# cboin1996/avddpg

Hardware: AMD Instinct MI355X
Metric: env-steps/sec + DDPG updates/sec, 4096x5-vehicle platoons (higher is better)
Workload: dtype f32-class (fp16 hi+lo operand pairs on the 16-bit matrix cores, f32 accumulate)

## Files before the change

avddpg_amd/_hip.py:

```python
import ctypes as C
import os

_HERE = os.path.dirname(os.path.abspath(__file__))
LIB_PATH = os.path.join(_HERE, "lib", "libavddpg_hip.so")
if os.environ.get("AVDDPG_HIP_LIB"):
    LIB_PATH = os.path.abspath(os.environ["AVDDPG_HIP_LIB"])
HEADER_PATH = os.path.join(os.path.dirname(_HERE), "include", "avddpg_hip.h")
AVD_MAX_L = 16


class AvdError(RuntimeError):
    pass


class EnvConsts(C.Structure):
    _fields_ = [("L", C.c_int32), ("model_a", C.c_int32), ("can_terminate", C.c_int32), ("uniform_reset", C.c_int32),
                ("max_ep", C.c_float), ("max_ev", C.c_float), ("abs_action_high", C.c_float),
                ("two_max_a", C.c_float), ("T", C.c_float),
                ("ca", C.c_float), ("cb", C.c_float), ("cc", C.c_float), ("cd", C.c_float),
                ("re_scalar", C.c_float), ("terminal_reward", C.c_float),
                ("stand_still", C.c_float), ("timegap", C.c_float),
                ("reset_ep_max", C.c_float), ("reset_max_ev", C.c_float), ("reset_max_a", C.c_float),
                ("reset_ep_eval", C.c_float), ("reset_ev_eval", C.c_float), ("reset_a_eval", C.c_float),
                ("leader_reset_a", C.c_float),
                ("A", (C.c_float * 16) * AVD_MAX_L), ("B", (C.c_float * 4) * AVD_MAX_L),
                ("C", (C.c_float * 4) * AVD_MAX_L)]


_LAYOUT_FIELDS = ["S", "A", "H1", "H2", "Ha", "B",
                  "aW1", "ab1", "ag1", "abe1", "aW2", "ab2", "ag2", "abe2", "aW3", "ab3", "actor_size",
                  "cWs", "cbs", "cgs", "cbes", "cWa", "cba", "cga", "cbea", "cW2", "cb2", "cg3", "cbe3", "cW3", "cb3",
                  "theta_size",
                  "amm1", "amv1", "amm2", "amv2", "cmms", "cmvs", "cmma", "cmva", "cmm3", "cmv3", "stats_size"]


class MlpLayout(C.Structure):
    _fields_ = [(n, C.c_int32) for n in _LAYOUT_FIELDS]


_P = C.c_void_p
_i, _f, _d, _u64, _i64 = C.c_int, C.c_float, C.c_double, C.c_uint64, C.c_int64
_LP = C.POINTER(MlpLayout)

_PROTOS = {
    "avd_mlp_layout_init": [_LP, _i, _i, _i, _i, _i, _i],
    "avd_env_step_f32": [_P, _i, _i, _P, _P, _P, _P, _P, _P, _P, _P, _P, _P, _P, _P],
    "avd_env_reset_f32": [_P, _i, _i, _P, _P, _P, _P, _P, _i, _u64, _u64, _P, _P],
    "avd_episode_end_f32": [_P, _i, _i, _i, _P, _P, _P, _P, _P, _P, _i, _P, _P, _P, _P, _i, _u64, _u64, _P],
    "avd_ou_step_f32": [_i, _P, _P, _f, _f, _f, _f, _u64, _u64, _P],
    "avd_policy_f32": [_i, _P, _P, _f, _f, _P, _P],
    "avd_normal_f32": [_i, _P, _f, _u64, _u64, _P],
    "avd_uniform_f32": [_i, _P, _f, _u64, _u64, _P],
    "avd_step_fused_f32": [_P, _i, _i, _i, _P, _P, _P, _P, _P, _P, _P, _P, _P, _P, _P, _P, _P, _f, _f, _f, _f, _f, _f, _f, _i, _u64, _u64,
                           _u64, _P, _i, _i64, _P, _P],
    "avd_replay_sample_f32": [_i, _i, _i, _i, _i, _P, _i, _u64, _u64, _P, _P, _P, _P, _P, _P],
    "avd_actor_forward_set_f32": [_LP, _i, _i, _P, _P, _P, _i, _f, _P, _P, _P],
    "avd_replay_add_f32": [_i, _i, _i, _i, _P, _i64, _P, _P, _i, _P, _P, _P],
    "avd_replay_indices": [_i, _i, _i, _u64, _u64, _P, _P],
    "avd_replay_gather_f32": [_i, _i, _i, _i, _i, _P, _P, _P, _P, _P, _P, _P],
    "avd_actor_forward_f32": [_LP, _i, _i, _P, _P, _P, _i, _f, _P, _P],
    "avd_actor_forward_cond_f32": [_LP, _i, _i, _P, _P, _P, _i, _f, _P, _P, _P],
    "avd_critic_forward_f32": [_LP, _i, _i, _P, _P, _P, _i, _P, _P, _P],
    "avd_learn_f32": [_LP, _i, _i, _P, _P, _P, _P, _P, _P, _P, _P, _f, _f, _P, _P, _P],
    "avd_learn_update_f32": [_LP, _i, _P, _P, _P, _P, _P, _P, _P, _P, _P, _P, _P, _P, _f, _f, _f, _f, _d, _P, _P, _P],
    "avd_learn_update_act_f32": [_LP, _i, _P, _P, _P, _P, _P, _P, _P, _P, _P, _P, _P, _P, _f, _f, _f, _f, _d, _P, _P, _P, _i, _P, _P],
    "avd_learn_update_plan": [_LP, _i, C.POINTER(C.c_int), C.POINTER(C.c_int), C.POINTER(C.c_int)],
    "avd_adam_polyak_f32": [_LP, _i, _P, _P, _P, _P, _P, _P, _P, _P, _f, _f, _d, _P],
    "avd_adam_polyak_guarded_f32": [_LP, _i, _P, _P, _P, _P, _P, _P, _P, _P, _f, _f, _d, _P, _P],
    "avd_polyak_f32": [_i64, _P, _P, _d, _P],
    "avd_fed_sum_f32": [_i, _i, _i, _i, _i, _P, _P, _P, _P, _P],
    "avd_fed_finalize_f32": [_i, _i, _P, _f, _P, _P],
    "avd_fed_scatter_f32": [_i, _i, _i, _i, _i, _i, _P, _P, _P],
    "avd_adam_polyak_intra_f32": [_LP, _i, _i, _i, _P, _P, _P, _P, _P, _P, _P, _P, _P, _f, _f, _d, _P],
    "avd_fed_history_push_f32": [_i, _i, _i, _P, _P, _P, _i, _P, _i, _i, _P, _P, _P],
    "avd_fed_weights_f32": [_i, _i, _i, _P, _P, _i, _P, _P, _P, _P],
    "avd_learn_shared_workspace": [_LP, _i, _i, C.POINTER(C.c_size_t)],
    "avd_learn_shared_bf16": [_LP, _i, _i, _P, _P, _P, _P, _P, _P, _P, _P, _P, _f, _f, _P, _P, _P, C.c_size_t, _P],
    "avd_learn_set_fused_workspace": [_LP, _i, _i, C.POINTER(C.c_size_t)],
    "avd_learn_set_fused_bf16": [_LP, _i, _i, _P, _P, _P, _P, _P, _P, _P, _P, _P, _f, _f, _P, _P, _P, C.c_size_t, _P],
    "avd_learn_set_split_workspace": [_LP, _i, _i, C.POINTER(C.c_size_t)],
    "avd_learn_set_split_mfma_count": [_LP, _i, _i, C.POINTER(C.c_ulonglong)],
    "avd_learn_set_split_critic": [_LP, _i, _i, _P, _P, _P, _P, _P, _P, _P, _P, _P, _f, _f, _P, _P, _P, C.c_size_t, _P],
    "avd_learn_set_split_actor": [_LP, _i, _i, _P, _P, _P, _f, _P, _P, C.c_size_t, _P],
    "avd_learn_set_split_bf16x3": [_LP, _i, _i, _P, _P, _P, _P, _P, _P, _P, _P, _P, _f, _f, _P, _P, _P, C.c_size_t, _P],
    "avd_learn_set_split_f16x3": [_LP, _i, _i, _P, _P, _P, _P, _P, _P, _P, _P, _P, _f, _f, _P, _P, _P, C.c_size_t, _P],
    "avd_actor_forward_shared_workspace": [_LP, _i, _i, C.POINTER(C.c_size_t)],
    "avd_actor_forward_shared_bf16": [_LP, _i, _i, _P, _P, _P, _f, _P, _P, C.c_size_t, _P],
    "avd_eval_rollout_f32": [_LP, _P, _i, _i, _i, _i, _P, _P, _i, _P, _P, _P, _P, _i, _P, _f, _f, _f, _f, _P, _i, _P, _P, _P, _P,
                             _P],
    "avd_gemm_bt_bf16": [_i, _i, _i, _P, C.c_long, _P, C.c_long, _P, C.c_long, _P],
}

_lib = None
DIAG_LIB_PATH = os.path.join(_HERE, "lib", "libavddpg_hip_diag.so")


def _load(path):
    if not os.path.exists(path):
        raise AvdError(f"{path} not found: build the HIP extension first (__graft_entry__.build()); "
                       "avddpg_amd has no CPU fallback")
    l = C.CDLL(path)
    missing = []
    for name, args in _PROTOS.items():
        fn = getattr(l, name, None)
        if fn is None:
            missing.append(name)
            continue
        fn.argtypes = args
        fn.restype = C.c_int
    if missing and not os.environ.get("AVDDPG_HIP_LIB"):
        raise AvdError(f"{path} does not export {', '.join(missing)}: rebuild it (make -C avddpg_amd/csrc)")
    l.avd_last_error.restype = C.c_char_p
    l.avd_last_error.argtypes = []
    l.avd_version.restype, l.avd_version.argtypes = C.c_int, []
    if getattr(l, "avd_diagnostics_enabled", None) is None:
        l.avd_diagnostics_enabled = lambda: 0
    else:
        l.avd_diagnostics_enabled.restype, l.avd_diagnostics_enabled.argtypes = C.c_int, []
    return l


def lib():
    global _lib
    if _lib is None:
        _lib = _load(LIB_PATH)
    return _lib


class diag_library:
    _cached = None
    _stack = []

    def __enter__(self):
        global _lib, LIB_PATH
        if diag_library._cached is None:
            diag_library._cached = _load(DIAG_LIB_PATH)
            if not diag_library._cached.avd_diagnostics_enabled():
                raise AvdError(f"{DIAG_LIB_PATH} is not a diagnostic build")
        diag_library._stack.append((lib(), LIB_PATH))
        _lib, LIB_PATH = diag_library._cached, DIAG_LIB_PATH
        return _lib

    def __exit__(self, *exc):
        global _lib, LIB_PATH
        _lib, LIB_PATH = diag_library._stack.pop()
        return False


def call(name, *args):
    fn = getattr(lib(), name, None)
    if fn is None:
        raise AvdError(f"{name} is not exported by the loaded library (an older build?)")
    rc = fn(*args)
    if rc != 0:
        raise AvdError(f"{name} failed ({rc}): {lib().avd_last_error().decode()}")


def ptr(t):
    if t is None:
        return None
    if not t.is_contiguous():
        raise AvdError("non-contiguous tensor passed to the C ABI")
    return C.c_void_p(t.data_ptr())


def stream_handle():
    import torch
    return C.c_void_p(torch.cuda.current_stream().cuda_stream)


def make_layout(S, A, H1, H2, Ha, B):
    lay = MlpLayout()
    call("avd_mlp_layout_init", C.byref(lay), S, A, H1, H2, Ha, B)
    return lay
```

avddpg_amd/csrc/fset.hip:

```cpp
#include "fset_common.h"

namespace avd {
namespace fset {

__device__ __forceinline__ bf16x8 make_xf(float x0, float x1, float x2, float x3, int h) {
    const bf16 a0 = (bf16)x0, a1 = (bf16)x1, a2 = (bf16)x2, a3 = (bf16)x3;
    const bf16 l0 = (bf16)(x0 - (float)a0), l1 = (bf16)(x1 - (float)a1), l2 = (bf16)(x2 - (float)a2), l3 = (bf16)(x3 - (float)a3);
    const bf16 one = (bf16)1.f, zero = (bf16)0.f;
    bf16x8 v;
    v[0] = a0, v[1] = a1, v[2] = a2, v[3] = a3;
    v[4] = h ? one : l0, v[5] = h ? one : l1, v[6] = h ? zero : l2, v[7] = h ? zero : l3;
    return v;
}
__device__ __forceinline__ bf16x8 make_wf(float w0, float w1, float w2, float w3, float b, int h) {
    const bf16 a0 = (bf16)w0, a1 = (bf16)w1, a2 = (bf16)w2, a3 = (bf16)w3, bh = (bf16)b;
    const bf16 l0 = (bf16)(w0 - (float)a0), l1 = (bf16)(w1 - (float)a1), l2 = (bf16)(w2 - (float)a2), l3 = (bf16)(w3 - (float)a3);
    const bf16 bl = (bf16)(b - (float)bh), zero = (bf16)0.f;
    bf16x8 v;
    v[0] = h ? l0 : a0, v[1] = h ? l1 : a1, v[2] = h ? l2 : a2, v[3] = h ? l3 : a3;
    v[4] = h ? bh : a0, v[5] = h ? bl : a1, v[6] = h ? zero : a2, v[7] = h ? zero : a3;
    return v;
}

struct NetP {
// ... 412 lines not shown
    };
    bf16x8 nx0 = {}, nx1 = {};
    float na0 = 0.f, na1 = 0.f;
    auto fetch_x = [&](int agent) {
        const bf16x8* xa = (const bf16x8*)p.xf + (long)agent * TILE * 2;
        nx0 = xa[2 * r + h], nx1 = xa[2 * (32 + r) + h];
        if (act_tiles) na0 = p.act[(long)agent * TILE + r], na1 = p.act[(long)agent * TILE + 32 + r];
    };
    if (j0 < P) fetch(j0 * p.n_sets + set), fetch_x(j0 * p.n_sets + set), stage(0);
    __syncthreads();
    const int g4 = lane >> 4, q = (lane & 15) >> 2, pp = lane & 3;
    int buf = 0;
    for (int pi = j0; pi < P; pi += J, buf ^= 1) {
        const bool more = pi + J < P;
        const bf16x8 xs0 = nx0, xs1 = nx1;
        const bf16x8 xa0 = make_xf(na0, 0.f, 0.f, 0.f, h), xa1 = make_xf(na1, 0.f, 0.f, 0.f, h);
        if (more) fetch((pi + J) * p.n_sets + set), fetch_x((pi + J) * p.n_sets + set);
        bf16x8 bfr[2][2];
#pragma unroll
        for (int rh = 0; rh < 2; ++rh)
#pragma unroll
            for (int s = 0; s < 2; ++s)
#pragma unroll
                for (int hf = 0; hf < 2; ++hf) {
                    const int R0 = 32 * rh + 16 * s + 8 * hf + 4 * (g4 >> 1);
                    const bf16x4 t = __builtin_amdgcn_ds_read_tr16_b64_v4bf16(
                        (__attribute__((address_space(3))) bf16x4*)(dzimg[buf] + (R0 + q) * LDZ + 32 * wn + 16 * (g4 & 1) + 4 * pp));
#pragma unroll
                    for (int j = 0; j < 4; ++j) bfr[rh][s][4 * hf + j] = t[j];
                }
#pragma unroll
        for (int i = 0; i < NFW; ++i) {
            if (fg * NFW + i >= NGT) continue;
            const bool at = act_tiles && i >= 3;
#pragma unroll
            for (int rh = 0; rh < 2; ++rh) {
                const bf16x8 xf = rh ? (at ? xa1 : xs1) : (at ? xa0 : xs0);
                const f32x16 p1 = mfma(xf, wf[i], zero16);
#pragma unroll
                for (int s = 0; s < 2; ++s) {
                    uint4 xu;
                    xu.x = relu_bf16x2(p1[8 * s], p1[8 * s + 1]), xu.y = relu_bf16x2(p1[8 * s + 2], p1[8 * s + 3]);
                    xu.z = relu_bf16x2(p1[8 * s + 4], p1[8 * s + 5]), xu.w = relu_bf16x2(p1[8 * s + 6], p1[8 * s + 7]);
                    G[i] = mfma(__builtin_bit_cast(bf16x8, xu), bfr[rh][s], G[i]);
                }
            }
        }
        if (more) stage(buf ^ 1);
        __syncthreads();
    }
#pragma unroll
    for (int i = 0; i < NFW; ++i) {
        if (fg * NFW + i >= NGT) continue;
        float* dst = p.partG + ((long)blockIdx.x * KG + 32 * (fg * NFW + i)) * H2 + 32 * wn + r;
#pragma unroll
        for (int k = 0; k < 16; ++k) dst[(long)acc_row(k, h) * H2] = G[i][k];
    }
}

struct DxArgs {
    NetP net;
    int n_agents, n_sets;
    const bf16* xf;
    const float* x;
    const bf16* dz;
    float* partU;
    float* partV;
};
template <int S, class NET>
__global__ __launch_bounds__(NT) void dx_kernel(const DxArgs p) {
    constexpr int KP = NET::KP, NF = 2, LDZ = 136;
    __shared__ __attribute__((aligned(16))) bf16 dzimg[2][TILE * LDZ];
    __shared__ __attribute__((aligned(16))) bf16 xt[8][2][32 * 32];
    const int tid = threadIdx.x, w = tid >> 6, lane = tid & 63, r = lane & 31, h = lane >> 5, rh = w & 1, fg = w >> 1;
    const int set = blockIdx.x % p.n_sets, j0 = blockIdx.x / p.n_sets, J = gridDim.x / p.n_sets, P = p.n_agents / p.n_sets;
    const float* th = p.net.th + (long)set * p.net.th_stride;
    const f32x16 zero16 = {};
    bf16x8 w2[NF][8], wf[NF];
    f32x16 V[NF];
    float U0[NF], U1[NF];
#pragma unroll
    for (int i = 0; i < NF; ++i) {
        const int ft = fg + 4 * i;
        const bf16* src = p.net.W2R + ((long)set * KP + 32 * ft + r) * H2 + 8 * h;
#pragma unroll
        for (int s = 0; s < 8; ++s) w2[i][s] = *(const bf16x8*)(src + 16 * s);
        wf[i] = layer1_wf<S, NET>(p.net, th, ft, r, h);
        V[i] = zero16, U0[i] = 0.f, U1[i] = 0.f;
    }
    for (int i = lane; i < 2 * 32 * 32; i += 64) {
        const int k = (i >> 5) & 31;
        xt[w][0][i] = (bf16)(k == 8 ? 1.f : 0.f);
    }
    const int srow = tid >> 3, sch = tid & 7;
    uint4 d0 = {}, d1 = {};
    auto fetch = [&](int agent) {
        const uint4* src = (const uint4*)(p.dz + ((long)agent * TILE + srow) * H2 + 16 * sch);
        d0 = src[0], d1 = src[1];
    };
    auto stage = [&](int buf) {
        uint4* dst = (uint4*)(dzimg[buf] + srow * LDZ + 16 * sch);
        dst[0] = d0, dst[1] = d1;
    };
    bf16x8 xfn = {};
    auto fetch_x = [&](int agent) { xfn = ((const bf16x8*)p.xf)[((long)agent * TILE + 32 * rh + r) * 2 + h]; };
    auto stage_x = [&](int buf) {
        if (h == 0) {
#pragma unroll
            for (int k = 0; k < 8; ++k) xt[w][buf][k * 32 + r] = xfn[k];
        }
    };
    __syncthreads();
    if (j0 < P) fetch(j0 * p.n_sets + set), fetch_x(j0 * p.n_sets + set), stage(0), stage_x(0);
    __syncthreads();
    int buf = 0;
    for (int pi = j0; pi < P; pi += J, buf ^= 1) {
        const bool more = pi + J < P;
        const bf16x8 xf = xfn;
        if (more) fetch((pi + J) * p.n_sets + set), fetch_x((pi + J) * p.n_sets + set);
        bf16x8 dzf[8];
        const bf16* arow = dzimg[buf] + (32 * rh + r) * LDZ + 8 * h;
#pragma unroll
        for (int s = 0; s < 8; ++s) dzf[s] = *(const bf16x8*)(arow + 16 * s);
        bf16x8 xb[2];
#pragma unroll
        for (int s = 0; s < 2; ++s) {
            const bf16x4 lo = *(const bf16x4*)(&xt[w][buf][r * 32 + 16 * s + 4 * h]);
            const bf16x4 hi = *(const bf16x4*)(&xt[w][buf][r * 32 + 16 * s + 8 + 4 * h]);
#pragma unroll
            for (int j = 0; j < 4; ++j) xb[s][j] = lo[j], xb[s][4 + j] = hi[j];
        }
#pragma unroll
        for (int i = 0; i < NF; ++i) {
            f32x16 dc = zero16;
#pragma unroll
            for (int s = 0; s < 8; ++s) dc = mfma(dzf[s], w2[i][s], dc);
            const f32x16 p1 = mfma(xf, wf[i], zero16);
            float u0 = 0.f, u1 = 0.f;
            bf16x8 va[2];
#pragma unroll
            for (int k = 0; k < 16; ++k) {
                const float pr = relu(p1[k]);
                u0 += dc[k];
                u1 = fmaf(dc[k], pr, u1);
                va[k >> 3][k & 7] = (bf16)(pr > 0.f ? dc[k] : 0.f);
            }
            U0[i] += u0, U1[i] += u1;
            V[i] = mfma(va[0], xb[0], V[i]);
            V[i] = mfma(va[1], xb[1], V[i]);
        }
        if (more) stage(buf ^ 1), stage_x(buf ^ 1);
        __syncthreads();
    }
#pragma unroll
    for (int i = 0; i < NF; ++i) {
        const int ft = fg + 4 * i;
        float* pu = p.partU + ((((long)blockIdx.x * 2 + rh) * 2 + h) * KP + 32 * ft + r) * 2;
        pu[0] = U0[i], pu[1] = U1[i];
        if (r < 16) {
            float* pv = p.partV + (((long)blockIdx.x * 2 + rh) * KP + 32 * ft) * 16 + r;
#pragma unroll
            for (int k = 0; k < 16; ++k) pv[(long)acc_row(k, h) * 16] = V[i][k];
        }
    }
}

template <int S>
__global__ __launch_bounds__(NT) void dxa_kernel(const DxArgs p) {
    typedef Critic NET;
    constexpr int KP = NET::KP;
    __shared__ __attribute__((aligned(16))) bf16 xt[8][2][32 * 32];
    __shared__ float comb[4][64][2 + 16];
    const int tid = threadIdx.x, w = tid >> 6, lane = tid & 63, r = lane & 31, h = lane >> 5, rh = w & 1, ftl = (w >> 1) & 1, par = w >> 2;
    const int set = blockIdx.x % p.n_sets, j0 = blockIdx.x / p.n_sets, J = gridDim.x / p.n_sets, P = p.n_agents / p.n_sets;
    const float* th = p.net.th + (long)set * p.net.th_stride;
    const f32x16 zero16 = {};
    const int ft = 8 + ftl;
    bf16x8 w2[8];
    {
        const bf16* src = p.net.W2R + ((long)set * KP + 32 * ft + r) * H2 + 8 * h;
#pragma unroll
        for (int s = 0; s < 8; ++s) w2[s] = *(const bf16x8*)(src + 16 * s);
    }
    const bf16x8 wf = layer1_wf<S, NET>(p.net, th, ft, r, h);
    f32x16 V = zero16;
    float U0 = 0.f, U1 = 0.f;
    for (int i = lane; i < 2 * 32 * 32; i += 64) {
        const int k = (i >> 5) & 31;
        xt[w][0][i] = (bf16)(k == 8 ? 1.f : 0.f);
    }
    __syncthreads();
    const int ntile = j0 < P ? (P - j0 + J - 1) / J : 0;
    bf16x8 dzn[8];
    float an = 0.f;
    auto fetch = [&](int k) {
        const long ri = (long)((j0 + k * J) * p.n_sets + set) * TILE + 32 * rh + r;
        const bf16* src = p.dz + ri * H2 + 8 * h;
#pragma unroll
        for (int s = 0; s < 8; ++s) dzn[s] = *(const bf16x8*)(src + 16 * s);
        an = p.x[ri];
    };
    if (par < ntile) fetch(par);
    int buf = 0;
    for (int k = par; k < ntile; k += 2, buf ^= 1) {
        bf16x8 dzf[8];
#pragma unroll
        for (int s = 0; s < 8; ++s) dzf[s] = dzn[s];
        const bf16x8 xf = make_xf(an, 0.f, 0.f, 0.f, h);
        if (k + 2 < ntile) fetch(k + 2);
        if (h == 0) {
            xt[w][buf][r] = xf[0];
            xt[w][buf][4 * 32 + r] = xf[4];
        }
        __builtin_amdgcn_fence(__ATOMIC_RELEASE, "wavefront");
        __builtin_amdgcn_wave_barrier();
        bf16x8 xb[2];
#pragma unroll
        for (int s = 0; s < 2; ++s) {
            const bf16x4 lo = *(const bf16x4*)(&xt[w][buf][r * 32 + 16 * s + 4 * h]);
            const bf16x4 hi = *(const bf16x4*)(&xt[w][buf][r * 32 + 16 * s + 8 + 4 * h]);
#pragma unroll
            for (int j = 0; j < 4; ++j) xb[s][j] = lo[j], xb[s][4 + j] = hi[j];
        }
        f32x16 dc = zero16;
#pragma unroll
        for (int s = 0; s < 8; ++s) dc = mfma(dzf[s], w2[s], dc);
        const f32x16 p1 = mfma(xf, wf, zero16);
        float u0 = 0.f, u1 = 0.f;
        bf16x8 va[2];
#pragma unroll
        for (int i = 0; i < 16; ++i) {
            const float pr = relu(p1[i]);
            u0 += dc[i];
            u1 = fmaf(dc[i], pr, u1);
            va[i >> 3][i & 7] = (bf16)(pr > 0.f ? dc[i] : 0.f);
        }
        U0 += u0, U1 += u1;
        V = mfma(va[0], xb[0], V);
        V = mfma(va[1], xb[1], V);
    }
    const int pw = w & 3;
    if (par == 1) {
        comb[pw][lane][0] = U0, comb[pw][lane][1] = U1;
#pragma unroll
        for (int i = 0; i < 16; ++i) comb[pw][lane][2 + i] = V[i];
    }
    __syncthreads();
    if (par == 0) {
        U0 += comb[pw][lane][0], U1 += comb[pw][lane][1];
        float* pu = p.partU + ((((long)blockIdx.x * 2 + rh) * 2 + h) * KP + 32 * ft + r) * 2;
        pu[0] = U0, pu[1] = U1;
        if (r < 16) {
            float* pv = p.partV + (((long)blockIdx.x * 2 + rh) * KP + 32 * ft) * 16 + r;
#pragma unroll
            for (int i = 0; i < 16; ++i) pv[(long)acc_row(i, h) * 16] = V[i] + comb[pw][lane][2 + i];
        }
    }
}

__global__ __launch_bounds__(512) void finalize_small_kernel(const FinArgs a) {
    const int set = blockIdx.x, net = a.net_lo + blockIdx.y, tid = threadIdx.x, jl = tid & 31;
    const int item = a.item_base + blockIdx.z * 16 + (tid >> 5);
    const bool critic = net;
    const avd_mlp_layout& L = a.L;
    const float* th = a.theta + (long)set * L.theta_size + (critic ? L.actor_size : 0);
    const float* st = a.stats + (long)set * L.stats_size;
    float* g = a.grads + (long)set * L.theta_size + (critic ? L.actor_size : 0);
    const int K = critic ? Critic::K : Actor::K, KP = critic ? Critic::KP : Actor::KP;
    auto allsum = [&](float v) {
#pragma unroll
        for (int o = 1; o < 32; o <<= 1) v += __shfl_xor(v, o);
        return v;
    };
    if (item < H2) {
        const int n = item;
        const int og2 = critic ? L.cg3 : L.ag2, obe2 = critic ? L.cbe3 : L.abe2, omm2 = critic ? L.cmm3 : L.amm2, omv2 = critic ? L.cmv3 : L.amv2;
        const int oW3 = critic ? L.cW3 : L.aW3, ob3 = critic ? L.cb3 : L.ab3, ob2 = critic ? L.cb2 : L.ab2;
        const int KG = critic ? Critic::KG : Actor::KG;
        float T1 = 0.f, S2 = 0.f, D = 0.f, Lc = 0.f, La = 0.f;
        const bool t1g = a.t1_from_g[net] != 0;
        for (int j = jl; j < a.J; j += 32) {
            const long wg = (long)j * a.n_sets + set;
            for (int w = 0; w < 8; ++w) {
                if (!t1g) T1 += a.partH[net][(wg * 8 + w) * H2 + n];
                D += a.partHs[net][(wg * 8 + w) * 2];
                if (critic && n == 0) Lc += a.partHs[1][(wg * 8 + w) * 2 + 1], La += a.partLa[(wg * 8 + w) * 2 + 1];
            }
            S2 += a.partG[net][(wg * KG + K) * H2 + n];
        }
        T1 = allsum(T1), S2 = allsum(S2), D = allsum(D);
        if (t1g && jl == 0) a.s2raw[((long)net * a.n_sets + set) * H2 + n] = S2;
        if (a.c3[net]) S2 *= a.c3[net][(long)set * VEC + H2 + n];
        if (critic && n == 0) Lc = allsum(Lc), La = allsum(La);
        if (a.bad && *a.bad) T1 = S2 = D = Lc = La = __uint_as_float(0x7fc00000u);
        if (jl == 0) {
            const float rs2 = 1.0f / sqrtf(st[omv2 + n] + BN_EPS), inv2 = rs2 * th[og2 + n], mm2 = st[omm2 + n];
            const float sh2 = th[obe2 + n] - mm2 * inv2, w3 = th[oW3 + n];
            if (!t1g) {
                g[oW3 + n] = inv2 * T1 + sh2 * D;
                g[og2 + n] = w3 * rs2 * (T1 - mm2 * D);
            }
            g[obe2 + n] = w3 * D;
            g[ob2 + n] = S2;
            if (n == 0) g[ob3] = D;
            if (critic && n == 0 && a.losses) a.losses[2 * set] = Lc * a.inv_n, a.losses[2 * set + 1] = -La * a.inv_n;
        }
        return;
    }
    const int f = item - H2;
    if (f >= K) return;
    float U0 = 0.f, U1 = 0.f, V[9];
#pragma unroll
    for (int k = 0; k < 9; ++k) V[k] = 0.f;
    const bool have_u = a.partU[net] != nullptr;
    for (int j = jl; j < a.J; j += 32) {
        const long wg = (long)j * a.n_sets + set;
        for (int rh = 0; rh < a.nrh; ++rh) {
            if (have_u)
                for (int h = 0; h < 2; ++h) {
                    const float* pu = a.partU[net] + ((((wg * a.nrh + rh) * 2 + h) * KP) + f) * 2;
                    U0 += pu[0], U1 += pu[1];
                }
            const float* pv = a.partV[net] + ((wg * a.nrh + rh) * KP + f) * 16;
#pragma unroll
            for (int k = 0; k < 9; ++k) V[k] += pv[k];
        }
    }
    U0 = allsum(U0), U1 = allsum(U1);
#pragma unroll
    for (int k = 0; k < 9; ++k) V[k] = allsum(V[k]);
    if (!have_u) {
        const int oW2 = critic ? L.cW2 : L.aW2, ob2 = critic ? L.cb2 : L.ab2;
        float u0 = 0.f;
        for (int n = jl; n < H2; n += 32) u0 = fmaf(th[oW2 + (long)f * H2 + n], g[ob2 + n], u0);
        U0 = allsum(u0);
        int oW, ob, ff = f, ld = H1, sin = a.S;
        if (!critic) oW = L.aW1, ob = L.ab1;
        else if (f < H1) oW = L.cWs, ob = L.cbs;
        else oW = L.cWa, ob = L.cba, ff = f - H1, ld = HA, sin = 1;
        U1 = th[ob + ff] * V[8];
        for (int k = 0; k < sin; ++k) U1 = fmaf(th[oW + k * ld + ff], V[k] + V[4 + k], U1);
    }
    if (a.bad && *a.bad) U0 = U1 = V[0] = V[4] = V[8] = __uint_as_float(0x7fc00000u);
    if (jl == 0) {
        int og, obe, omm, omv, oW, ob, ff = f, ld = H1, sin = a.S;
        if (!critic) og = L.ag1, obe = L.abe1, omm = L.amm1, omv = L.amv1, oW = L.aW1, ob = L.ab1;
        else if (f < H1) og = L.cgs, obe = L.cbes, omm = L.cmms, omv = L.cmvs, oW = L.cWs, ob = L.cbs;
        else og = L.cga, obe = L.cbea, omm = L.cmma, omv = L.cmva, oW = L.cWa, ob = L.cba, ff = f - H1, ld = HA, sin = 1;
        const float rs1 = 1.0f / sqrtf(st[omv + ff] + BN_EPS), inv1 = rs1 * th[og + ff], mm1 = st[omm + ff];
        g[obe + ff] = U0;
        g[og + ff] = rs1 * (U1 - mm1 * U0);
        g[ob + ff] = inv1 * V[8];
        for (int k = 0; k < sin; ++k) g[oW + k * ld + ff] = inv1 * (V[k] + V[4 + k]);
    }
}
__global__ __launch_bounds__(128) void finalize_w2_kernel(const FinArgs a) {
    const int f = blockIdx.x, set = blockIdx.y, net = a.net_lo + blockIdx.z, n = threadIdx.x;
    const bool critic = net;
    const int K = critic ? Critic::K : Actor::K, KG = critic ? Critic::KG : Actor::KG;
    if (f >= K) return;
    const avd_mlp_layout& L = a.L;
    const float* th = a.theta + (long)set * L.theta_size + (critic ? L.actor_size : 0);
    const float* st = a.stats + (long)set * L.stats_size;
    float* g = a.grads + (long)set * L.theta_size + (critic ? L.actor_size : 0);
    int og, obe, omm, omv, ff = f;
    if (!critic) og = L.ag1, obe = L.abe1, omm = L.amm1, omv = L.amv1;
    else if (f < H1) og = L.cgs, obe = L.cbes, omm = L.cmms, omv = L.cmvs;
    else og = L.cga, obe = L.cbea, omm = L.cmma, omv = L.cmva, ff = f - H1;
    const float inv1 = (1.0f / sqrtf(st[omv + ff] + BN_EPS)) * th[og + ff], sh1 = th[obe + ff] - st[omm + ff] * inv1;
    float G = 0.f;
    const float* pg = a.partG[net] + ((long)set * KG + f) * H2 + n;
    const long stride = (long)a.n_sets * KG * H2;
    int j = 0;
    for (; j + 8 <= a.J; j += 8) {
        float v[8];
#pragma unroll
        for (int u = 0; u < 8; ++u) v[u] = pg[(j + u) * stride];
#pragma unroll
        for (int u = 0; u < 8; ++u) G += v[u];
    }
    for (; j < a.J; ++j) G += pg[j * stride];
    const int oW2 = critic ? L.cW2 : L.aW2, ob2 = critic ? L.cb2 : L.ab2;
    if (a.t1_from_g[net]) a.t1p[(((long)net * a.n_sets + set) * Critic::K + f) * H2 + n] = inv1 * th[oW2 + (long)f * H2 + n] * G;
    if (a.c3[net]) G *= a.c3[net][(long)set * VEC + H2 + n];
    if (a.bad && *a.bad) G = __uint_as_float(0x7fc00000u);
    g[oW2 + (long)f * H2 + n] = inv1 * G + sh1 * g[ob2 + n];
}
__global__ __launch_bounds__(128) void finalize_t1_kernel(const FinArgs a) {
    const int set = blockIdx.x, net = a.net_lo + blockIdx.y, n = threadIdx.x;
    if (!a.t1_from_g[net]) return;
    const bool critic = net;
    const avd_mlp_layout& L = a.L;
    const float* th = a.theta + (long)set * L.theta_size + (critic ? L.actor_size : 0);
    const float* st = a.stats + (long)set * L.stats_size;
    float* g = a.grads + (long)set * L.theta_size + (critic ? L.actor_size : 0);
    const int K = critic ? Critic::K : Actor::K;
    const int og2 = critic ? L.cg3 : L.ag2, obe2 = critic ? L.cbe3 : L.abe2, omm2 = critic ? L.cmm3 : L.amm2, omv2 = critic ? L.cmv3 : L.amv2;
    const int oW3 = critic ? L.cW3 : L.aW3, ob3 = critic ? L.cb3 : L.ab3;
    const float* tp = a.t1p + ((long)net * a.n_sets + set) * Critic::K * H2 + n;
    float T1 = 0.f;
    int f = 0;
    for (; f + 8 <= K; f += 8) {
        float v[8];
#pragma unroll
        for (int u = 0; u < 8; ++u) v[u] = tp[(long)(f + u) * H2];
#pragma unroll
        for (int u = 0; u < 8; ++u) T1 += v[u];
    }
    for (; f < K; ++f) T1 += tp[(long)f * H2];
    T1 = fmaf(a.c3[net][(long)set * VEC + n], a.s2raw[((long)net * a.n_sets + set) * H2 + n], T1);
    const float D = g[ob3];
    if (a.bad && *a.bad) T1 = __uint_as_float(0x7fc00000u);
    const float rs2 = 1.0f / sqrtf(st[omv2 + n] + BN_EPS), inv2 = rs2 * th[og2 + n], mm2 = st[omm2 + n];
    const float sh2 = th[obe2 + n] - mm2 * inv2, w3 = th[oW3 + n];
    g[oW3 + n] = inv2 * T1 + sh2 * D;
    g[og2 + n] = w3 * rs2 * (T1 - mm2 * D);
}

void launch_finalize(const FinArgs& fa0, hipStream_t st, int net_lo, int n_nets) {
    FinArgs fa = fa0;
    fa.net_lo = net_lo, fa.item_base = 0;
    const int K = (net_lo + n_nets > 1) ? Critic::K : Actor::K;
    if (fa.partU[net_lo]) {
        hipLaunchKernelGGL(finalize_small_kernel, dim3(fa.n_sets, n_nets, (H2 + K + 15) / 16), dim3(512), 0, st, fa);
    } else {
        hipLaunchKernelGGL(finalize_small_kernel, dim3(fa.n_sets, n_nets, H2 / 16), dim3(512), 0, st, fa);
        fa.item_base = H2;
        hipLaunchKernelGGL(finalize_small_kernel, dim3(fa.n_sets, n_nets, (K + 15) / 16), dim3(512), 0, st, fa);
    }
    hipLaunchKernelGGL(finalize_w2_kernel, dim3(K, fa.n_sets, n_nets), dim3(H2), 0, st, fa);
    bool any = false;
    for (int net = net_lo; net < net_lo + n_nets; ++net) any = any || fa.t1_from_g[net];
    if (any) hipLaunchKernelGGL(finalize_t1_kernel, dim3(fa.n_sets, n_nets), dim3(H2), 0, st, fa);
}

struct Plan {
    int grid, J;
    size_t W2T[4], W2R[2], vec[4], a2, y, mu, dmu, dz, xfs, xfs2, partH[2], partHs[3], partU[2], partV[2], partG[2], bad, total;
};
int cu_count() {
    static int cache[64] = {0};
    int dev = 0;
    if (hipGetDevice(&dev) != hipSuccess || dev < 0) return 256;
    if (dev < 64 && cache[dev]) return cache[dev];
    hipDeviceProp_t prop;
    if (hipGetDeviceProperties(&prop, dev) != hipSuccess) return 256;
    const int n = prop.multiProcessorCount > 0 ? prop.multiProcessorCount : 256;
    if (dev < 64) cache[dev] = n;
    return n;
}
static Plan make_plan(int n_agents, int n_sets) {
    Plan pl;
    const int P = n_agents / n_sets;
    int J = cu_count() / n_sets;
    if (J < 1) J = 1;
    if (J > P) J = P;
    pl.J = J, pl.grid = J * n_sets;
    size_t o = 0;
    auto take = [&](size_t bytes) {
        const size_t at = o;
        o += (bytes + 255) / 256 * 256;
        return at;
    };
    for (int i = 0; i < 4; ++i) {
        const int KP = (i & 1) ? Critic::KP : Actor::KP, KW = (i & 1) ? Critic::KW : Actor::KW;
        pl.W2T[i] = take(sizeof(bf16) * (size_t)n_sets * H2 * KW);
        pl.vec[i] = take(sizeof(float) * (size_t)n_sets * VEC);
        if (i < 2) pl.W2R[i] = take(sizeof(bf16) * (size_t)n_sets * KP * H2);
    }
    const size_t rows = (size_t)n_agents * TILE;
    pl.a2 = take(4 * rows), pl.y = take(4 * rows), pl.mu = take(4 * rows), pl.dmu = take(4 * rows);
    pl.dz = take(sizeof(bf16) * rows * H2);
    pl.xfs = take(sizeof(bf16) * rows * 16), pl.xfs2 = take(sizeof(bf16) * rows * 16);
    for (int i = 0; i < 2; ++i) {
        const int KP = i ? Critic::KP : Actor::KP, KG = i ? Critic::KG : Actor::KG;
        pl.partH[i] = take(4 * (size_t)pl.grid * 8 * H2);
        pl.partU[i] = take(4 * (size_t)pl.grid * 2 * 2 * KP * 2);
        pl.partV[i] = take(4 * (size_t)pl.grid * 2 * KP * 16);
        pl.partG[i] = take(4 * (size_t)pl.grid * KG * H2);
    }
    for (int i = 0; i < 3; ++i) pl.partHs[i] = take(4 * (size_t)pl.grid * 8 * 2);
    pl.bad = take(sizeof(int));
    pl.total = o;
    return pl;
}
static int check_fset(const avd_mlp_layout* L, int n_agents, int n_sets, const char* who) {
    AVD_REQUIRE(L, "%s: null layout", who);
    if (L->H1 != H1 || L->H2 != H2 || L->Ha != HA || L->A != 1 || (L->S != 3 && L->S != 4) || L->B != TILE) {
        set_error("%s: serves the reference widths only (layer1 256, layer2 128, action layer 48, A = 1, S in {3, 4}, B = 64); "
                  "got H1=%d H2=%d Ha=%d A=%d S=%d B=%d (avd_learn_shared_bf16 takes other widths)",
                  who, L->H1, L->H2, L->Ha, L->A, L->S, L->B);
        return AVD_E_UNSUPPORTED;
    }
    AVD_REQUIRE(n_sets > 0 && n_sets <= 64 && n_agents > 0 && n_agents % n_sets == 0, "%s: n_agents=%d n_sets=%d", who, n_agents,
                n_sets);
    return AVD_OK;
}

template <int S>
static int run(const avd_mlp_layout& L, int n_agents, int n_sets, const float* theta, const float* stats, const float* theta_t,
               const float* stats_t, const float* s, const float* a, const float* r, const float* s2, const float* aw, float gamma,
               float high, float* grads, float* losses, unsigned char* ws, const Plan& pl, hipStream_t st) {
    PrepArgs pa;
    pa.L = L, pa.theta = theta, pa.stats = stats, pa.theta_t = theta_t, pa.stats_t = stats_t;
    NetP net[4];
    for (int i = 0; i < 4; ++i) {
        const bool critic = i & 1, target = i >= 2;
        pa.W2T[i] = (bf16*)(ws + pl.W2T[i]), pa.vec[i] = (float*)(ws + pl.vec[i]);
        pa.W2R[i] = i < 2 ? (bf16*)(ws + pl.W2R[i]) : nullptr;
        NetP& n = net[i];
        n.th = (target ? theta_t : theta) + (critic ? L.actor_size : 0), n.st = target ? stats_t : stats;
        n.th_stride = L.theta_size, n.st_stride = L.stats_size;
        n.oW1 = critic ? L.cWs : L.aW1, n.ob1 = critic ? L.cbs : L.ab1;
        n.oWa = critic ? L.cWa : 0, n.oba = critic ? L.cba : 0, n.oga = critic ? L.cga : 0, n.omva = critic ? L.cmva : 0;
        n.W2T = pa.W2T[i], n.W2R = pa.W2R[i], n.vec = pa.vec[i];
    }
    pa.bad = (int*)(ws + pl.bad);
    (void)hipMemsetAsync(ws + pl.bad, 0, sizeof(int), st);
    hipLaunchKernelGGL(prep_kernel, dim3(H2, 4, n_sets), dim3(320), 0, st, pa);
    const long nrows = (long)n_agents * TILE;
    bf16 *xfs = (bf16*)(ws + pl.xfs), *xfs2 = (bf16*)(ws + pl.xfs2);
    int* bad = (int*)(ws + pl.bad);
    hipLaunchKernelGGL(pack_x_kernel<S>, dim3((unsigned)((2 * nrows + 255) / 256)), dim3(256), 0, st, s, a, nrows, xfs, bad);
    hipLaunchKernelGGL(pack_x_kernel<S>, dim3((unsigned)((2 * nrows + 255) / 256)), dim3(256), 0, st, s2, r, nrows, xfs2, bad);
    const int P = n_agents / n_sets;
    const float inv_n = 1.0f / ((float)P * TILE);
    float *a2 = (float*)(ws + pl.a2), *y = (float*)(ws + pl.y), *mu = (float*)(ws + pl.mu), *dmu = (float*)(ws + pl.dmu);
    bf16* dz = (bf16*)(ws + pl.dz);
    auto F = [&](size_t off) { return (float*)(ws + off); };
    const dim3 grid(pl.grid), block(NT);
    HeadArgs h;
    h.n_agents = n_agents, h.n_sets = n_sets, h.gamma = gamma, h.high = high, h.inv_n = inv_n, h.aw = aw, h.dz = dz, h.dmu = dmu;
    auto head = [&](auto kern, int mode, int ni, const bf16* x, const float* act, const float* rr, const float* yin, float* out,
                    float* part, float* part_s) {
        h.net = net[ni], h.xf = x, h.act = act, h.r = rr, h.yin = yin, h.out = out, h.part = part, h.part_s = part_s;
        hipLaunchKernelGGL(kern, grid, dim3(64 * head_waves(mode)), 0, st, h);
    };
    DwArgs dw;
    dw.n_agents = n_agents, dw.n_sets = n_sets, dw.dz = dz;
    DxArgs dx;
    dx.n_agents = n_agents, dx.n_sets = n_sets, dx.dz = dz;
    head(head_kernel<S, Actor, OUT_TANH>, OUT_TANH, 2, xfs2, nullptr, nullptr, nullptr, a2, nullptr, nullptr);
    head(head_kernel<S, Critic, OUT_TD>, OUT_TD, 3, xfs2, a2, r, nullptr, y, nullptr, nullptr);
    head(head_kernel<S, Actor, OUT_TANH>, OUT_TANH, 0, xfs, nullptr, nullptr, nullptr, mu, nullptr, nullptr);
    head(head_kernel<S, Critic, HEAD_CRITIC>, HEAD_CRITIC, 1, xfs, a, nullptr, y, nullptr, F(pl.partH[1]), F(pl.partHs[1]));
    dw.net = net[1], dw.xf = xfs, dw.act = a, dw.partG = F(pl.partG[1]);
    hipLaunchKernelGGL((dw_kernel<S, Critic>), grid, block, 0, st, dw);
    dx.net = net[1], dx.partU = F(pl.partU[1]), dx.partV = F(pl.partV[1]);
    dx.xf = xfs, dx.x = nullptr;
    hipLaunchKernelGGL((dx_kernel<S, Critic>), grid, block, 0, st, dx);
    dx.x = a;
    hipLaunchKernelGGL((dxa_kernel<S>), grid, block, 0, st, dx);
    head(head_kernel<S, Critic, HEAD_CONST>, HEAD_CONST, 1, xfs, mu, nullptr, nullptr, nullptr, nullptr, F(pl.partHs[2]));
    head(head_kernel<S, Actor, HEAD_ACTOR>, HEAD_ACTOR, 0, xfs, nullptr, nullptr, dmu, nullptr, F(pl.partH[0]), F(pl.partHs[0]));
    dw.net = net[0], dw.xf = xfs, dw.act = nullptr, dw.partG = F(pl.partG[0]);
    hipLaunchKernelGGL((dw_kernel<S, Actor>), grid, block, 0, st, dw);
    dx.net = net[0], dx.partU = F(pl.partU[0]), dx.partV = F(pl.partV[0]), dx.x = nullptr;
    hipLaunchKernelGGL((dx_kernel<S, Actor>), grid, block, 0, st, dx);
    FinArgs fa;
    fa.L = L, fa.n_sets = n_sets, fa.J = pl.J, fa.S = S, fa.theta = theta, fa.stats = stats, fa.grads = grads, fa.losses = losses;
    fa.inv_n = inv_n, fa.partLa = F(pl.partHs[2]);
    for (int i = 0; i < 2; ++i)
        fa.partH[i] = F(pl.partH[i]), fa.partHs[i] = F(pl.partHs[i]), fa.partU[i] = F(pl.partU[i]), fa.partV[i] = F(pl.partV[i]),
        fa.partG[i] = F(pl.partG[i]);
    fa.nrh = 2, fa.c3[0] = fa.c3[1] = nullptr, fa.bad = (const int*)(ws + pl.bad);
    fa.t1_from_g[0] = fa.t1_from_g[1] = 0, fa.t1p = nullptr, fa.s2raw = nullptr;
    launch_finalize(fa, st);
    return check_launch("avd_learn_set_fused_bf16");
}

}
}

using namespace avd;

extern "C" int avd_learn_set_fused_workspace(const avd_mlp_layout* lay, int n_agents, int n_sets, size_t* bytes) {
    int rc = fset::check_fset(lay, n_agents, n_sets, "avd_learn_set_fused_workspace");
    if (rc) return rc;
    AVD_REQUIRE(bytes, "avd_learn_set_fused_workspace: null pointer");
    *bytes = fset::make_plan(n_agents, n_sets).total;
    return AVD_OK;
}

extern "C" int avd_learn_set_fused_bf16(const avd_mlp_layout* lay, int n_agents, int n_sets, const float* theta, const float* stats,
                                        const float* theta_t, const float* stats_t, const float* s, const float* a, const float* r,
                                        const float* s2, const float* agent_weight, float gamma, float high, float* grads,
                                        float* losses, void* workspace, size_t workspace_bytes, void* stream) {
    int rc = fset::check_fset(lay, n_agents, n_sets, "avd_learn_set_fused_bf16");
    if (rc) return rc;
    AVD_REQUIRE(theta && stats && theta_t && stats_t && s && a && r && s2 && grads && workspace,
                "avd_learn_set_fused_bf16: null pointer");
    const fset::Plan pl = fset::make_plan(n_agents, n_sets);
    AVD_REQUIRE(workspace_bytes >= pl.total, "avd_learn_set_fused_bf16: workspace %zu B < %zu B", workspace_bytes, pl.total);
    if (hipMemsetAsync(grads, 0, sizeof(float) * (size_t)n_sets * lay->theta_size, (hipStream_t)stream) != hipSuccess)
        return check_launch("avd_learn_set_fused_bf16: hipMemsetAsync(grads)");
    if (lay->S == 4)
        return fset::run<4>(*lay, n_agents, n_sets, theta, stats, theta_t, stats_t, s, a, r, s2, agent_weight, gamma, high, grads,
                            losses, (unsigned char*)workspace, pl, (hipStream_t)stream);
    return fset::run<3>(*lay, n_agents, n_sets, theta, stats, theta_t, stats_t, s, a, r, s2, agent_weight, gamma, high, grads, losses,
                        (unsigned char*)workspace, pl, (hipStream_t)stream);
}
```

avddpg_amd/csrc/fsplit.hip:

```cpp
#include <type_traits>

#include "fset_common.h"

namespace avd {
namespace fsplit {
using namespace fset;

struct ActorS {
    static constexpr int K = 256, KP = 256, NFT = 8, NKS = 16, LD = 264, NGT = 9, KG = 288;
    static constexpr bool critic = false;
};
struct CriticS {
    static constexpr int K = 304, KP = 320, NFT = 10, NKS = 19, LD = 312, NGT = 10, KG = 320;
    static constexpr bool critic = true;
};
constexpr int NGT_MAX = 10;

template <int I, int N, class F>
__device__ __forceinline__ void static_for(F&& f) {
    if constexpr (I < N) {
        f(std::integral_constant<int, I>{});
        static_for<I + 1, N>(f);
    }
}

typedef _Float16 f16;
typedef _Float16 f16x2 __attribute__((ext_vector_type(2)));
typedef _Float16 f16x8 __attribute__((ext_vector_type(8)));
constexpr float S1 = 64.f;
constexpr float F16_OVERFLOW = 65520.f;
#if defined(FSPLIT_ABL_CONST)
#define FSPLIT_ABL(x) FSPLIT_ABL_CONST
#elif defined(AVD_DIAG)
#define FSPLIT_ABL(x) (x)
#else
#define FSPLIT_ABL(x) 0
#endif
__device__ __forceinline__ void split2h(float a, float b, unsigned& hi, unsigned& lo) {
    const f32x2 f = {a, b};
    const f16x2 h = __builtin_convertvector(f, f16x2);
    hi = __builtin_bit_cast(unsigned, h);
    f32x2 l;
#ifdef __HIP_DEVICE_COMPILE__
    asm("v_fma_mix_f32 %0, -%1, 1.0, %2 op_sel:[0,0,0] op_sel_hi:[1,0,0]" : "=v"(l[0]) : "v"(hi), "v"(a));
    asm("v_fma_mix_f32 %0, -%1, 1.0, %2 op_sel:[1,0,0] op_sel_hi:[1,0,0]" : "=v"(l[1]) : "v"(hi), "v"(b));
#else
    l[0] = a - (float)h[0], l[1] = b - (float)h[1];
#endif
    lo = __builtin_bit_cast(unsigned, __builtin_convertvector(l, f16x2));
}
__device__ __forceinline__ void split1h(float x, f16& hi, f16& lo) {
    hi = (f16)x;
    lo = (f16)(x - (float)hi);
}
template <class V>
__device__ __forceinline__ void pin16(V& x) {
#pragma unroll
    for (int q = 0; q < 2; ++q) {
        float a = x[8 * q], b = x[8 * q + 1], c = x[8 * q + 2], d = x[8 * q + 3], e = x[8 * q + 4], f = x[8 * q + 5], g = x[8 * q + 6], h = x[8 * q + 7];
        asm volatile("" : "+v"(a), "+v"(b), "+v"(c), "+v"(d), "+v"(e), "+v"(f), "+v"(g), "+v"(h));
        x[8 * q] = a, x[8 * q + 1] = b, x[8 * q + 2] = c, x[8 * q + 3] = d, x[8 * q + 4] = e, x[8 * q + 5] = f, x[8 * q + 6] = g, x[8 * q + 7] = h;
    }
}
__device__ __forceinline__ f16x8 fragh(unsigned a, unsigned b, unsigned c, unsigned d) {
    uint4 o;
    o.x = a, o.y = b, o.z = c, o.w = d;
    return __builtin_bit_cast(f16x8, o);
}
__device__ __forceinline__ f32x16 mfmah(f16x8 a, f16x8 b, f32x16 c) {
    return __builtin_amdgcn_mfma_f32_32x32x16_f16(a, b, c, 0, 0, 0);
}
__device__ __forceinline__ f16x8 make_xh(float x0, float x1, float x2, float x3, int h) {
    f16 a0, a1, a2, a3, l0, l1, l2, l3;
    split1h(x0, a0, l0), split1h(x1, a1, l1), split1h(x2, a2, l2), split1h(x3, a3, l3);
    const f16 one = (f16)1.f, zero = (f16)0.f;
    f16x8 v;
    v[0] = a0, v[1] = a1, v[2] = a2, v[3] = a3;
    v[4] = h ? one : l0, v[5] = h ? one : l1, v[6] = h ? zero : l2, v[7] = h ? zero : l3;
    return v;
}
__device__ __forceinline__ f16x8 make_wh(float w0, float w1, float w2, float w3, float b, float sc, int h) {
    f16 a0, a1, a2, a3, l0, l1, l2, l3, bh, bl;
    split1h(sc * w0, a0, l0), split1h(sc * w1, a1, l1), split1h(sc * w2, a2, l2), split1h(sc * w3, a3, l3), split1h(sc * b, bh, bl);
    const f16 zero = (f16)0.f;
    f16x8 v;
    v[0] = h ? l0 : a0, v[1] = h ? l1 : a1, v[2] = h ? l2 : a2, v[3] = h ? l3 : a3;
    v[4] = h ? bh : a0, v[5] = h ? bl : a1, v[6] = h ? bh : a2, v[7] = h ? zero : a3;
    return v;
}
__device__ __forceinline__ f16x8 make_xg(float x0, float x1, float x2, float x3, float g, int h) {
    f16 a0, a1, a2, a3, l0, l1, l2, l3, gh, gl;
    split1h(x0, a0, l0), split1h(x1, a1, l1), split1h(x2, a2, l2), split1h(x3, a3, l3), split1h(g, gh, gl);
    const f16 zero = (f16)0.f;
    f16x8 v;
    v[0] = a0, v[1] = a1, v[2] = a2, v[3] = a3;
    v[4] = h ? gh : l0, v[5] = h ? gh : l1, v[6] = h ? gl : l2, v[7] = h ? zero : l3;
    return v;
}

template <int S>
__device__ __forceinline__ void load_x(const float* xa, long row, float (&x)[4]) {
    if (S == 4) {
        const float4 v = *(const float4*)(xa + 4 * row);
        x[0] = v.x, x[1] = v.y, x[2] = v.z, x[3] = v.w;
    } else {
#pragma unroll
        for (int k = 0; k < 4; ++k) x[k] = k < S ? xa[S * row + k] : 0.f;
    }
}

__host__ __device__ constexpr int wpos(int f) { return (f & ~12) | ((f & 4) << 1) | ((f & 8) >> 1); }

struct NetP {
    const float* th;
    long th_stride;
    const f16* Whi;
    const f16* Wlo;
    const f16* Wchi;
    const f16* Wclo;
    const f16x8* wf1h;
    const float* vec;
    const unsigned* wap;
};

struct PackArgs {
    const float* x[2];
    const float* extra[2];
    f16x8* outh[2];
    long rows;
    int* bad;
};
template <int S>
__global__ __launch_bounds__(256) void pack_x_kernel(const PackArgs a) {
    const int which = blockIdx.y;
    const float* x = a.x[which];
    const float* extra = a.extra[which];
    const bool extra_is_action = which == 0;
    const long i = (long)blockIdx.x * 256 + threadIdx.x;
    if (i >= 2 * a.rows) return;
    float v[4];
    load_x<S>(x, i >> 1, v);
    bool nf = not_finite(v[0]) || not_finite(v[1]) || not_finite(v[2]) || not_finite(v[3]);
    nf = nf || fmaxf(fmaxf(fabsf(v[0]), fabsf(v[1])), fmaxf(fabsf(v[2]), fabsf(v[3]))) >= F16_OVERFLOW;
    if (!(i & 1)) {
        const float e = extra[i >> 1];
        nf = nf || not_finite(e) || (extra_is_action && fabsf(e) >= F16_OVERFLOW);
    }
    if (nf) atomicOr(a.bad, 1);
    a.outh[which][i] = make_xh(v[0], v[1], v[2], v[3], (int)(i & 1));
}

struct PrepArgs {
    avd_mlp_layout L;
    int S;
    const float *theta, *stats, *theta_t, *stats_t;
    f16 *Whi[4], *Wlo[4];
    f16 *Wchi[4], *Wclo[4];
    f16x8* wf1h[4];
    float* vec[4];
    unsigned* wap;
    unsigned* smax;
    int* bad;
};
constexpr int SCALE_SLICES = 16;
__device__ __forceinline__ float pow2_for(float mx) {
    int e = 0;
    if (mx > 0.f && !not_finite(mx)) (void)frexpf(mx, &e);
    int k = 13 - e;
    k = k < -14 ? -14 : (k > 30 ? 30 : k);
    return ldexpf(1.f, k);
}
__global__ __launch_bounds__(256) void scale_kernel(const PrepArgs a) {
    __shared__ float red[256], red2[256], c3a[H2], inva[CriticS::K];
    const int net = blockIdx.x, set = blockIdx.y, slice = blockIdx.z, tid = threadIdx.x;
    const bool critic = net & 1, target = net >= 2;
    const avd_mlp_layout& L = a.L;
    const float* th = (target ? a.theta_t : a.theta) + (long)set * L.theta_size + (critic ? L.actor_size : 0);
    const float* st = (target ? a.stats_t : a.stats) + (long)set * L.stats_size;
    const int K = critic ? CriticS::K : ActorS::K, oW2 = critic ? L.cW2 : L.aW2;
    const int og2 = critic ? L.cg3 : L.ag2, omv2 = critic ? L.cmv3 : L.amv2, oW3 = critic ? L.cW3 : L.aW3;
    if (tid < H2) c3a[tid] = fabsf((1.0f / sqrtf(st[omv2 + tid] + BN_EPS)) * th[og2 + tid] * th[oW3 + tid]);
    for (int f = tid; f < K; f += 256) {
        int og, omv, ff = f;
        if (!critic) og = L.ag1, omv = L.amv1;
        else if (f < H1) og = L.cgs, omv = L.cmvs;
        else og = L.cga, omv = L.cmva, ff = f - H1;
        inva[f] = fabsf((1.0f / sqrtf(st[omv + ff] + BN_EPS)) * th[og + ff]);
    }
    __syncthreads();
    const int total = K * H2, per = (total + SCALE_SLICES - 1) / SCALE_SLICES, lo = slice * per, hi = min(total, lo + per);
    float m = 0.f, m2 = 0.f;
    for (int i = lo + tid; i < hi; i += 256) {
        const float w = fabsf(th[oW2 + i]);
        m = fmaxf(m, inva[i / H2] * w);
        m2 = fmaxf(m2, c3a[i % H2] * w);
    }
    red[tid] = m, red2[tid] = m2;
    __syncthreads();
    for (int o = 128; o > 0; o >>= 1) {
        if (tid < o) red[tid] = fmaxf(red[tid], red[tid + o]), red2[tid] = fmaxf(red2[tid], red2[tid + o]);
        __syncthreads();
    }
    if (tid == 0) {
        unsigned* dst = a.smax + ((long)net * gridDim.y + set) * 2;
        atomicMax(dst, __float_as_uint(red[0]));
        atomicMax(dst + 1, __float_as_uint(red2[0]));
    }
}
__global__ __launch_bounds__(320) void prep_kernel(const PrepArgs a) {
    __shared__ float red[320];
    const int n = blockIdx.x, net = blockIdx.y, set = blockIdx.z, f = threadIdx.x;
    const bool critic = net & 1, target = net >= 2;
    const avd_mlp_layout& L = a.L;
    const float* th = (target ? a.theta_t : a.theta) + (long)set * L.theta_size + (critic ? L.actor_size : 0);
    const float* st = (target ? a.stats_t : a.stats) + (long)set * L.stats_size;
    const int K = critic ? CriticS::K : ActorS::K, KP = critic ? CriticS::KP : ActorS::KP;
    const int oW2 = critic ? L.cW2 : L.aW2, ob2 = critic ? L.cb2 : L.ab2, oW3 = critic ? L.cW3 : L.aW3, ob3 = critic ? L.cb3 : L.ab3;
    const int og2 = critic ? L.cg3 : L.ag2, obe2 = critic ? L.cbe3 : L.abe2, omm2 = critic ? L.cmm3 : L.amm2, omv2 = critic ? L.cmv3 : L.amv2;
    const float inv2n = (1.0f / sqrtf(st[omv2 + n] + BN_EPS)) * th[og2 + n], c3n = inv2n * th[oW3 + n];
    const unsigned* smax = a.smax + ((long)net * gridDim.z + set) * 2;
    const float SW = pow2_for(__uint_as_float(smax[0])), SWC = pow2_for(__uint_as_float(smax[1]));
    float shw = 0.f;
    if (f < KP) {
        float w = 0.f, inv = 0.f;
        if (f < K) {
            int og, obe, omm, omv, ff = f;
            if (!critic) og = L.ag1, obe = L.abe1, omm = L.amm1, omv = L.amv1;
            else if (f < H1) og = L.cgs, obe = L.cbes, omm = L.cmms, omv = L.cmvs;
            else og = L.cga, obe = L.cbea, omm = L.cmma, omv = L.cmva, ff = f - H1;
            inv = (1.0f / sqrtf(st[omv + ff] + BN_EPS)) * th[og + ff];
            const float sh = th[obe + ff] - st[omm + ff] * inv;
            w = th[oW2 + (long)f * H2 + n];
            shw = sh * w;
            if (not_finite(w) || not_finite(inv) || not_finite(sh)) atomicOr(a.bad, 1);
            f16 hi, lo;
            const float ws = SW * (inv * w);
            if (fabsf(ws) >= F16_OVERFLOW) atomicOr(a.bad, 1);
            split1h(ws, hi, lo);
            const long at = ((long)set * H2 + n) * K + wpos(f);
            a.Whi[net][at] = hi, a.Wlo[net][at] = lo;
        }
        if (!target) {
            f16 hi, lo;
            const float wc = SWC * (c3n * w);
            if (fabsf(wc) >= F16_OVERFLOW) atomicOr(a.bad, 1);
            split1h(wc, hi, lo);
            const long at = ((long)set * KP + f) * H2 + n;
            a.Wchi[net][at] = hi, a.Wclo[net][at] = lo;
        }
    }
    red[f] = shw;
    __syncthreads();
    if (f < 64) red[f] += red[f + 256];
    __syncthreads();
    for (int o = 128; o > 0; o >>= 1) {
        if (f < o) red[f] += red[f + o];
        __syncthreads();
    }
    float* vec = a.vec[net] + (long)set * VEC;
    if (f == 0) {
        if (n == 0) vec[2 * H2 + 1] = SW, vec[2 * H2 + 2] = SWC;
        vec[n] = th[ob2 + n] + red[0];
        vec[H2 + n] = c3n;
        if (not_finite(vec[n]) || not_finite(c3n) || not_finite(th[ob3])) atomicOr(a.bad, 1);
    }
    if (n == 0) {
        __syncthreads();
        float v = 0.f;
        if (f < H2) {
            const float inv2 = (1.0f / sqrtf(st[omv2 + f] + BN_EPS)) * th[og2 + f];
            v = (th[obe2 + f] - st[omm2 + f] * inv2) * th[oW3 + f];
        }
        red[f] = v;
        __syncthreads();
        for (int o = 64; o > 0; o >>= 1) {
            if (f < o) red[f] += red[f + o];
            __syncthreads();
        }
        if (f == 0) vec[2 * H2] = th[ob3] + red[0];
    }
}
__global__ __launch_bounds__(64) void prep1_kernel(const PrepArgs a) {
    const int ft = blockIdx.x, net = blockIdx.y, set = blockIdx.z, lane = threadIdx.x, r = lane & 31, h = lane >> 5;
    const bool critic = net & 1, target = net >= 2;
    const avd_mlp_layout& L = a.L;
    const float* th = (target ? a.theta_t : a.theta) + (long)set * L.theta_size + (critic ? L.actor_size : 0);
    const int K = critic ? CriticS::K : ActorS::K;
    const int f = 32 * ft + r;
    float w[4] = {0.f, 0.f, 0.f, 0.f}, b = 0.f;
    if (f == K) {
        b = 1.f;
    } else if (f < K) {
        if (critic && ft >= 8) {
            w[0] = th[L.cWa + (f - H1)], b = th[L.cba + (f - H1)];
        } else {
            const float* W = th + (critic ? L.cWs : L.aW1);
#pragma unroll
            for (int k = 0; k < 4; ++k) w[k] = k < a.S ? W[k * H1 + f] : 0.f;
            b = th[(critic ? L.cbs : L.ab1) + f];
        }
        if (not_finite(w[0]) || not_finite(w[1]) || not_finite(w[2]) || not_finite(w[3]) || not_finite(b)) atomicOr(a.bad, 1);
        if (S1 * fmaxf(fmaxf(fabsf(w[0]), fabsf(w[1])), fmaxf(fmaxf(fabsf(w[2]), fabsf(w[3])), fabsf(b))) >= F16_OVERFLOW) atomicOr(a.bad, 1);
    }
    a.wf1h[net][((long)set * NGT_MAX + ft) * 64 + lane] = make_wh(w[0], w[1], w[2], w[3], b, S1, h);
    if (net == 1 && ft == 0 && lane < 48) {
        const int hl = lane / 24, hh = (lane / 12) & 1, ks = (lane / 4) % 3, m = lane & 3;
        unsigned v = 0;
#pragma unroll
        for (int e = 0; e < 2; ++e) {
            const int jj = 2 * m + e, fa = 16 * ks + 8 * (jj >> 2) + 4 * hh + (jj & 3);
            f16 hi, lo;
            split1h(S1 * th[L.cWa + fa], hi, lo);
            v |= (unsigned)__builtin_bit_cast(unsigned short, hl ? lo : hi) << (16 * e);
        }
        a.wap[(long)set * 48 + lane] = v;
    }
}

enum HeadMode { OUT_TANH = 0, OUT_TD = 1, HEAD_BOTH = 5, OUT_TANH_SAVE = 6 };
struct HeadArgs {
    unsigned long long* stamp;
    NetP net;
    int n_agents, n_sets;
    const f16x8* xf;
    const float* act;
    const float* act2;
    const float* r;
    const float* yin;
    const float* aw;
    float* out;
    f16* sm;
    float* g3;
    float* dmu;
    float* part_s;
    float* part_s2;
    float* part_m;
    float* tz;
    float gamma, high, inv_n;
    int* bad;
    int abl;
};
#ifndef HEAD_FAST
#define HEAD_FAST 5
#define HEAD_SLOW 3
#endif

template <int S, class NET, int MODE>
__global__ __launch_bounds__(NT) void head_kernel(const HeadArgs p) {
    constexpr int K = NET::K, NKS = NET::NKS, NFT = NET::NFT, LD = NET::LD;
    constexpr int NTH = NT;
    constexpr bool BOTH = (MODE == HEAD_BOTH);
    static_assert(!BOTH || NET::critic, "HEAD_BOTH is a critic mode");
    __shared__ __attribute__((aligned(16))) f16 wimg[2][H2 * LD];
    __shared__ __attribute__((aligned(16))) float b2s[H2];
    __shared__ __attribute__((aligned(16))) float c3s[H2];
    __shared__ __attribute__((aligned(16))) unsigned waps[BOTH ? 48 : 4];
    const int tid = threadIdx.x, w = tid >> 6, lane = tid & 63, r = lane & 31, h = lane >> 5, q = w >> 1, rh = w & 1;
    const int set = blockIdx.x % p.n_sets, j0 = blockIdx.x / p.n_sets, J = gridDim.x / p.n_sets, P = p.n_agents / p.n_sets;
    for (int i = tid; i < 2 * H2 * (K / 8); i += NTH) {
        const int hl = i / (H2 * (K / 8)), rem = i - hl * (H2 * (K / 8)), n = rem / (K / 8), c = rem - n * (K / 8);
        const f16* src = (hl ? p.net.Wlo : p.net.Whi) + ((long)set * H2 + n) * K + 8 * c;
        *(uint4*)(&wimg[hl][n * LD + 8 * c]) = *(const uint4*)src;
    }
    const float* vec = p.net.vec + (long)set * VEC;
    const float SW = vec[2 * H2 + 1], sc = SW * S1, isc = 1.f / sc;
    if (tid < H2) b2s[tid] = vec[tid] * sc, c3s[tid] = vec[H2 + tid] * isc;
    if (BOTH && tid < 48) waps[tid] = p.net.wap[(long)set * 48 + tid];
    const float d3 = vec[2 * H2];
    const f16x8* wf1 = p.net.wf1h + (long)set * NGT_MAX * 64 + lane;
    const f32x16 zero16 = {};
#ifdef AVD_STAMP
    unsigned long long hacc[4] = {0, 0, 0, 0}, hlast = __builtin_amdgcn_s_memtime();
    const unsigned long long hstart = hlast;
#define HSTAMP(i) { const unsigned long long t_ = __builtin_amdgcn_s_memtime(); hacc[i] += t_ - hlast; hlast = t_; }
#else
#define HSTAMP(i)
#endif
    float Dacc = 0.f, Lacc = 0.f, Dacc2 = 0.f, Lacc2 = 0.f, gmax = 0.f;
    unsigned watch = 0;
    auto look = [&](float x) {
        unsigned u = __float_as_uint(x);
        asm volatile("" : "+v"(u));
        u &= 0x7fffffffu;
        watch = watch > u ? watch : u;
    };
    __syncthreads();

    const int ntile = j0 < P ? (P - j0 + J - 1) / J : 0;
    const int row = 32 * rh + r;
    f16x8 nx = {};
    float na = 0.f, nb = 0.f, ny = 0.f, nw = 1.f;
    auto fetch_in = [&](int k) {
        const int agent = (j0 + k * J) * p.n_sets + set;
        const long ri = (long)agent * TILE + row;
        nx = p.xf[2 * ri + h];
        if (NET::critic) na = p.act[ri];
        if (BOTH) nb = p.act2[ri];
        if (MODE == OUT_TD) ny = p.r[ri];
        if (BOTH) ny = p.yin[ri];
        if (BOTH && p.aw) nw = p.aw[agent];
    };
    const f16* whi0 = &wimg[0][r * LD + 8 * h];
    const f16* wlo0 = &wimg[1][r * LD + 8 * h];
    constexpr int NSEQ = BOTH ? 8 : NFT;
    HSTAMP(3);
    constexpr int FAST = HEAD_FAST, SLOW = HEAD_SLOW, PERIOD = 2 * (FAST + SLOW);
    const int qs = __builtin_amdgcn_readfirstlane(q);
    const int cnt = qs < 2 ? FAST : SLOW, start = qs < 2 ? qs * FAST : 2 * FAST + (qs - 2) * SLOW;
    int k = start, pos = 0;
    auto next_tile = [&](int kk, int pp) { return pp + 1 == cnt ? kk + PERIOD - cnt + 1 : kk + 1; };
    if (k < ntile) fetch_in(k);
    for (int ui = 0; k < ntile; ++ui, k = next_tile(k, pos), pos = pos + 1 == cnt ? 0 : pos + 1) {
        const int agent = (j0 + k * J) * p.n_sets + set;
        const long ri = (long)agent * TILE + row;
        const f16x8 xs = nx, xa = make_xh(na, 0.f, 0.f, 0.f, h), xb = BOTH ? make_xh(nb, 0.f, 0.f, 0.f, h) : xa;
        const float ty = ny, tw = nw;
        if (next_tile(k, pos) < ntile) fetch_in(next_tile(k, pos));
        f32x16 acc[4];
#pragma unroll
        for (int t = 0; t < 4; ++t)
#pragma unroll
            for (int g = 0; g < 4; ++g) {
                const float4 b = *(const float4*)(b2s + 32 * t + 8 * g + 4 * h);
                acc[t][4 * g] = b.x, acc[t][4 * g + 1] = b.y, acc[t][4 * g + 2] = b.z, acc[t][4 * g + 3] = b.w;
            }
        unsigned ph[8], pl[8];
        auto split16 = [&](const f32x16& p1) {
            if (FSPLIT_ABL(p.abl) & 4) {
#pragma unroll
                for (int m = 0; m < 8; ++m) ph[m] = __float_as_uint(p1[2 * m]), pl[m] = __float_as_uint(p1[2 * m + 1]);
                return;
            }
#pragma unroll
            for (int m = 0; m < 8; ++m) split2h(relu(p1[2 * m]), relu(p1[2 * m + 1]), ph[m], pl[m]);
        };
        auto zdot_t = [&](f32x16& a, int t) {
            float zp = 0.f;
#pragma unroll
            for (int g = 0; g < 4; ++g) {
                const float4 c = *(const float4*)(c3s + 32 * t + 8 * g + 4 * h);
                const float cc[4] = {c.x, c.y, c.z, c.w};
#pragma unroll
                for (int j = 0; j < 4; ++j) {
                    a[4 * g + j] = relu(a[4 * g + j]);
                    zp = fmaf(a[4 * g + j], cc[j], zp);
                }
            }
            return zp;
        };
        auto zdot_nd = [&](const f32x16& a, int t) {
            float zp = 0.f;
#pragma unroll
            for (int g = 0; g < 4; ++g) {
                const float4 c = *(const float4*)(c3s + 32 * t + 8 * g + 4 * h);
                const float cc[4] = {c.x, c.y, c.z, c.w};
#pragma unroll
                for (int j = 0; j < 4; ++j) zp = fmaf(relu(a[4 * g + j]), cc[j], zp);
            }
            return zp;
        };
        auto mask_t = [&](const f32x16& a, int t, unsigned s16, f16* dst) {
            unsigned pk[4][2];
#pragma unroll
            for (int g = 0; g < 4; ++g)
#pragma unroll
                for (int e = 0; e < 2; ++e) {
                    const int i = 4 * g + 2 * e;
                    pk[g][e] = (a[i] > 0.f ? s16 : 0u) | (a[i + 1] > 0.f ? s16 << 16 : 0u);
                }
#pragma unroll
            for (int gg = 0; gg < 2; ++gg) {
                const auto s0 = __builtin_amdgcn_permlane32_swap(pk[2 * gg][0], pk[2 * gg + 1][0], false, false);
                const auto s1 = __builtin_amdgcn_permlane32_swap(pk[2 * gg][1], pk[2 * gg + 1][1], false, false);
                uint4 o;
                o.x = s0[0], o.y = s1[0], o.z = s0[1], o.w = s1[1];
                *(uint4*)(dst + 32 * t + 16 * gg) = o;
            }
        };
        auto out_z = [&](f32x16 (&ac)[4]) {
            float zp = 0.f;
#pragma unroll
            for (int t = 0; t < 4; ++t) zp += zdot_t(ac[t], t);
            zp += __shfl_xor(zp, 32);
            return d3 + zp;
        };
        split16(mfmah(wf1[0], xs, zero16));
        f16x8 wfn = wf1[64];
        f16x8 wg[2][2][2];
        auto read_group = [&](int g, f16x8 (&dst)[2][2]) {
            const int ks = g >> 1, th = g & 1;
#pragma unroll
            for (int tt = 0; tt < 2; ++tt) {
                dst[tt][0] = *(const f16x8*)(whi0 + 32 * (2 * th + tt) * LD + 16 * ks);
                dst[tt][1] = *(const f16x8*)(wlo0 + 32 * (2 * th + tt) * LD + 16 * ks);
            }
        };
        read_group(0, wg[0]);
        auto tile = [&](auto si_c, f32x16 (&ac)[4]) {
            constexpr int si = decltype(si_c)::value;
            constexpr int ft = si;
            f32x16 p1n = zero16;
            if constexpr (si + 1 < NSEQ) {
                p1n = mfmah(wfn, (NET::critic && si + 1 >= 8) ? xa : xs, zero16);
                if constexpr (si + 2 < NSEQ) wfn = wf1[64 * (si + 2)];
            }
#pragma unroll
            for (int s = 0; s < 2; ++s) {
                const int ks = 2 * ft + s;
                if (ks >= NKS) continue;
                const f16x8 bhi = fragh(ph[4 * s], ph[4 * s + 1], ph[4 * s + 2], ph[4 * s + 3]);
                const f16x8 blo = fragh(pl[4 * s], pl[4 * s + 1], pl[4 * s + 2], pl[4 * s + 3]);
#pragma unroll
                for (int th = 0; th < 2; ++th) {
                    const int g = 2 * ks + th;
                    if (g + 1 < 2 * (BOTH ? 16 : NKS)) read_group(g + 1, wg[(g + 1) & 1]);
#pragma unroll
                    for (int tt = 0; tt < 2; ++tt) {
                        const int t = 2 * th + tt;
                        const f16x8 whi = wg[g & 1][tt][0], wlo = wg[g & 1][tt][1];
                        ac[t] = mfmah(whi, bhi, ac[t]);
                        ac[t] = mfmah(wlo, bhi, ac[t]);
                        ac[t] = mfmah(whi, blo, ac[t]);
                    }
                }
// ... 389 lines not shown
    if (p.stamp && blockIdx.x == 16 && lane == 0)
        for (int i = 0; i < 4; ++i) p.stamp[w * 8 + i] = tacc[i];
#endif
    const float dsc = 1.f / (gsc * S1);
    float* comb = (float*)&smimg[0][0];
    const int cidx = NET::critic ? 2 * (w >> 2) + (w & 1) : (w & 3);
    if (xrh == 1) {
#pragma unroll
        for (int c = 0; c < XC; ++c)
#pragma unroll
            for (int k = 0; k < 16; ++k) comb[((cidx * XC + c) * 16 + k) * 64 + lane] = G1[c][k];
    }
    __syncthreads();
#pragma unroll
    for (int c = 0; c < 4; ++c) {
        float* dst = p.partG + ((long)blockIdx.x * KG + 32 * w) * H2 + 32 * c + r;
#pragma unroll
        for (int k = 0; k < 16; ++k) dst[(long)acc_row(k, h) * H2] = G0[c][k] * dsc;
    }
    if (xrh == 0) {
#pragma unroll
        for (int c = 0; c < XC; ++c) {
            float* dst = p.partG + ((long)blockIdx.x * KG + 32 * xt) * H2 + 32 * (xc0 + c) + r;
#pragma unroll
            for (int k = 0; k < 16; ++k) dst[(long)acc_row(k, h) * H2] = (G1[c][k] + comb[((cidx * XC + c) * 16 + k) * 64 + lane]) * dsc;
        }
    }
}

struct DxArgs {
    NetP net;
    int n_agents, n_sets;
    const f16x8* xfh;
    const float* act;
    int L_cWa, L_cba;
    const float* g3;
    const float* part_m;
    const f16* sm;
    int unsigned_mask;
    float* partV;
    int abl;
    unsigned long long* stamp;
};
template <int S, class NET>
__global__ __launch_bounds__(NT) void dx_kernel(const DxArgs p) {
    constexpr int KP = NET::KP, LDZ = 136;
    constexpr float VSH = 1.f / 32.f;
    __shared__ __attribute__((aligned(16))) f16 smimg[2][TILE * LDZ];
    __shared__ __attribute__((aligned(16))) f16 xt[2][2][32 * 32];
    __shared__ __attribute__((aligned(16))) float g3s[2][TILE];
    __shared__ float gred[8];
    const int tid = threadIdx.x, w = __builtin_amdgcn_readfirstlane(tid >> 6), lane = tid & 63, r = lane & 31, h = lane >> 5, ft = w;
    const int set = blockIdx.x % p.n_sets, j0 = blockIdx.x / p.n_sets, J = gridDim.x / p.n_sets, P = p.n_agents / p.n_sets;
    const f32x16 zero16 = {};
    const float gsc = set_gscale(p.part_m, set, p.n_sets, J, gred);
    f16x8 wch[8], wcl[8];
    {
        const long at = ((long)set * KP + 32 * ft + r) * H2 + 8 * h;
#pragma unroll
        for (int s = 0; s < 8; ++s) wch[s] = *(const f16x8*)(p.net.Wchi + at + 16 * s), wcl[s] = *(const f16x8*)(p.net.Wclo + at + 16 * s);
    }
    const float swc = __uint_as_float(__builtin_amdgcn_readfirstlane(__float_as_uint(p.net.vec[(long)set * VEC + 2 * H2 + 2])));
    const float gv = gsc * VSH, vs = gsc * swc * VSH;
    const f16x8 wf = p.net.wf1h[((long)set * NGT_MAX + ft) * 64 + lane];
    f32x16 V = zero16;
    for (int i = tid; i < 2 * 2 * 32 * 32; i += NT) {
        const int k = (i >> 5) & 31;
        (&xt[0][0][0])[i] = (f16)(k == 8 ? 1.f : 0.f);
    }
    const int srow = tid >> 3, sch = tid & 7;
    uint4 d0 = {}, d1 = {};
    float gn = 0.f;
    auto fetch = [&](int agent) {
        if (FSPLIT_ABL(p.abl) & 1) agent = j0 * p.n_sets + set;
        const uint4* src = (const uint4*)(p.sm + ((long)agent * TILE + srow) * H2 + 16 * sch);
        d0 = src[0], d1 = src[1];
        if (tid < TILE) gn = p.g3[(long)agent * TILE + tid];
    };
    auto stage = [&](int buf) {
        uint4* dst = (uint4*)(smimg[buf] + srow * LDZ + 16 * sch);
        dst[0] = d0, dst[1] = d1;
        if (tid < TILE) g3s[buf][tid] = (p.unsigned_mask ? gn : fabsf(gn)) * gv;
    };
    f16x8 xfn0 = {}, xfn1 = {};
    auto fetch_x = [&](int agent) {
        xfn0 = p.xfh[((long)agent * TILE + r) * 2 + h];
        xfn1 = p.xfh[((long)agent * TILE + 32 + r) * 2 + h];
    };
    auto stage_x = [&](int buf) {
        if (w < 2 && h == 0) {
            f16x8 src = xfn0;
            if (w == 1) src = xfn1;
            asm volatile("" : "+v"(src));
#pragma unroll
            for (int k = 0; k < 8; ++k) xt[buf][w][k * 32 + r] = src[k];
        }
    };
    __syncthreads();
    if (j0 < P) fetch(j0 * p.n_sets + set), fetch_x(j0 * p.n_sets + set), stage(0), stage_x(0);
    __syncthreads();
#ifdef AVD_STAMP
    unsigned long long dacc[4] = {0, 0, 0, 0}, dlast = __builtin_amdgcn_s_memtime();
#define DXSTAMP(i) { const unsigned long long t_ = __builtin_amdgcn_s_memtime(); dacc[i] += t_ - dlast; dlast = t_; }
#else
#define DXSTAMP(i)
#endif
    int buf = 0;
    for (int pi = j0; pi < P; pi += J, buf ^= 1) {
        const bool more = pi + J < P;
        const f16x8 xf[2] = {xfn0, xfn1};
        if (more) fetch((pi + J) * p.n_sets + set), fetch_x((pi + J) * p.n_sets + set);
        DXSTAMP(0);
        auto read_a = [&](int e, f16x8 (&smf)[8]) {
            const f16* arow = smimg[buf] + (32 * e + r) * LDZ + 8 * h;
#pragma unroll
            for (int s = 0; s < 8; ++s) smf[s] = *(const f16x8*)(arow + 16 * s);
        };
        typedef _Float16 f16x4 __attribute__((ext_vector_type(4)));
        auto read_img = [&](const f16* img, f16x8 (&xb)[2]) {
#pragma unroll
            for (int s = 0; s < 2; ++s) {
                const f16x4 lo = *(const f16x4*)(img + r * 32 + 16 * s + 4 * h);
                const f16x4 hi = *(const f16x4*)(img + r * 32 + 16 * s + 8 + 4 * h);
#pragma unroll
                for (int j = 0; j < 4; ++j) xb[s][j] = lo[j], xb[s][4 + j] = hi[j];
            }
        };
        auto backward = [&](int e, const f32x16& dc, const f32x16& p1, unsigned (&vh)[8], unsigned (&vl)[8]) {
            if (FSPLIT_ABL(p.abl) & 4) {
#pragma unroll
                for (int m = 0; m < 8; ++m) vh[m] = __float_as_uint(dc[2 * m]) ^ __float_as_uint(p1[2 * m]), vl[m] = __float_as_uint(dc[2 * m + 1]);
                return;
            }
#pragma unroll
            for (int g = 0; g < 4; ++g) {
                const float4 gq = *(const float4*)(&g3s[buf][32 * e + 8 * g + 4 * h]);
                const float gg[4] = {gq.x, gq.y, gq.z, gq.w};
                float dm[4];
#pragma unroll
                for (int j = 0; j < 4; ++j) {
                    const int k = 4 * g + j;
                    dm[j] = p1[k] > 0.f ? dc[k] * gg[j] : 0.f;
                }
                split2h(dm[0], dm[1], vh[2 * g], vl[2 * g]);
                split2h(dm[2], dm[3], vh[2 * g + 1], vl[2 * g + 1]);
            }
        };
        f16x8 smf[8], xb0[2], xb1[2];
        unsigned vh0[8], vl0[8], vh1[8], vl1[8];
        read_a(0, smf);
        f32x16 dc0 = zero16;
#pragma unroll
        for (int s = 0; s < 8; ++s) dc0 = mfmah(smf[s], wch[s], dc0), dc0 = mfmah(smf[s], wcl[s], dc0);
        const f32x16 p10 = mfmah(xf[0], wf, zero16);
        __builtin_amdgcn_sched_barrier(0);
        read_a(1, smf);
        read_img(xt[buf][0], xb0);
        f32x16 dc1 = zero16;
#pragma unroll
        for (int s = 0; s < 8; ++s) dc1 = mfmah(smf[s], wch[s], dc1), dc1 = mfmah(smf[s], wcl[s], dc1);
        const f32x16 p11 = mfmah(xf[1], wf, zero16);
        backward(0, dc0, p10, vh0, vl0);
        __builtin_amdgcn_sched_group_barrier(0x100, 12, 0);
#pragma unroll
        for (int i = 0; i < 17; ++i) {
            __builtin_amdgcn_sched_group_barrier(0x008, 1, 0);
            __builtin_amdgcn_sched_group_barrier(0x002, 5, 0);
            __builtin_amdgcn_sched_group_barrier(0x100, 1, 0);
        }
        __builtin_amdgcn_sched_barrier(0);
        read_img(xt[buf][1], xb1);
#pragma unroll
        for (int s = 0; s < 2; ++s) {
            V = mfmah(fragh(vh0[4 * s], vh0[4 * s + 1], vh0[4 * s + 2], vh0[4 * s + 3]), xb0[s], V);
            V = mfmah(fragh(vl0[4 * s], vl0[4 * s + 1], vl0[4 * s + 2], vl0[4 * s + 3]), xb0[s], V);
        }
        backward(1, dc1, p11, vh1, vl1);
#pragma unroll
        for (int s = 0; s < 2; ++s) {
            V = mfmah(fragh(vh1[4 * s], vh1[4 * s + 1], vh1[4 * s + 2], vh1[4 * s + 3]), xb1[s], V);
            V = mfmah(fragh(vl1[4 * s], vl1[4 * s + 1], vl1[4 * s + 2], vl1[4 * s + 3]), xb1[s], V);
        }
        DXSTAMP(1);
        if (more) stage(buf ^ 1), stage_x(buf ^ 1);
        DXSTAMP(2);
        if (!(FSPLIT_ABL(p.abl) & 2)) __syncthreads();
        DXSTAMP(3);
    }
#ifdef AVD_STAMP
    if (p.stamp && blockIdx.x == 16 && lane == 0)
        for (int i = 0; i < 4; ++i) p.stamp[w * 8 + i] = dacc[i];
#endif
    const float ivs = 1.f / vs;
    if (r < 16) {
        float* pv = p.partV + ((long)blockIdx.x * KP + 32 * ft) * 16 + r;
#pragma unroll
        for (int k = 0; k < 16; ++k) pv[(long)acc_row(k, h) * 16] = V[k] * ivs;
    }
}

template <int S>
__global__ __launch_bounds__(NT) void dxa_kernel(const DxArgs p) {
    typedef CriticS NET;
    constexpr int KP = NET::KP;
    constexpr float VSH = 1.f / 32.f;
    constexpr int LDZ = 136;
    __shared__ __attribute__((aligned(16))) f16 simg[8][32 * LDZ];
    __shared__ __attribute__((aligned(16))) float ga[8][2][2][32];
    __shared__ float comb[8][64][2];
    __shared__ float gred[8];
    const int tid = threadIdx.x, w = __builtin_amdgcn_readfirstlane(tid >> 6), lane = tid & 63, r = lane & 31, h = lane >> 5;
    const int rh = w & 1, ftl = (w >> 1) & 1, par = w >> 2;
    const int set = blockIdx.x % p.n_sets, j0 = blockIdx.x / p.n_sets, J = gridDim.x / p.n_sets, P = p.n_agents / p.n_sets;
    const f32x16 zero16 = {};
    const int ft = 8 + ftl, f = 32 * ftl + r;
    const float gsc = set_gscale(p.part_m, set, p.n_sets, J, gred);
    f16x8 wch[8], wcl[8];
    {
        const long at = ((long)set * KP + 32 * ft + r) * H2 + 8 * h;
#pragma unroll
        for (int s = 0; s < 8; ++s) wch[s] = *(const f16x8*)(p.net.Wchi + at + 16 * s), wcl[s] = *(const f16x8*)(p.net.Wclo + at + 16 * s);
    }
    const float swc = __uint_as_float(__builtin_amdgcn_readfirstlane(__float_as_uint(p.net.vec[(long)set * VEC + 2 * H2 + 2])));
    const float gv = gsc * VSH, vs = gsc * swc * VSH;
    const float* th = p.net.th + (long)set * p.net.th_stride;
    const float wa = f < HA ? th[p.L_cWa + f] : 0.f, ba = f < HA ? th[p.L_cba + f] : 0.f;
    float Sa = 0.f, Sb = 0.f;
    const int ntile = j0 < P ? (P - j0 + J - 1) / J : 0;
    uint4 A0 = {}, A1 = {}, A2 = {}, A3 = {}, A4 = {}, A5 = {}, A6 = {}, A7 = {}, B0 = {}, B1 = {}, B2 = {}, B3 = {}, B4 = {}, B5 = {}, B6 = {}, B7 = {};
    float gA = 0.f, aA = 0.f, gB = 0.f, aB = 0.f;
#define DXA_FETCH(k_, X, g_, a_)                                                                                    \
    {                                                                                                               \
        const long r0_ = (long)((j0 + (k_) * J) * p.n_sets + set) * TILE + 32 * rh;                                 \
        const uint4* src_ = (const uint4*)(p.sm + r0_ * H2) + lane;  \
        X##0 = src_[0], X##1 = src_[64], X##2 = src_[128], X##3 = src_[192], X##4 = src_[256], X##5 = src_[320], X##6 = src_[384], X##7 = src_[448]; \
        g_ = p.g3[r0_ + r], a_ = p.act[r0_ + r];                                                                    \
    }
#define DXA_PUT(buf_, X, g_, a_)                                                                                    \
    {                                                                                                               \
        if (h == 0) ga[w][buf_][0][r] = fabsf(g_) * gv, ga[w][buf_][1][r] = a_;                                     \
        f16* dst_ = simg[w] + (lane >> 4) * LDZ + 8 * (lane & 15);                                                   \
        *(uint4*)(dst_) = X##0, *(uint4*)(dst_ + 4 * LDZ) = X##1, *(uint4*)(dst_ + 8 * LDZ) = X##2, *(uint4*)(dst_ + 12 * LDZ) = X##3; \
        *(uint4*)(dst_ + 16 * LDZ) = X##4, *(uint4*)(dst_ + 20 * LDZ) = X##5, *(uint4*)(dst_ + 24 * LDZ) = X##6, *(uint4*)(dst_ + 28 * LDZ) = X##7; \
        __builtin_amdgcn_fence(__ATOMIC_RELEASE, "wavefront");                                                      \
        __builtin_amdgcn_wave_barrier();                                                                            \
    }
    auto unit = [&](int buf) {
        f32x16 dc = zero16;
        const f16* arow = simg[w] + r * LDZ + 8 * h;
#pragma unroll
        for (int s = 0; s < 8; ++s) {
            const f16x8 af = *(const f16x8*)(arow + 16 * s);
            dc = mfmah(af, wch[s], dc), dc = mfmah(af, wcl[s], dc);
        }
        float sa = 0.f, sb = 0.f;
#pragma unroll
        for (int q = 0; q < 4; ++q) {
            const float4 gq = *(const float4*)(&ga[w][buf][0][8 * q + 4 * h]), aq = *(const float4*)(&ga[w][buf][1][8 * q + 4 * h]);
            const float gg[4] = {gq.x, gq.y, gq.z, gq.w}, av[4] = {aq.x, aq.y, aq.z, aq.w};
#pragma unroll
            for (int j = 0; j < 4; ++j) {
                const float m = fmaf(av[j], wa, ba) > 0.f ? dc[4 * q + j] * gg[j] : 0.f;
                sa = fmaf(m, av[j], sa);
                sb += m;
            }
        }
        Sa += sa, Sb += sb;
        __builtin_amdgcn_fence(__ATOMIC_ACQ_REL, "wavefront");
        __builtin_amdgcn_wave_barrier();
    };
    if (par < ntile) DXA_FETCH(par, A, gA, aA);
    if (par + 2 < ntile) DXA_FETCH(par + 2, B, gB, aB);
    for (int k = par; k < ntile; k += 4) {
        DXA_PUT(0, A, gA, aA);
        if (k + 4 < ntile) DXA_FETCH(k + 4, A, gA, aA);
        unit(0);
        if (k + 2 < ntile) {
            DXA_PUT(1, B, gB, aB);
            if (k + 6 < ntile) DXA_FETCH(k + 6, B, gB, aB);
            unit(1);
        }
    }
#undef DXA_FETCH
#undef DXA_PUT
    comb[w][lane][0] = Sa, comb[w][lane][1] = Sb;
    __syncthreads();
    if (rh == 0 && par == 0 && h == 0) {
        const int ws[4] = {w, w + 1, w + 4, w + 5};
        float t[2] = {0.f, 0.f};
#pragma unroll
        for (int i = 0; i < 4; ++i)
#pragma unroll
            for (int c = 0; c < 2; ++c) t[c] += comb[ws[i]][r][c] + comb[ws[i]][32 + r][c];
        const float ivs = 1.f / vs;
        float* pv = p.partV + ((long)blockIdx.x * KP + 32 * ft + r) * 16;
#pragma unroll
        for (int c = 0; c < 9; ++c) pv[c] = c == 0 ? t[0] * ivs : (c == 8 ? t[1] * ivs : 0.f);
    }
}

struct Plan {
    int grid, J;
    size_t Whi[4], Wlo[4], Wchi[2], Wclo[2], wf1h[4], vec[4], wap, a2, y, mu, dmu, g3, sm, sma, tz, t1p, s2raw, xfs, xfs2, partHs[3], partM[2],
        partV[2], partG[2], bad, total;
};
static Plan make_plan(int n_agents, int n_sets) {
    Plan pl;
    const int P = n_agents / n_sets;
    int J = cu_count() / n_sets;
    if (const char* e = AVD_DIAG_ENV("FSPLIT_J")) J = atoi(e);
    if (J < 1) J = 1;
    if (J > P) J = P;
    pl.J = J, pl.grid = J * n_sets;
    size_t o = 0;
    auto take = [&](size_t bytes) {
        const size_t at = o;
        o += (bytes + 255) / 256 * 256;
        return at;
    };
    for (int i = 0; i < 4; ++i) {
        const int K = (i & 1) ? CriticS::K : ActorS::K, KP = (i & 1) ? CriticS::KP : ActorS::KP;
        pl.Whi[i] = take(sizeof(f16) * (size_t)n_sets * H2 * K), pl.Wlo[i] = take(sizeof(f16) * (size_t)n_sets * H2 * K);
        pl.vec[i] = take(sizeof(float) * (size_t)n_sets * VEC);
        pl.wf1h[i] = take(16 * (size_t)n_sets * NGT_MAX * 64);
        if (i < 2) pl.Wchi[i] = take(sizeof(f16) * (size_t)n_sets * KP * H2), pl.Wclo[i] = take(sizeof(f16) * (size_t)n_sets * KP * H2);
    }
    pl.wap = take(4 * (size_t)n_sets * 48);
    const size_t rows = (size_t)n_agents * TILE;
    pl.a2 = take(4 * rows), pl.y = take(4 * rows), pl.mu = take(4 * rows), pl.dmu = take(4 * rows), pl.g3 = take(4 * rows);
    pl.sm = take(sizeof(f16) * rows * H2);
    pl.sma = take(sizeof(f16) * rows * H2);
    pl.tz = take(4 * rows);
    pl.t1p = take(2 * 4 * (size_t)n_sets * CriticS::K * H2), pl.s2raw = take(2 * 4 * (size_t)n_sets * H2);
    pl.xfs = take(32 * rows), pl.xfs2 = take(32 * rows);
    for (int i = 0; i < 2; ++i) {
        const int KP = i ? CriticS::KP : ActorS::KP, KG = i ? CriticS::KG : ActorS::KG;
        pl.partM[i] = take(4 * (size_t)pl.grid * 8);
        pl.partV[i] = take(4 * (size_t)pl.grid * KP * 16);
        pl.partG[i] = take(4 * (size_t)pl.grid * KG * H2);
    }
    for (int i = 0; i < 3; ++i) pl.partHs[i] = take(4 * (size_t)pl.grid * 8 * 2);
    pl.bad = take(sizeof(int) + sizeof(unsigned) * 4 * (size_t)n_sets * 2);
    pl.total = o;
    return pl;
}
static int check_shape(const avd_mlp_layout* L, int n_agents, int n_sets, const char* who) {
    AVD_REQUIRE(L, "%s: null layout", who);
    if (L->H1 != H1 || L->H2 != H2 || L->Ha != HA || L->A != 1 || (L->S != 3 && L->S != 4) || L->B != TILE) {
        set_error("%s: serves the reference widths only (layer1 256, layer2 128, action layer 48, A = 1, S in {3, 4}, B = 64); "
                  "got H1=%d H2=%d Ha=%d A=%d S=%d B=%d (avd_learn_shared_bf16 takes other widths)",
                  who, L->H1, L->H2, L->Ha, L->A, L->S, L->B);
        return AVD_E_UNSUPPORTED;
    }
    AVD_REQUIRE(n_sets > 0 && n_sets <= 64 && n_agents > 0 && n_agents % n_sets == 0, "%s: n_agents=%d n_sets=%d", who, n_agents,
                n_sets);
    return AVD_OK;
}

enum Phase { PH_CRITIC = 1, PH_ACTOR = 2, PH_BOTH = 3 };
template <int S>
static int run(int phases, const avd_mlp_layout& L, int n_agents, int n_sets, const float* theta, const float* stats, const float* theta_t,
               const float* stats_t, const float* s, const float* a, const float* r, const float* s2, const float* aw, float gamma,
               float high, float* grads, float* losses, unsigned char* ws, const Plan& pl, hipStream_t st) {
    PrepArgs pa;
    pa.L = L, pa.S = S, pa.theta = theta, pa.stats = stats, pa.theta_t = theta_t, pa.stats_t = stats_t;
    pa.wap = (unsigned*)(ws + pl.wap), pa.bad = (int*)(ws + pl.bad), pa.smax = (unsigned*)(ws + pl.bad + sizeof(int));
    NetP net[4];
    for (int i = 0; i < 4; ++i) {
        const bool critic = i & 1, target = i >= 2;
        pa.Whi[i] = (f16*)(ws + pl.Whi[i]), pa.Wlo[i] = (f16*)(ws + pl.Wlo[i]), pa.vec[i] = (float*)(ws + pl.vec[i]);
        pa.wf1h[i] = (f16x8*)(ws + pl.wf1h[i]);
        pa.Wchi[i] = i < 2 ? (f16*)(ws + pl.Wchi[i]) : nullptr, pa.Wclo[i] = i < 2 ? (f16*)(ws + pl.Wclo[i]) : nullptr;
        NetP& n = net[i];
        n.th = (target ? theta_t : theta) + (critic ? L.actor_size : 0), n.th_stride = L.theta_size;
        n.Whi = pa.Whi[i], n.Wlo = pa.Wlo[i], n.Wchi = pa.Wchi[i], n.Wclo = pa.Wclo[i], n.wf1h = pa.wf1h[i], n.vec = pa.vec[i];
        n.wap = pa.wap;
    }
    const int P = n_agents / n_sets;
    const float inv_n = 1.0f / ((float)P * TILE);
    const long nrows = (long)n_agents * TILE;
    f16x8 *xfs = (f16x8*)(ws + pl.xfs), *xfs2 = (f16x8*)(ws + pl.xfs2);
    int* bad = (int*)(ws + pl.bad);
    float *a2 = (float*)(ws + pl.a2), *y = (float*)(ws + pl.y), *mu = (float*)(ws + pl.mu), *dmu = (float*)(ws + pl.dmu);
    float* g3 = (float*)(ws + pl.g3);
    f16 *sm = (f16*)(ws + pl.sm), *sma = (f16*)(ws + pl.sma);
    auto F = [&](size_t off) { return (float*)(ws + off); };
    const dim3 grid(pl.grid), block(NT);
    HeadArgs h;
    h.n_agents = n_agents, h.n_sets = n_sets, h.gamma = gamma, h.high = high, h.inv_n = inv_n, h.aw = aw, h.sm = sm, h.g3 = g3, h.dmu = dmu;
    h.act2 = nullptr, h.part_s2 = nullptr, h.stamp = nullptr, h.bad = bad, h.part_m = nullptr, h.tz = F(pl.tz), h.abl = 0;
    if (const char* e = AVD_DIAG_ENV("FSPLIT_ABL")) h.abl = atoi(e);
    auto head = [&](auto kern, int ni, const f16x8* x, const float* act, const float* rr, const float* yin, float* out, float* part_s) {
        h.net = net[ni], h.xf = x, h.act = act, h.r = rr, h.yin = yin, h.out = out, h.part_s = part_s;
        hipLaunchKernelGGL(kern, grid, block, 0, st, h);
    };
    DwArgs dw;
    dw.n_agents = n_agents, dw.n_sets = n_sets, dw.sm = sm, dw.g3 = g3, dw.x = s, dw.stamp = nullptr, dw.abl = 0;
    if (const char* e = AVD_DIAG_ENV("FSPLIT_ABL")) dw.abl = atoi(e);
#ifdef AVD_STAMP
    static unsigned long long* d_stamp = nullptr;
    if (!d_stamp) (void)hipMalloc(&d_stamp, 128 * 8);
    dw.stamp = d_stamp;
#endif
    DxArgs dx;
    dx.n_agents = n_agents, dx.n_sets = n_sets, dx.sm = sm, dx.g3 = g3, dx.xfh = xfs, dx.stamp = nullptr, dx.L_cWa = dx.L_cba = 0, dx.unsigned_mask = 0;
    dx.abl = dw.abl;
#ifdef AVD_STAMP
    dx.stamp = d_stamp;
#endif
    FinArgs fa;
    fa.L = L, fa.n_sets = n_sets, fa.J = pl.J, fa.S = S, fa.nrh = 1, fa.theta = theta, fa.stats = stats, fa.grads = grads, fa.losses = losses;
    fa.inv_n = inv_n, fa.partLa = F(pl.partHs[2]), fa.bad = bad;
    for (int i = 0; i < 2; ++i)
        fa.partH[i] = nullptr, fa.partHs[i] = F(pl.partHs[i]), fa.partU[i] = nullptr, fa.partV[i] = F(pl.partV[i]),
        fa.partG[i] = F(pl.partG[i]), fa.c3[i] = F(pl.vec[i]);
    fa.t1_from_g[0] = fa.t1_from_g[1] = 1, fa.t1p = F(pl.t1p), fa.s2raw = F(pl.s2raw);
    if (phases & PH_CRITIC) {
        if (hipMemsetAsync(ws + pl.bad, 0, sizeof(int) + sizeof(unsigned) * 4 * (size_t)n_sets * 2, st) != hipSuccess)
            return check_launch("avd_learn_set_split: memset");
        hipLaunchKernelGGL(scale_kernel, dim3(4, n_sets, SCALE_SLICES), dim3(256), 0, st, pa);
        hipLaunchKernelGGL(prep_kernel, dim3(H2, 4, n_sets), dim3(320), 0, st, pa);
        hipLaunchKernelGGL(prep1_kernel, dim3(NGT_MAX, 4, n_sets), dim3(64), 0, st, pa);
        PackArgs pk;
        pk.x[0] = s, pk.extra[0] = a, pk.outh[0] = xfs, pk.x[1] = s2, pk.extra[1] = r, pk.outh[1] = xfs2, pk.rows = nrows, pk.bad = bad;
        hipLaunchKernelGGL(pack_x_kernel<S>, dim3((unsigned)((2 * nrows + 255) / 256), 2), dim3(256), 0, st, pk);
        head(head_kernel<S, ActorS, OUT_TANH>, 2, xfs2, nullptr, nullptr, nullptr, a2, nullptr);
        head(head_kernel<S, CriticS, OUT_TD>, 3, xfs2, a2, r, nullptr, y, nullptr);
        h.sm = sma;
        head(head_kernel<S, ActorS, OUT_TANH_SAVE>, 0, xfs, nullptr, nullptr, nullptr, mu, nullptr);
        h.sm = sm;
        h.act2 = mu, h.part_s2 = F(pl.partHs[2]), h.part_m = F(pl.partM[1]);
        head(head_kernel<S, CriticS, HEAD_BOTH>, 1, xfs, a, nullptr, y, nullptr, F(pl.partHs[1]));
        dw.net = net[1], dw.act = a, dw.partG = F(pl.partG[1]), dw.part_m = F(pl.partM[1]);
        hipLaunchKernelGGL((dw_kernel<S, CriticS>), grid, block, 0, st, dw);
        dx.net = net[1], dx.partV = F(pl.partV[1]), dx.act = a, dx.part_m = F(pl.partM[1]);
        hipLaunchKernelGGL((dx_kernel<S, CriticS>), grid, block, 0, st, dx);
        dx.L_cWa = L.cWa, dx.L_cba = L.cba;
        hipLaunchKernelGGL((dxa_kernel<S>), grid, block, 0, st, dx);
        if (phases == PH_CRITIC) launch_finalize(fa, st, 1, 1);
    }
    if (phases & PH_ACTOR) {
        SeedArgs sd;
        sd.n_agents = n_agents, sd.n_sets = n_sets, sd.dmu = dmu, sd.tz = F(pl.tz), sd.high = high, sd.g3 = g3, sd.part_m = F(pl.partM[0]),
        sd.part_s = F(pl.partHs[0]);
        hipLaunchKernelGGL(actor_seed_kernel, grid, block, 0, st, sd);
        dw.sm = sma, dx.sm = sma;
        dw.net = net[0], dw.act = nullptr, dw.partG = F(pl.partG[0]), dw.part_m = F(pl.partM[0]);
        hipLaunchKernelGGL((dw_kernel<S, ActorS>), grid, block, 0, st, dw);
        dx.net = net[0], dx.partV = F(pl.partV[0]), dx.act = nullptr, dx.part_m = F(pl.partM[0]), dx.L_cWa = dx.L_cba = 0, dx.unsigned_mask = 1;
        hipLaunchKernelGGL((dx_kernel<S, ActorS>), grid, block, 0, st, dx);
        if (phases == PH_ACTOR) launch_finalize(fa, st, 0, 1);
        else launch_finalize(fa, st, 0, 2);
    }
    return check_launch("avd_learn_set_split");
}

}
}

using namespace avd;

namespace avd { namespace fsplit {
constexpr long MFMA_PER_TILE = 2 * (200 + 238 + 200 + 314)
                               + 8 * (2 + 32 + 1 + 2 * 2 * 2)
                               + 8 * (2 + 32 + 1 + 2 * 1 * 2)
                               + 2 * 8 * (32 + 2 + 8)
                               + 4 * 16;
static_assert(MFMA_PER_TILE == 3296, "update DESIGN.md 3.4 and the count above together");
}}
extern "C" int avd_learn_set_split_mfma_count(const avd_mlp_layout* lay, int n_agents, int n_sets, unsigned long long* mfma_32x32x16) {
    int rc = fsplit::check_shape(lay, n_agents, n_sets, "avd_learn_set_split_mfma_count");
    if (rc) return rc;
    AVD_REQUIRE(mfma_32x32x16, "avd_learn_set_split_mfma_count: null pointer");
    *mfma_32x32x16 = (unsigned long long)fsplit::MFMA_PER_TILE * (unsigned long long)n_agents;
    return AVD_OK;
}

extern "C" int avd_learn_set_split_workspace(const avd_mlp_layout* lay, int n_agents, int n_sets, size_t* bytes) {
    int rc = fsplit::check_shape(lay, n_agents, n_sets, "avd_learn_set_split_workspace");
    if (rc) return rc;
    AVD_REQUIRE(bytes, "avd_learn_set_split_workspace: null pointer");
    *bytes = fsplit::make_plan(n_agents, n_sets).total;
    return AVD_OK;
}

static int split_entry(int phases, const char* who, const avd_mlp_layout* lay, int n_agents, int n_sets, const float* theta, const float* stats,
                       const float* theta_t, const float* stats_t, const float* s, const float* a, const float* r, const float* s2,
                       const float* agent_weight, float gamma, float high, float* grads, float* losses, void* workspace,
                       size_t workspace_bytes, void* stream) {
    int rc = fsplit::check_shape(lay, n_agents, n_sets, who);
    if (rc) return rc;
    const bool cr = phases & fsplit::PH_CRITIC;
    AVD_REQUIRE(theta && stats && s && grads && workspace && (!cr || (theta_t && stats_t && a && r && s2)), "%s: null pointer", who);
    const fsplit::Plan pl = fsplit::make_plan(n_agents, n_sets);
    AVD_REQUIRE(workspace_bytes >= pl.total, "%s: workspace %zu B < %zu B", who, workspace_bytes, pl.total);
    if (cr && hipMemsetAsync(grads, 0, sizeof(float) * (size_t)n_sets * lay->theta_size, (hipStream_t)stream) != hipSuccess)
        return check_launch("avd_learn_set_split: hipMemsetAsync(grads)");
    if (lay->S == 4)
        return fsplit::run<4>(phases, *lay, n_agents, n_sets, theta, stats, theta_t, stats_t, s, a, r, s2, agent_weight, gamma, high, grads,
                              losses, (unsigned char*)workspace, pl, (hipStream_t)stream);
    return fsplit::run<3>(phases, *lay, n_agents, n_sets, theta, stats, theta_t, stats_t, s, a, r, s2, agent_weight, gamma, high, grads, losses,
                          (unsigned char*)workspace, pl, (hipStream_t)stream);
}

extern "C" int avd_learn_set_split_f16x3(const avd_mlp_layout* lay, int n_agents, int n_sets, const float* theta, const float* stats,
                                          const float* theta_t, const float* stats_t, const float* s, const float* a, const float* r,
                                          const float* s2, const float* agent_weight, float gamma, float high, float* grads,
                                          float* losses, void* workspace, size_t workspace_bytes, void* stream) {
    return split_entry(fsplit::PH_BOTH, "avd_learn_set_split_f16x3", lay, n_agents, n_sets, theta, stats, theta_t, stats_t, s, a, r, s2,
                       agent_weight, gamma, high, grads, losses, workspace, workspace_bytes, stream);
}

extern "C" int avd_learn_set_split_bf16x3(const avd_mlp_layout* lay, int n_agents, int n_sets, const float* theta, const float* stats,
                                          const float* theta_t, const float* stats_t, const float* s, const float* a, const float* r,
                                          const float* s2, const float* agent_weight, float gamma, float high, float* grads,
                                          float* losses, void* workspace, size_t workspace_bytes, void* stream) {
    return avd_learn_set_split_f16x3(lay, n_agents, n_sets, theta, stats, theta_t, stats_t, s, a, r, s2, agent_weight, gamma, high, grads,
                                     losses, workspace, workspace_bytes, stream);
}

extern "C" int avd_learn_set_split_critic(const avd_mlp_layout* lay, int n_agents, int n_sets, const float* theta, const float* stats,
                                          const float* theta_t, const float* stats_t, const float* s, const float* a, const float* r,
                                          const float* s2, const float* agent_weight, float gamma, float high, float* grads,
                                          float* losses, void* workspace, size_t workspace_bytes, void* stream) {
    return split_entry(fsplit::PH_CRITIC, "avd_learn_set_split_critic", lay, n_agents, n_sets, theta, stats, theta_t, stats_t, s, a, r, s2,
                       agent_weight, gamma, high, grads, losses, workspace, workspace_bytes, stream);
}

extern "C" int avd_learn_set_split_actor(const avd_mlp_layout* lay, int n_agents, int n_sets, const float* theta, const float* stats,
                                         const float* s, float high, float* grads, void* workspace, size_t workspace_bytes, void* stream) {
    return split_entry(fsplit::PH_ACTOR, "avd_learn_set_split_actor", lay, n_agents, n_sets, theta, stats, nullptr, nullptr, s, nullptr, nullptr,
                       nullptr, nullptr, 0.f, high, grads, nullptr, workspace, workspace_bytes, stream);
}
```

avddpg_amd/csrc/replay.hip:

```cpp
#include "common.h"

namespace avd {

__global__ void replay_add_kernel(int n_agents, int cap, int S, int A, float* __restrict__ ring, int slot,
                                  const float* __restrict__ s_prev, const float* __restrict__ s_next, int x_stride,
                                  const float* __restrict__ action, const float* __restrict__ reward) {
    const int row = 2 * S + A + 1;
    const long t = (long)blockIdx.x * blockDim.x + threadIdx.x;
    if (t >= (long)n_agents * row) return;
    const int a = (int)(t / row);
    const int j = (int)(t - (long)a * row);
    float val;
    if (j < S)
        val = s_prev[(long)a * x_stride + j];
    else if (j < S + A)
        val = action[(long)a * A + (j - S)];
    else if (j == S + A)
        val = reward[a];
    else
        val = s_next[(long)a * x_stride + (j - S - A - 1)];
    ring[((long)a * cap + slot) * row + j] = val;
}

__global__ void replay_indices_kernel(int n_agents, int B, uint32_t range, uint64_t seed, uint64_t counter,
                                      int32_t* __restrict__ idx) {
    const long t = (long)blockIdx.x * blockDim.x + threadIdx.x;
    const long total = (long)n_agents * B;
    const long base = t * 4;
    if (base >= total) return;
    const u32x4 r = philox_at(seed, counter, (uint32_t)t, STREAM_REPLAY);
    const uint32_t w[4] = {r.x, r.y, r.z, r.w};
#pragma unroll
    for (int k = 0; k < 4; ++k)
        if (base + k < total) idx[base + k] = (int32_t)(((uint64_t)w[k] * range) >> 32);
}

__global__ void replay_gather_kernel(int n_agents, int cap, int S, int A, int B, const float* __restrict__ ring,
                                     const int32_t* __restrict__ idx, float* __restrict__ s, float* __restrict__ a,
                                     float* __restrict__ r, float* __restrict__ s2) {
    const int row = 2 * S + A + 1;
    const long t = (long)blockIdx.x * blockDim.x + threadIdx.x;
    const long total = (long)n_agents * B * row;
    if (t >= total) return;
    const long ab = t / row;
    const int j = (int)(t - ab * row);
    const int ag = (int)(ab / B);
    const int ix = idx[ab];
    const float val = ring[((long)ag * cap + ix) * row + j];
    if (j < S)
        s[ab * S + j] = val;
    else if (j < S + A)
        a[ab * A + (j - S)] = val;
    else if (j == S + A)
        r[ab] = val;
    else
        s2[ab * S + (j - S - A - 1)] = val;
}

template <int S>
__global__ __launch_bounds__(256) void replay_sample_kernel(int n_agents, int cap, int B, const float* __restrict__ ring,
                                                            uint32_t range, uint64_t seed, uint64_t counter,
                                                            int32_t* __restrict__ idx, float* __restrict__ s,
                                                            float* __restrict__ a, float* __restrict__ r,
                                                            float* __restrict__ s2) {
    constexpr int row = 2 * S + 2;
    const long t = (long)blockIdx.x * blockDim.x + threadIdx.x;
    const long total = (long)n_agents * B, base = t * 4;
    if (base >= total) return;
    const u32x4 rr = philox_at(seed, counter, (uint32_t)t, STREAM_REPLAY);
    const uint32_t w[4] = {rr.x, rr.y, rr.z, rr.w};
    const int ag = (int)(base / B);
    int ix[4];
    float v[4][row];
#pragma unroll
    for (int k = 0; k < 4; ++k) {
        ix[k] = (int32_t)(((uint64_t)w[k] * range) >> 32);
        const float2* src = (const float2*)(ring + ((long)ag * cap + ix[k]) * row);
#pragma unroll
        for (int j = 0; j < row / 2; ++j) {
            const float2 q = src[j];
            v[k][2 * j] = q.x, v[k][2 * j + 1] = q.y;
        }
    }
    *(int4*)(idx + base) = make_int4(ix[0], ix[1], ix[2], ix[3]);
    *(float4*)(a + base) = make_float4(v[0][S], v[1][S], v[2][S], v[3][S]);
    *(float4*)(r + base) = make_float4(v[0][S + 1], v[1][S + 1], v[2][S + 1], v[3][S + 1]);
#pragma unroll
    for (int k = 0; k < 4; ++k) {
        if (S == 4) {
            *(float4*)(s + (base + k) * 4) = make_float4(v[k][0], v[k][1], v[k][2], v[k][3]);
            *(float4*)(s2 + (base + k) * 4) = make_float4(v[k][6], v[k][7], v[k][8], v[k][9]);
        } else {
#pragma unroll
            for (int j = 0; j < S; ++j) s[(base + k) * S + j] = v[k][j], s2[(base + k) * S + j] = v[k][S + 2 + j];
        }
    }
}

}

using namespace avd;

extern "C" int avd_replay_sample_f32(int n_agents, int cap, int S, int A, int B, const float* ring, int range, uint64_t seed,
                                     uint64_t counter, int32_t* idx, float* s, float* a, float* r, float* s2, void* stream) {
    AVD_REQUIRE(n_agents > 0 && cap > 0 && (S == 3 || S == 4) && A == 1 && B > 0 && B % 4 == 0 && range > 0 && range <= cap,
                "avd_replay_sample_f32: n=%d cap=%d S=%d A=%d B=%d range=%d (S in {3, 4}, A = 1, B a multiple of 4)", n_agents, cap, S,
                A, B, range);
    AVD_REQUIRE(ring && idx && s && a && r && s2, "avd_replay_sample_f32: null pointer");
    const long calls = (long)n_agents * B / 4;
    const dim3 grid((unsigned)((calls + 255) / 256));
    if (S == 4)
        hipLaunchKernelGGL(replay_sample_kernel<4>, grid, dim3(256), 0, (hipStream_t)stream, n_agents, cap, B, ring, (uint32_t)range,
                           seed, counter, idx, s, a, r, s2);
    else
        hipLaunchKernelGGL(replay_sample_kernel<3>, grid, dim3(256), 0, (hipStream_t)stream, n_agents, cap, B, ring, (uint32_t)range,
                           seed, counter, idx, s, a, r, s2);
    return check_launch("avd_replay_sample_f32");
}

extern "C" int avd_replay_add_f32(int n_agents, int cap, int S, int A, float* ring, int64_t counter,
                                  const float* s_prev, const float* s_next, int x_stride, const float* action,
                                  const float* reward, void* stream) {
    AVD_REQUIRE(n_agents > 0 && cap > 0 && S > 0 && A > 0 && counter >= 0 && x_stride >= S,
                "avd_replay_add_f32: n=%d cap=%d S=%d A=%d counter=%ld x_stride=%d", n_agents, cap, S, A, (long)counter,
                x_stride);
    AVD_REQUIRE(ring && s_prev && s_next && action && reward, "avd_replay_add_f32: null pointer");
    const int slot = (int)(counter % cap);
    const long total = (long)n_agents * (2 * S + A + 1);
    hipLaunchKernelGGL(replay_add_kernel, dim3((unsigned)((total + 255) / 256)), dim3(256), 0, (hipStream_t)stream,
                       n_agents, cap, S, A, ring, slot, s_prev, s_next, x_stride, action, reward);
    return check_launch("avd_replay_add_f32");
}

extern "C" int avd_replay_indices(int n_agents, int B, int range, uint64_t seed, uint64_t counter, int32_t* idx,
                                  void* stream) {
    AVD_REQUIRE(n_agents > 0 && B > 0 && range > 0 && idx, "avd_replay_indices: n=%d B=%d range=%d", n_agents, B,
                range);
    const long calls = ((long)n_agents * B + 3) / 4;
    hipLaunchKernelGGL(replay_indices_kernel, dim3((unsigned)((calls + 255) / 256)), dim3(256), 0,
                       (hipStream_t)stream, n_agents, B, (uint32_t)range, seed, counter, idx);
    return check_launch("avd_replay_indices");
}

extern "C" int avd_replay_gather_f32(int n_agents, int cap, int S, int A, int B, const float* ring,
                                     const int32_t* idx, float* s, float* a, float* r, float* s2, void* stream) {
    AVD_REQUIRE(n_agents > 0 && cap > 0 && S > 0 && A > 0 && B > 0, "avd_replay_gather_f32: bad sizes");
    AVD_REQUIRE(ring && idx && s && a && r && s2, "avd_replay_gather_f32: null pointer");
    const long total = (long)n_agents * B * (2 * S + A + 1);
    hipLaunchKernelGGL(replay_gather_kernel, dim3((unsigned)((total + 255) / 256)), dim3(256), 0,
                       (hipStream_t)stream, n_agents, cap, S, A, B, ring, idx, s, a, r, s2);
    return check_launch("avd_replay_gather_f32");
}
```

avddpg_amd/trainer.py:

```python
import logging

import numpy as np
import torch

from . import vec
from ._hip import call, ptr, stream_handle

log = logging.getLogger(__name__)


def is_fed_enabled(conf):
    return (conf.fed_method == conf.interfrl or conf.fed_method == conf.intrafrl) and (conf.framework == conf.dcntrl)


def is_gradient_updates_enabled(conf):
    return conf.aggregation_method == conf.gradients


def is_model_weight_updates_enabled(conf):
    return conf.aggregation_method == conf.weights


def is_weighted_fed_enabled(conf, training_episode):
    return conf.weighted_average_enabled and training_episode >= conf.weighted_window


def is_valid_update_episode(conf, training_episode):
    return conf.fed_enabled and (training_episode % conf.fed_update_count) == 0 and \
        training_episode <= conf.fed_cutoff_episode


def is_valid_update_step(conf, training_step):
    return (training_step % conf.fed_update_delay_steps) == 0


def is_valid_step_for_federated_training_with_gradients(conf, training_episode, training_step):
    return is_fed_enabled(conf) and is_valid_update_episode(conf, training_episode) and \
        is_valid_update_step(conf, training_step) and is_gradient_updates_enabled(conf)


def is_valid_step_for_federated_training_with_weights(conf, training_episode, training_step):
    return is_fed_enabled(conf) and is_valid_update_episode(conf, training_episode) and \
        is_valid_update_step(conf, training_step) and is_model_weight_updates_enabled(conf)


class VecTrainer:
    def __init__(self, conf, device=None, rng="device", group=None, shared_sets=None, seed=None, auto_reset=False,
                 pipeline_chunks=1, fused_update=False, shared_engine=None, init_seed=None, fused_step=None,
                 replay_ring=None, overlap_allreduce=None):
        conf.refresh()
        self.conf, self.rng, self.group = conf, rng, group
        self.device = torch.device(device if device is not None else "cuda")
        self.P, self.L = conf.num_platoons, conf.pl_size
        seed = conf.random_seed if seed is None else seed
        self.env = vec.VecPlatoon(self.P, self.L, conf, self.device, rand_states=conf.rand_states, rng=rng, seed=seed)
        self.centralized = conf.framework == conf.cntrl
        self.M = self.env.num_models
        self.S, self.A = self.env.num_states, self.env.num_actions
        if self.centralized and conf.model == conf.modelA and self.L > 1:
            raise ValueError("centralized + Model A with pl_size > 1: the reference's observation is 4L wide but its "
                             "network input 3L (src/environment.py:45-63, 518); not a runnable configuration")
        self.x_stride = 4 * self.L // self.M
        n_agents = self.P * self.M
        self.n_agents = n_agents
        self.ou = vec.VecOUNoise(n_agents, conf, self.device, rng=rng, seed=seed)
        fed = is_fed_enabled(conf)
        can_share = (fed and conf.fed_method == conf.interfrl and is_gradient_updates_enabled(conf)
                     and conf.fed_update_delay_steps == 1 and conf.fed_update_count == 1
                     and conf.fed_cutoff_ratio >= 1.0)
        self.shared = can_share if shared_sets is None else bool(shared_sets)
        if self.shared and not can_share:
            raise ValueError("shared weight sets are only exact for interfrl+gradients with every step federated")
        self.set_mod = self.M if self.shared else 0
        self.agents = vec.AgentGroup(self.M if self.shared else n_agents, self.S, self.A, conf, self.device,
                                     seed=conf.random_seed if init_seed is None else init_seed,
                                     hidd_mult=self.env.hidden_multiplier)
        from . import dist as _dist
        _dist.broadcast_agents(self.agents, group)
        self.total_platoons = _dist.total_platoons(self.P, group, self.device)
        self.replay = vec.VecReplay(n_agents, conf.buffer_size, conf.batch_size, self.S, self.A, self.device, rng=rng,
                                    seed=seed, ring=replay_ring)
        f32 = dict(dtype=torch.float32, device=self.device)
        lay = self.agents.lay
        fits = lay.H2 <= 256
        self.shared_engine = shared_engine or ("batched" if (self.shared and not fits) else "per_agent")
        if self.shared_engine not in ("per_agent", "batched", "fused", "fused3"):
            raise ValueError(f"shared_engine={shared_engine!r}")
        if self.shared_engine in ("batched", "fused", "fused3") and not self.shared:
            raise ValueError("the batched learners need shared weight sets (interfrl + gradients, every step federated)")
        if self.shared_engine in ("fused", "fused3") and (lay.H1, lay.H2, lay.Ha, lay.A, lay.B) != (256, 128, 48, 1, 64):
            raise ValueError("shared_engine='fused' / 'fused3' (csrc/fset.hip, fsplit.hip) serve the reference widths 256/128/48, A = 1, batch 64 only; "
                             f"got {lay.H1}/{lay.H2}/{lay.Ha}, A = {lay.A}, batch {lay.B}: use shared_engine='batched'")
        self.actor_out = torch.zeros(n_agents, self.A, **f32)
        self.actions = torch.zeros(self.P, self.M, self.A, **f32)
        self.leader_exog = torch.zeros(self.P, **f32)
        batched = self.shared and self.shared_engine in ("batched", "fused", "fused3")
        self.grads = None if batched else torch.zeros(n_agents, self.agents.lay.theta_size, **f32)
        self.losses = torch.zeros(n_agents, 2, **f32)
        self.ep_reward = torch.zeros(self.P, self.M, **f32)
        self.all_ep_reward_lists = [[[] for _ in range(self.M)] for _ in range(self.P)]
        self.all_avg_reward_lists = [[[] for _ in range(self.M)] for _ in range(self.P)]
        self.fed_weights = None
        self.exog_calls = 0
        self.seed = seed
        if auto_reset not in (False, True, "platoon"):
            raise ValueError(f"auto_reset={auto_reset!r}: False, True (any-terminal, all platoons) or 'platoon'")
        self.auto_reset = auto_reset
        if auto_reset and rng != "device":
            raise ValueError("auto_reset needs rng='device'")
        self._dev_weighted = bool(auto_reset and fed and conf.weighted_average_enabled)
        if self._dev_weighted:
            W = int(conf.weighted_window)
            self._hist_ring = torch.zeros(n_agents, W, **f32)
            self._hist_cnt = torch.zeros(self.P, dtype=torch.int32, device=self.device)
            self._w_raw, self._aw = torch.ones(n_agents, **f32), torch.ones(n_agents, **f32)
            self._wsum = torch.full((self.M,), float(self.P), **f32)
        self.steps_total = 0
        can_fuse_step = rng == "device" and not self.centralized and self.A == 1 and self.S in (3, 4)
        self.fused_step = can_fuse_step if fused_step is None else bool(fused_step)
        if self.fused_step and not can_fuse_step:
            raise ValueError("fused_step needs rng='device' and the decentralized framework")
        self.act_mfma = (self.shared and self.shared_engine in ("fused", "fused3")
                         and (lay.H1, lay.H2, lay.A) == (256, 128, 1) and lay.S in (3, 4))
        can_overlap = group is not None and self.shared and self.shared_engine == "fused3"
        self.overlap_allreduce = False if overlap_allreduce is None else bool(overlap_allreduce)
        if self.overlap_allreduce and not can_overlap:
            raise ValueError("overlap_allreduce needs a process group and shared_engine='fused3' (the two-phase learn call)")
        self._side = None
        self._xbuf = None
        self._flag_exchanged = False
        ws = 1
        if group is not None:
            import torch.distributed as _td
            ws = _td.get_world_size(group)
        self._equal_shards = abs(self.total_platoons - self.P * ws) < 0.5
        self._step_parity = 0
        self._added = False
        self.fused_update = bool(fused_update)
        self._act_ready = False
        self.pipeline_chunks = int(pipeline_chunks)
        self.intra_fused = True
        self.timers = None
        self.episode, self.ep_step = 0, 0
        self.updates = 0
        self.env_steps = 0

    def _timed(self, name, fn, *args, **kw):
        if self.timers is None:
            return fn(*args, **kw)
        e0, e1 = torch.cuda.Event(enable_timing=True), torch.cuda.Event(enable_timing=True)
        e0.record()
        out = fn(*args, **kw)
        e1.record()
        self.timers.setdefault(name, []).append((e0, e1))
        return out

    def reset_episode(self):
        self._act_ready = False
        self.env.reset()
        self.ep_reward.zero_()
        self.ep_step = 0

    def _act(self):
        conf, P, M = self.conf, self.P, self.M
        states = self.env.x.view(P * M, self.x_stride)
        if self.shared and self.shared_engine == "batched" and self.agents.lay.H2 > 256:
            sm = self.env.x.view(P, M, 4)[..., :self.S].transpose(0, 1).contiguous()
            o = self.agents.actor_shared(sm, P * M)
            self.actor_out.copy_(o.transpose(0, 1).reshape(P * M, 1))
        elif self._act_ready:
            self.agents.actor(states, self.set_mod, x_stride=self.x_stride, out=self.actor_out,
                              run_if_nonzero=self.env.any_done)
        elif self.act_mfma:
            self.agents.actor_set(states, P * M, x_stride=self.x_stride, out=self.actor_out.view(-1))
        else:
            self.agents.actor(states, self.set_mod, x_stride=self.x_stride, out=self.actor_out)
        if self.fused_step:
            self._step_fused()
            return
        if self.rng == "host":
            normals = np.empty((P, M))
            exog = np.empty(P)
            for p in range(P):
                for m in range(M):
                    normals[p, m] = np.random.normal(0, 1.0)
                exog[p] = (np.random.uniform(-conf.reset_max_u, conf.reset_max_u) if conf.rand_gen == conf.uniform
                           else np.random.normal(0, conf.reset_max_u))
            noise = self.ou(normals.reshape(-1))
            self.leader_exog.copy_(torch.from_numpy(exog.astype(np.float32)))
        else:
            noise = self.ou()
            call("avd_uniform_f32" if conf.rand_gen == conf.uniform else "avd_normal_f32", P, ptr(self.leader_exog),
                 conf.reset_max_u, self.seed, self.exog_calls, stream_handle())
            self.exog_calls += 1
        if self.A > 1:
            noise = noise.view(-1, 1).expand(-1, self.A).contiguous()
        call("avd_policy_f32", self.n_agents * self.A, ptr(self.actor_out), ptr(noise), conf.action_low,
             conf.action_high, ptr(self.actions), stream_handle())
        self.env.any_done.zero_()
        self.env.step(self.actions.view(P, self.L), self.leader_exog)

    def _step_fused(self):
        conf, env, ou, rp = self.conf, self.env, self.ou, self.replay
        k = self._step_parity
        self._step_parity ^= 1
        env.any_done = env._any_flags[k:k + 1]
        other = env._any_flags[1 - k:2 - k]
        env.x, env.x_prev = env.x_prev, env.x
        call("avd_step_fused_f32", ptr(env.d_consts), self.P, self.L, self.S, ptr(env.x_prev), ptr(env.x), ptr(env.prev_a),
             ptr(env.cum_accel), ptr(env.reward), ptr(env.term), ptr(env.done), ptr(env.any_done), ptr(other),
             ptr(self.actor_out), ptr(ou.state), ptr(self.actions), ptr(self.leader_exog), conf.theta, ou.mean, conf.ou_dt,
             conf.std_dev, conf.action_low, conf.action_high, conf.reset_max_u, 1 if conf.rand_gen == conf.uniform else 0,
             self.seed, ou.calls, self.exog_calls, ptr(rp.ring), rp.cap, rp.buffer_counter, ptr(self.ep_reward), stream_handle())
        ou.calls += 1
        self.exog_calls += 1
        env.step_count += 1
        rp.buffer_counter += 1
        self._added = True

    def _weights_for_fed(self, ep):
        w = np.empty((self.P, self.M), dtype=np.float32)
        for p in range(self.P):
            for m in range(self.M):
                hist = self.all_ep_reward_lists[p][m][-self.conf.weighted_window:]
                if not hist:
                    raise RuntimeError(f"weighted federated averaging at episode {ep} needs the episodic rewards of agent "
                                       f"({p}, {m}), but none were recorded (update_reward_list is called by run())")
                w[p, m] = abs(1 / np.mean(hist))
        if not np.all(np.isfinite(w)):
            raise FloatingPointError(f"non-finite federated weights at episode {ep} (an episodic-reward mean of 0?)")
        return torch.from_numpy(w).to(self.device)

    def _train(self, ep, i):
        conf, P, M = self.conf, self.P, self.M
        env = self.env

        def replay_part():
            reward = env.reward_mean.view(P, 1) if self.centralized else env.reward
            xs = self.x_stride
            if self._added:
                self._added = False
            else:
                self.replay.add(env.x_prev.view(P * M, xs), self.actions.view(P * M, self.A), reward.view(-1),
                                env.x.view(P * M, xs), xs)
                self.ep_reward += reward
            if not self.replay.buffer_counter > conf.batch_size:
                return None
            return self.replay.sample()

        batch = self._timed("replay", replay_part)
        if batch is None:
            return
        s, a, r, s2 = batch
        fed = is_fed_enabled(conf)
        self.updates += self.n_agents
        if not fed and self.fused_update:
            nxt = self.A == 1 and self.auto_reset
            self._timed("learn+update", self.agents.learn_update, s, a, r, s2, self.grads, self.losses,
                        next_states=env.x.view(P * M, self.x_stride) if nxt else None, x_stride=self.x_stride,
                        next_actions=self.actor_out.view(-1) if nxt else None)
            self._act_ready = nxt
            return
        if not fed and self.pipeline_chunks > 1:
            self.agents.learn_apply(s, a, r, s2, self.grads, self.losses, chunks=self.pipeline_chunks,
                                    timers=self.timers)
            return
        if (fed and conf.fed_method == conf.intrafrl and not self.shared and self.pipeline_chunks > 1
                and is_valid_update_step(conf, i) and is_valid_step_for_federated_training_with_gradients(conf, ep, i)):
            w = self._intra_weights(ep)
            e0, e1 = torch.cuda.Event(enable_timing=True), torch.cuda.Event(enable_timing=True)
            if self.timers is not None:
                e0.record()
            self.agents.learn_apply_intra(s, a, r, s2, self.grads, P, M, losses=self.losses, chunks=self.pipeline_chunks, weights=w,
                                          lead_skip=bool(conf.intra_directional_averaging), timers=self.timers)
            if self.timers is not None:
                e1.record()
                self.timers.setdefault("learn+update", []).append((e0, e1))
            return
        if self.shared and self.shared_engine in ("batched", "fused", "fused3"):
            weights = None
            if self._dev_weighted:
                weights = "device"
            elif is_weighted_fed_enabled(conf, ep):
                if self.fed_weights is None or self.fed_weights[0] != ep:
                    self.fed_weights = (ep, self._weights_for_fed(ep))
                weights = self.fed_weights[1]
            self._timed("learn", self._learn_batched, s, a, r, s2, weights)
            self._timed("update", self.agents.apply, self.set_grads, guarded=self.shared_engine in ("fused", "fused3"))
            return
        self._timed("learn", self.agents.learn, s, a, r, s2, self.set_mod, grads=self.grads, losses=self.losses)
        self._timed("update", self._update, ep, i, fed)

    def _learn_batched(self, s, a, r, s2, weights=None):
        P, M, B = self.P, self.M, self.conf.batch_size
        sm = lambda x: x.view(P, M, *x.shape[1:]).transpose(0, 1).reshape(M, P * B, *x.shape[2:]).contiguous()
        if getattr(self, "set_grads", None) is None:
            from .dist import set_exchange_buffer
            self._xbuf, self.set_grads = set_exchange_buffer(M, self.agents.lay.theta_size, self.device)
            self.set_losses = torch.zeros(M, 2, dtype=torch.float32, device=self.device)
        carry = self.env.any_done if (self.group is not None and self.auto_reset is True) else None
        rw = wsum = aw_dev = None
        if isinstance(weights, str):
            aw_dev, wsum, weights = self._aw, self._wsum, None
        elif weights is not None:
            wsum = weights.sum(dim=0)
        if self.shared_engine in ("fused", "fused3"):
            aw = aw_dev if aw_dev is not None else (None if weights is None else (weights * (float(P) / wsum)).reshape(P * M).contiguous())
            if self.overlap_allreduce:
                self._learn_split_overlapped(s, a, r, s2, aw, wsum, carry)
                self._flag_exchanged = carry is not None
                return
            self.agents.learn_set_fused(s, a, r, s2, P * M, grads=self.set_grads, losses=self.set_losses, agent_weight=aw,
                                        split=self.shared_engine == "fused3")
        else:
            if aw_dev is not None:
                rw = aw_dev.view(P, M).transpose(0, 1).reshape(M, P, 1).expand(M, P, B).reshape(M, P * B).contiguous()
            elif weights is not None:
                rw = (weights * (float(P) / wsum)).transpose(0, 1).reshape(M, P, 1).expand(M, P, B).reshape(M, P * B).contiguous()
            self.agents.learn_shared(sm(s), sm(a), sm(r), sm(s2), P * M, grads=self.set_grads, losses=self.set_losses,
                                     row_weight=rw)
        if self.group is not None:
            from .dist import exchange_set_slab
            self._timed("allreduce", exchange_set_slab, self._xbuf, M, self.agents.lay.theta_size, wsum, P, self.total_platoons,
                        self.group, flag=carry, equal_shards=self._equal_shards)
            self._flag_exchanged = carry is not None

    def _learn_split_overlapped(self, s, a, r, s2, aw, wsum, flag=None):
        from .dist import exchange_two_phase

        P, M = self.P, self.M
        lay = self.agents.lay
        A, T = lay.actor_size, lay.theta_size
        if self._side is None:
            f32 = dict(dtype=torch.float32, device=self.device)
            self._side = dict(stream=torch.cuda.Stream(device=self.device), ready=torch.cuda.Event(),
                              crit=torch.empty(M, T - A, **f32), act=torch.empty(M * A + M + 1, **f32))
        scale = float(P) if wsum is None else wsum.view(M, 1)
        learn = lambda phase: self.agents.learn_set_fused(s, a, r, s2, P * M, grads=self.set_grads, losses=self.set_losses,
                                                          agent_weight=aw, split=True, phase=phase)
        learn("critic")
        exchange_two_phase(self.set_grads, A, scale, wsum, self.total_platoons, self.group, self._side,
                           lambda: learn("actor"), timers=self.timers, flag=flag)

    def _update(self, ep, i, fed):
        conf, P, M = self.conf, self.P, self.M
        if not fed or not is_valid_update_step(conf, i):
            if self.shared:
                raise RuntimeError("local update requested in shared-set mode")
            self.agents.apply(self.grads)
            return
        weights = None
        if self._dev_weighted:
            weights = self._w_raw.view(P, M)
        elif is_weighted_fed_enabled(conf, ep):
            if self.fed_weights is None or self.fed_weights[0] != ep:
                self.fed_weights = (ep, self._weights_for_fed(ep))
            weights = self.fed_weights[1]
        method = conf.fed_method
        if is_valid_step_for_federated_training_with_gradients(conf, ep, i):
            if method == conf.intrafrl and self.intra_fused and not self.shared:
                self.agents.apply_intra(self.grads, P, M, weights=weights, lead_skip=bool(conf.intra_directional_averaging))
                return
            avg = vec.fed_mean(self.grads, P, M, weights=weights, group=self.group, method=method,
                               total=self.total_platoons)
            if self.shared:
                self.agents.apply(avg)
            elif method == conf.intrafrl and self.intra_fused:
                pass
            else:
                directional = method == conf.intrafrl and conf.intra_directional_averaging
                vec.fed_scatter(avg, self.grads, P, M, method)
                if directional:
                    ag = self.agents
                    lead = lambda x: x.view(P, M, -1)[:, 0]
                    keep = [lead(x).clone() for x in (ag.theta, ag.theta_t, ag.stats_t, ag.m, ag.v)]
                    keep_step = ag.step.view(P, M)[:, 0].clone()
                    ag.apply(self.grads)
                    for x, k in zip((ag.theta, ag.theta_t, ag.stats_t, ag.m, ag.v), keep):
                        lead(x).copy_(k)
                    ag.step.view(P, M)[:, 0].copy_(keep_step)
                else:
                    self.agents.apply(self.grads)
        elif is_valid_step_for_federated_training_with_weights(conf, ep, i):
            if self.shared:
                raise RuntimeError("weights aggregation needs per-agent weight sets")
            ag = self.agents
            tp = self.total_platoons
            avg_th = vec.fed_mean(ag.theta, P, M, weights=weights, group=self.group, method=method, total=tp)[0]
            avg_st = vec.fed_mean(ag.stats, P, M, weights=weights, group=self.group, method=method, total=tp)[0]
            directional = method == conf.intrafrl and conf.intra_directional_averaging
            for dst, src in ((ag.theta, avg_th), (ag.theta_t, avg_th), (ag.stats, avg_st), (ag.stats_t, avg_st)):
                view = dst.view(P, M, -1)
                (view[:, 1:] if directional else view).copy_(src.expand_as(view[:, 1:] if directional else view))

    def step(self, ep=None, i=None, sync=True):
        ep = self.episode if ep is None else ep
        i = self.ep_step if i is None else i
        self._flag_exchanged = False
        self._timed("act+env", self._act)
        self._train(ep, i)
        self.env_steps += self.P
        self.ep_step += 1
        if self.group is not None and self.auto_reset is True and not self._flag_exchanged:
            import torch.distributed as _td
            _td.all_reduce(self.env.any_done, op=_td.ReduceOp.MAX, group=self.group)
        self.steps_total += 1
        limit = self.conf.steps_per_episode
        if self.auto_reset == "platoon":
            if self._dev_weighted:
                self.env.ensure_episode_state()
                self._push_history(done=self.env.done, ep_len=self.env.ep_len, limit=limit, zero_after=0)
            self.env.episode_end(self.ep_reward, self.M, limit, any_reset=self.env.any_done)
            self.episode = self.steps_total // limit
            if self._dev_weighted:
                self._refresh_weights(1 if self.steps_total >= int(self.conf.weighted_window) * limit else 0)
            return None
        if self.auto_reset:
            if self.ep_step >= limit:
                if self._dev_weighted:
                    self._push_history(force=1, zero_after=1)
                self.env.reset()
                self._act_ready = False
                self.ep_step = 0
                self.episode += 1
            else:
                if self._dev_weighted:
                    self._push_history(cond=self.env.any_done, zero_after=1)
                self.env.reset(cond=self.env.any_done)
            if self._dev_weighted:
                self._refresh_weights(-1)
            return None
        if not sync:
            return None
        from .dist import any_terminal
        return any_terminal(self.env.any_done, self.group)

    def _intra_weights(self, ep):
        if self._dev_weighted:
            return self._w_raw.view(self.P, self.M)
        if is_weighted_fed_enabled(self.conf, ep):
            if self.fed_weights is None or self.fed_weights[0] != ep:
                self.fed_weights = (ep, self._weights_for_fed(ep))
            return self.fed_weights[1]
        return None

    def _push_history(self, done=None, ep_len=None, limit=0, cond=None, force=0, zero_after=0):
        call("avd_fed_history_push_f32", self.P, self.M, int(self.conf.weighted_window), ptr(self.ep_reward), ptr(done), ptr(ep_len),
             int(limit), ptr(cond), int(force), int(zero_after), ptr(self._hist_ring), ptr(self._hist_cnt), stream_handle())

    def _refresh_weights(self, host_enabled):
        call("avd_fed_weights_f32", self.P, self.M, int(self.conf.weighted_window), ptr(self._hist_ring), ptr(self._hist_cnt),
             int(host_enabled), ptr(self._w_raw), ptr(self._aw), ptr(self._wsum), stream_handle())

    def nonfinite_updates(self):
        n = getattr(self.agents, "nonfinite_skipped", None)
        return 0 if n is None else int(n.item())

    def update_reward_list(self, ep):
        rew = self.ep_reward.cpu().numpy()
        for p in range(self.P):
            for m in range(self.M):
                self.all_ep_reward_lists[p][m].append(rew[p, m])
                self.all_avg_reward_lists[p][m].append(
                    np.mean(self.all_ep_reward_lists[p][m][-self.conf.reward_averaging_window:]))

    def run(self, number_of_episodes=None):
        conf = self.conf
        n = conf.number_of_episodes if number_of_episodes is None else number_of_episodes
        for ep in range(n):
            self.episode = ep
            self.reset_episode()
            for i in range(conf.steps_per_episode):
                if self.step(ep, i):
                    break
            self.update_reward_list(ep)
        return self.all_ep_reward_lists, self.all_avg_reward_lists

    def evaluator_scores(self, platoons=None):
        from . import evaluator

        platoons = list(range(self.P)) if platoons is None else list(platoons)
        if self.shared:
            sc = evaluator.run_many(self.conf, self.agents, [0], set_mod=self.M)[0]
            return np.repeat(sc[:, 0], len(platoons))
        return evaluator.run_many(self.conf, self.agents, platoons)[0][:, 0]

    def run_simulations(self):
        return [float(r / self.conf.re_scalar) for r in self.evaluator_scores()]


class Trainer:

    def __init__(self, base_dir, timestamp, debug_enabled, conf, rng="host", device=None):
        self.base_dir, self.timestamp, self.debug_enabled, self.conf = base_dir, timestamp, debug_enabled, conf
        self.rng, self.device = rng, device
        self.engine = None

    def initialize(self):
        self.conf.timestamp = str(self.timestamp)
        self.conf.fed_enabled = is_fed_enabled(self.conf)
        self.engine = VecTrainer(self.conf, device=self.device, rng=self.rng)
        self.num_models, self.num_platoons = self.engine.M, self.engine.P
        self.num_states, self.num_actions = self.engine.S, self.engine.A
        self.all_ep_reward_lists = self.engine.all_ep_reward_lists
        self.all_avg_reward_lists = self.engine.all_avg_reward_lists

    def run(self, number_of_episodes=None):
        return self.engine.run(number_of_episodes)


def learn(rbuffer, actor_model, critic_model, target_actor, target_critic, gamma=0.99):
    from . import _hip, params

    lay = actor_model.lay
    s, a, r, s2 = rbuffer.sample()
    A = lay.actor_size
    theta = torch.cat([actor_model.theta[:, :A], critic_model.theta[:, A:]], dim=1).contiguous()
    theta_t = torch.cat([target_actor.theta[:, :A], target_critic.theta[:, A:]], dim=1).contiguous()

    def stats_of(act, cri):
        st = act.stats.clone()
        st[:, lay.cmms:] = cri.stats[:, lay.cmms:]
        return st

    stats, stats_t = stats_of(actor_model, critic_model), stats_of(target_actor, target_critic)
    grads = torch.empty(1, lay.theta_size, dtype=torch.float32, device=theta.device)
    call("avd_learn_f32", _hip.C.byref(lay), 1, 1, ptr(theta), ptr(stats), ptr(theta_t), ptr(stats_t),
         ptr(s.reshape(1, lay.B, lay.S).contiguous()), ptr(a.reshape(1, lay.B, lay.A).contiguous()),
         ptr(r.reshape(1, lay.B).contiguous()), ptr(s2.reshape(1, lay.B, lay.S).contiguous()), gamma,
         actor_model.high, ptr(grads), None, stream_handle())
    g = grads[0].cpu().numpy()
    dummy = np.zeros(lay.stats_size, dtype=np.float32)
    dims = getattr(actor_model, "dims", None)
    return (params.unpack(lay, g, dummy, "critic", trainable_only=True, dims=dims),
            params.unpack(lay, g, dummy, "actor", trainable_only=True, dims=dims))


Trainer.learn = staticmethod(learn)
```

avddpg_amd/vec.py:

```python
import ctypes as C

import numpy as np
import torch

from . import _hip, dynamics, params
from ._hip import call, ptr, stream_handle


def _dev(device):
    return torch.device(device if device is not None else "cuda")


class VecPlatoon:

    def __init__(self, num_platoons, length, config, device=None, rand_states=True, evaluator_states_enabled=False,
                 rng="host", seed=1, track_aux=False):
        self.P, self.L, self.config = int(num_platoons), int(length), config
        self.length = self.L
        self.device = _dev(device)
        self.rng, self.seed = rng, int(seed)
        self.rand_states, self.evaluator_states_enabled = rand_states, evaluator_states_enabled
        centralized = config.framework == config.cntrl
        self.multiplier = self.L if centralized else 1
        self.hidden_multiplier = config.centrl_hidd_mult if centralized else 1
        self.num_models = 1 if centralized else self.L
        self.def_num_actions = 1
        self.num_actions = self.def_num_actions * self.multiplier
        self.def_num_states = 3 if config.model == config.modelA else 4
        self.num_states = self.def_num_states * self.multiplier
        self.number_of_reward_components = 4
        self.state_lbs = {0: "$e_{pi,k}$", 1: "$e_{vi,k}$", 2: "$a_{i,k}$", 3: "$a_{i-1,k}$"}
        self.jerk_lb, self.exog_lbl = "jerk", "$u_{i,k}$"
        self.obs_width = min(4, self.num_states)

        self.h_consts = dynamics.env_consts(config, self.L)
        raw = np.frombuffer(bytes(self.h_consts), dtype=np.uint8).copy()
        self.d_consts = torch.from_numpy(raw).to(self.device)
        f32 = dict(dtype=torch.float32, device=self.device)
        P, L = self.P, self.L
        self.x = torch.zeros(P, L, 4, **f32)
        self.x_prev = torch.zeros(P, L, 4, **f32)
        self.prev_a = torch.zeros(P, L, **f32)
        self.cum_accel = torch.zeros(P, L, **f32) if track_aux else None
        self.reward = torch.zeros(P, L, **f32)
        self.reward_mean = torch.zeros(P, **f32) if centralized else None
        self.term = torch.zeros(P, L, dtype=torch.uint8, device=self.device)
        self.done = torch.zeros(P, dtype=torch.uint8, device=self.device)
        self._any_flags = torch.zeros(2, dtype=torch.int32, device=self.device)
        self.any_done = self._any_flags[0:1]
        self.reset_count = 0
        self.step_count = 0
        self.ep_len = self.ep_stats = None
        if rng == "host":
            self._host_ctor_draws()

    def _rand(self, val):
        c = self.config
        if c.rand_gen == c.uniform:
            return np.random.uniform(-1 * val, val)
        return np.random.normal(0, val)

    def _mode(self):
        if self.evaluator_states_enabled:
            return 1 if self.rand_states else 2
        return 0 if self.rand_states else 2

    def _host_ctor_draws(self):
        c, P, L = self.config, self.P, self.L
        self.front_accel = np.zeros(P)
        self.front_u = np.zeros(P)
        draws = np.zeros((P, L, 3), dtype=np.float64)
        for p in range(P):
            self.front_accel[p] = self._rand(c.pl_leader_reset_a)
            self.front_u[p] = self._rand(c.reset_max_u)
            if self._mode() == 0:
                for i in range(L):
                    draws[p, i, 0] = self._rand(c.reset_ep_max)
                    draws[p, i, 1] = self._rand(c.reset_max_ev)
                    draws[p, i, 2] = self._rand(c.reset_max_a)
        self._upload_reset(draws, self.front_accel)

    def _upload_reset(self, draws, fa, cond=None):
        d = torch.from_numpy(draws.astype(np.float32)).to(self.device) if draws is not None else None
        f = torch.from_numpy(np.asarray(fa, dtype=np.float32)).to(self.device) if fa is not None else None
        call("avd_env_reset_f32", ptr(self.d_consts), self.P, self.L, ptr(self.x), ptr(self.prev_a),
             ptr(self.cum_accel), ptr(d), ptr(f), self._mode(), self.seed, self.reset_count, ptr(cond),
             stream_handle())

    def _host_reset_draws(self):
        c, P, L = self.config, self.P, self.L
        draws = np.zeros((P, L, 3), dtype=np.float64)
        fa = np.zeros(P, dtype=np.float64)
        train = self._mode() == 0
        for p in range(P):
            fa[p] = self._rand(c.pl_leader_reset_a)
            for i in range(L):
                self.front_u[p] = self._rand(c.reset_max_u)
                if train:
                    draws[p, i, 0] = self._rand(c.reset_ep_max)
                    draws[p, i, 1] = self._rand(c.reset_max_ev)
                    draws[p, i, 2] = self._rand(c.reset_max_a)
        self.front_accel = fa.copy()
        return draws, fa

    def observations(self, x=None):
        x = self.x if x is None else x
        return x[..., : self.obs_width]

    def reset(self, cond=None):
        draws = fa = None
        if self.rng == "host":
            if cond is not None:
                raise ValueError("conditional reset needs rng='device'")
            draws, fa = self._host_reset_draws()
        self._upload_reset(draws, fa, cond)
        self.reset_count += 1
        return self.observations()

    def episode_end(self, ep_reward, M, limit, any_reset=None):
        if self.rng != "device":
            raise ValueError("per-platoon episode ends need rng='device'")
        self.ensure_episode_state()
        st = self.ep_stats
        call("avd_episode_end_f32", ptr(self.d_consts), self.P, self.L, M, ptr(self.x), ptr(self.prev_a), ptr(self.cum_accel),
             ptr(self.done), ptr(self.ep_len), ptr(ep_reward), int(limit), ptr(st["ret_sum"]), ptr(st["len_sum"]),
             ptr(st["count"]), ptr(any_reset), self._mode(), self.seed, self.reset_count, stream_handle())
        self.reset_count += 1

    def ensure_episode_state(self):
        if self.ep_len is None:
            z = lambda dt: torch.zeros(self.P, dtype=dt, device=self.device)
            self.ep_len = z(torch.int32)
            self.ep_stats = dict(ret_sum=z(torch.float32), len_sum=z(torch.float32), count=z(torch.int32))

    def pop_episode_stats(self):
        st = self.ep_stats
        n = int(st["count"].sum())
        ret, ln = float(st["ret_sum"].double().sum()), float(st["len_sum"].double().sum())
        for t in st.values():
            t.zero_()
        return (ret / n if n else float("nan")), (ln / n if n else float("nan")), n

    def step(self, actions, leader_exog):
        self.x, self.x_prev = self.x_prev, self.x
        call("avd_env_step_f32", ptr(self.d_consts), self.P, self.L, ptr(self.x_prev), ptr(self.x), ptr(self.prev_a),
             ptr(self.cum_accel), ptr(actions), ptr(leader_exog), ptr(self.reward), ptr(self.term), ptr(self.done),
             ptr(self.reward_mean), ptr(self.any_done), stream_handle())
        self.step_count += 1
        return self.observations(), self.reward, self.done

    def get_jerk_from(self, x_before, prev_a_before):
        return (x_before[..., 2] - prev_a_before) / self.config.sample_rate


class VecOUNoise:

    def __init__(self, n, config, device=None, rng="host", seed=1, mean=0.0):
        self.n, self.config, self.device = int(n), config, _dev(device)
        self.rng, self.seed, self.calls = rng, int(seed), 0
        self.mean = float(mean)
        self.state = torch.zeros(self.n, dtype=torch.float32, device=self.device)

    def reset(self):
        self.state.zero_()

    def __call__(self, normals=None):
        c = self.config
        d_n = None
        if self.rng == "host":
            if normals is None:
                normals = np.random.normal(0, 1.0, size=self.n)
            d_n = torch.from_numpy(np.asarray(normals, dtype=np.float32).reshape(self.n)).to(self.device)
        call("avd_ou_step_f32", self.n, ptr(self.state), ptr(d_n), c.theta, self.mean, c.ou_dt, c.std_dev, self.seed,
             self.calls, stream_handle())
        self.calls += 1
        return self.state


class VecReplay:

    def __init__(self, n_agents, buffer_capacity, batch_size, num_states, num_actions, device=None, rng="host",
                 seed=1, ring=None):
        self.n, self.cap, self.B = int(n_agents), int(buffer_capacity), int(batch_size)
        self.S, self.A = int(num_states), int(num_actions)
        self.row = 2 * self.S + self.A + 1
        self.device, self.rng, self.seed = _dev(device), rng, int(seed)
        if ring is not None:
            if tuple(ring.shape) != (self.n, self.cap, self.row) or ring.dtype != torch.float32 or not ring.is_contiguous():
                raise _hip.AvdError(f"replay ring must be contiguous float32 {(self.n, self.cap, self.row)}, got {tuple(ring.shape)}")
            self.ring = ring
        else:
            self.ring = torch.zeros(self.n, self.cap, self.row, dtype=torch.float32, device=self.device)
        self.buffer_counter = 0
        self.samples = 0
        f32 = dict(dtype=torch.float32, device=self.device)
        self.idx = torch.zeros(self.n, self.B, dtype=torch.int32, device=self.device)
        self.s = torch.zeros(self.n, self.B, self.S, **f32)
        self.a = torch.zeros(self.n, self.B, self.A, **f32)
        self.r = torch.zeros(self.n, self.B, **f32)
        self.s2 = torch.zeros(self.n, self.B, self.S, **f32)

    def add(self, s_prev, action, reward, s_next, x_stride):
        call("avd_replay_add_f32", self.n, self.cap, self.S, self.A, ptr(self.ring), self.buffer_counter, ptr(s_prev),
             ptr(s_next), x_stride, ptr(action), ptr(reward), stream_handle())
        self.buffer_counter += 1

    def sample_range(self):
        return min(self.buffer_counter, self.cap)

    def draw_indices(self, host_idx=None):
        if self.rng == "host":
            if host_idx is None:
                rr = self.sample_range()
                host_idx = np.stack([np.random.choice(rr, self.B) for _ in range(self.n)])
            self.idx.copy_(torch.from_numpy(np.asarray(host_idx).astype(np.int32)))
        else:
            call("avd_replay_indices", self.n, self.B, self.sample_range(), self.seed, self.samples, ptr(self.idx),
                 stream_handle())
        self.samples += 1
        return self.idx

    def gather(self):
        call("avd_replay_gather_f32", self.n, self.cap, self.S, self.A, self.B, ptr(self.ring), ptr(self.idx),
             ptr(self.s), ptr(self.a), ptr(self.r), ptr(self.s2), stream_handle())
        return self.s, self.a, self.r, self.s2

    def sample(self, host_idx=None):
        if self.rng != "host" and host_idx is None and self.A == 1 and self.S in (3, 4) and self.B % 4 == 0:
            call("avd_replay_sample_f32", self.n, self.cap, self.S, self.A, self.B, ptr(self.ring), self.sample_range(), self.seed,
                 self.samples, ptr(self.idx), ptr(self.s), ptr(self.a), ptr(self.r), ptr(self.s2), stream_handle())
            self.samples += 1
            return self.s, self.a, self.r, self.s2
        self.draw_indices(host_idx)
        return self.gather()


class AgentGroup:

    def __init__(self, n_sets, num_states, num_actions, config, device=None, hidd_mult=1, seed=None, high_bound=None):
        c = config
        self.config, self.device, self.n_sets = c, _dev(device), int(n_sets)
        if (c.critic_layer1_size, c.critic_layer2_size) != (c.actor_layer1_size, c.actor_layer2_size):
            raise _hip.AvdError("actor and critic layer1/layer2 sizes must match (reference defaults do)")
        self.dims = params.Dims(num_states, num_actions, int(c.actor_layer1_size * hidd_mult),
                                int(c.actor_layer2_size * hidd_mult), int(c.critic_act_layer_size * hidd_mult))
        H1p, H2p, Hap = params.padded_widths(self.dims.H1, self.dims.H2, self.dims.Ha)
        self.lay = _hip.make_layout(num_states, num_actions, H1p, H2p, Hap, c.batch_size)
        self.high = float(c.action_high if high_bound is None else high_bound)
        f32 = dict(dtype=torch.float32, device=self.device)
        n, T, S = self.n_sets, self.lay.theta_size, self.lay.stats_size
        self.theta = torch.zeros(n, T, **f32)
        self.stats = torch.zeros(n, S, **f32)
        self.theta_t = torch.zeros(n, T, **f32)
        self.stats_t = torch.zeros(n, S, **f32)
        self.m = torch.zeros(n, T, **f32)
        self.v = torch.zeros(n, T, **f32)
        self.step = torch.zeros(n, dtype=torch.int32, device=self.device)
        self._layp = C.byref(self.lay)
        rs = np.random.RandomState(c.random_seed if seed is None else seed)
        th, st = params.init_weights(self.lay, rs, nominal=(c.actor_layer1_size, c.actor_layer2_size), dims=self.dims)
        self.theta.copy_(torch.from_numpy(th).to(self.device).expand(n, T))
        self.stats.copy_(torch.from_numpy(st).to(self.device).expand(n, S))
        self.theta_t.copy_(self.theta)
        self.stats_t.copy_(self.stats)

    def actor(self, states, set_mod, x_stride=None, out=None, target=False, run_if_nonzero=None):
        n_agents = states.shape[0]
        x_stride = states.shape[-1] if x_stride is None else x_stride
        shape = (n_agents,) if self.lay.A == 1 else (n_agents, self.lay.A)
        out = torch.empty(*shape, dtype=torch.float32, device=self.device) if out is None else out
        th, st = (self.theta_t, self.stats_t) if target else (self.theta, self.stats)
        if run_if_nonzero is not None:
            call("avd_actor_forward_cond_f32", self._layp, n_agents, set_mod, ptr(th), ptr(st), ptr(states), x_stride,
                 self.high, ptr(out), ptr(run_if_nonzero), stream_handle())
        else:
            call("avd_actor_forward_f32", self._layp, n_agents, set_mod, ptr(th), ptr(st), ptr(states), x_stride,
                 self.high, ptr(out), stream_handle())
        return out

    def actor_set(self, states, n_agents, x_stride=None, out=None, run_if_nonzero=None):
        x_stride = states.shape[-1] if x_stride is None else x_stride
        out = torch.empty(n_agents, dtype=torch.float32, device=self.device) if out is None else out
        call("avd_actor_forward_set_f32", self._layp, n_agents, self.n_sets, ptr(self.theta), ptr(self.stats), ptr(states), x_stride,
             self.high, ptr(out), ptr(run_if_nonzero), stream_handle())
        return out

    def critic(self, states, actions, set_mod, x_stride=None, out=None, target=False):
        n_agents = states.shape[0]
        x_stride = states.shape[-1] if x_stride is None else x_stride
        shape = (n_agents,) if self.lay.A == 1 else (n_agents, self.lay.A)
        out = torch.empty(*shape, dtype=torch.float32, device=self.device) if out is None else out
        th, st = (self.theta_t, self.stats_t) if target else (self.theta, self.stats)
        call("avd_critic_forward_f32", self._layp, n_agents, set_mod, ptr(th), ptr(st), ptr(states), x_stride,
             ptr(actions), ptr(out), stream_handle())
        return out

    def learn(self, s, a, r, s2, set_mod, grads=None, losses=None):
        n_agents = s.shape[0]
        if grads is None:
            grads = torch.empty(n_agents, self.lay.theta_size, dtype=torch.float32, device=self.device)
        call("avd_learn_f32", self._layp, n_agents, set_mod, ptr(self.theta), ptr(self.stats), ptr(self.theta_t),
             ptr(self.stats_t), ptr(s), ptr(a), ptr(r), ptr(s2), self.config.gamma, self.high, ptr(grads),
             ptr(losses), stream_handle())
        return grads

    def learn_shared(self, s, a, r, s2, n_agents, grads=None, losses=None, row_weight=None):
        import ctypes
        if grads is None:
            grads = torch.empty(self.n_sets, self.lay.theta_size, dtype=torch.float32, device=self.device)
        need = ctypes.c_size_t(0)
        call("avd_learn_shared_workspace", self._layp, n_agents, self.n_sets, ctypes.byref(need))
        ws = getattr(self, "_wide_ws", None)
        if ws is None or ws.numel() < need.value:
            ws = self._wide_ws = torch.empty(need.value, dtype=torch.uint8, device=self.device)
        call("avd_learn_shared_bf16", self._layp, n_agents, self.n_sets, ptr(self.theta), ptr(self.stats),
             ptr(self.theta_t), ptr(self.stats_t), ptr(s), ptr(a), ptr(r), ptr(s2), ptr(row_weight), self.config.gamma,
             self.high, ptr(grads), ptr(losses), ptr(ws), ws.numel(), stream_handle())
        return grads

    def learn_set_fused(self, s, a, r, s2, n_agents, grads=None, losses=None, agent_weight=None, split=False, phase=None):
        import ctypes
        self._check_agent_major(s, a, r, s2, n_agents, agent_weight)
        if grads is None:
            grads = torch.empty(self.n_sets, self.lay.theta_size, dtype=torch.float32, device=self.device)
        wsf, fn, attr = (("avd_learn_set_split_workspace", "avd_learn_set_split_f16x3", "_fsplit_ws") if split else
                         ("avd_learn_set_fused_workspace", "avd_learn_set_fused_bf16", "_fset_ws"))
        need = ctypes.c_size_t(0)
        call(wsf, self._layp, n_agents, self.n_sets, ctypes.byref(need))
        ws = getattr(self, attr, None)
        if ws is None or ws.numel() < need.value:
            ws = torch.empty(need.value, dtype=torch.uint8, device=self.device)
            setattr(self, attr, ws)
        if phase is not None and not split:
            raise _hip.AvdError("phase= needs split=True (csrc/fsplit.hip)")
        if phase == "actor":
            call("avd_learn_set_split_actor", self._layp, n_agents, self.n_sets, ptr(self.theta), ptr(self.stats), ptr(s), self.high,
                 ptr(grads), ptr(ws), ws.numel(), stream_handle())
            return grads
        if phase not in (None, "critic"):
            raise _hip.AvdError(f"phase={phase!r}")
        call("avd_learn_set_split_critic" if phase == "critic" else fn, self._layp, n_agents, self.n_sets, ptr(self.theta), ptr(self.stats),
             ptr(self.theta_t), ptr(self.stats_t), ptr(s), ptr(a), ptr(r), ptr(s2), ptr(agent_weight), self.config.gamma, self.high,
             ptr(grads), ptr(losses), ptr(ws), ws.numel(), stream_handle())
        return grads

    def learn_set_split(self, s, a, r, s2, n_agents, grads=None, losses=None, agent_weight=None):
        return self.learn_set_fused(s, a, r, s2, n_agents, grads=grads, losses=losses, agent_weight=agent_weight, split=True)

    def _check_agent_major(self, s, a, r, s2, n_agents, agent_weight):
        lay = self.lay
        want = {"s": (n_agents, lay.B, lay.S), "s2": (n_agents, lay.B, lay.S), "r": (n_agents, lay.B)}
        for name, x in (("s", s), ("s2", s2), ("r", r)):
            if tuple(x.shape) != want[name] or x.dtype != torch.float32 or not x.is_contiguous():
                raise _hip.AvdError(f"set learner: {name} must be contiguous float32 {want[name]} (agent-major), got "
                                    f"{tuple(x.shape)} {x.dtype} contiguous={x.is_contiguous()}")
        if a.numel() != n_agents * lay.B * lay.A or a.dtype != torch.float32 or not a.is_contiguous() or a.shape[0] != n_agents:
            raise _hip.AvdError(f"set learner: a must be contiguous float32 [{n_agents}, {lay.B}(, {lay.A})], got {tuple(a.shape)} {a.dtype}")
        if n_agents <= 0 or n_agents % self.n_sets:
            raise _hip.AvdError(f"set learner: n_agents={n_agents} is not a multiple of n_sets={self.n_sets}")
        if agent_weight is not None and (agent_weight.numel() != n_agents or agent_weight.dtype != torch.float32
                                         or not agent_weight.is_contiguous()):
            raise _hip.AvdError(f"set learner: agent_weight must be contiguous float32 [{n_agents}]")

    def actor_shared(self, states_set_major, n_agents, out=None):
        import ctypes
        rows = n_agents // self.n_sets
        if out is None:
            out = torch.empty(self.n_sets, rows, dtype=torch.float32, device=self.device)
        need = ctypes.c_size_t(0)
        call("avd_actor_forward_shared_workspace", self._layp, n_agents, self.n_sets, ctypes.byref(need))
        ws = getattr(self, "_wide_act_ws", None)
        if ws is None or ws.numel() < need.value:
            ws = self._wide_act_ws = torch.empty(need.value, dtype=torch.uint8, device=self.device)
        call("avd_actor_forward_shared_bf16", self._layp, n_agents, self.n_sets, ptr(self.theta), ptr(self.stats),
             ptr(states_set_major), self.high, ptr(out), ptr(ws), ws.numel(), stream_handle())
        return out

    def apply(self, grads, guarded=False):
        c = self.config
        self.step += 1
        if guarded:
            if getattr(self, "nonfinite_skipped", None) is None:
                self.nonfinite_skipped = torch.zeros(1, dtype=torch.int32, device=self.device)
            call("avd_adam_polyak_guarded_f32", self._layp, self.n_sets, ptr(self.theta), ptr(self.stats), ptr(self.theta_t),
                 ptr(self.stats_t), ptr(self.m), ptr(self.v), ptr(grads), ptr(self.step), c.actor_lr, c.critic_lr,
                 float(c.tau), ptr(self.nonfinite_skipped), stream_handle())
            return
        call("avd_adam_polyak_f32", self._layp, self.n_sets, ptr(self.theta), ptr(self.stats), ptr(self.theta_t),
             ptr(self.stats_t), ptr(self.m), ptr(self.v), ptr(grads), ptr(self.step), c.actor_lr, c.critic_lr,
             float(c.tau), stream_handle())

    def apply_intra(self, grads, P, M, weights=None, lead_skip=False, lo=0, hi=None, stream=None, advance=True):
        c = self.config
        hi = P if hi is None else hi
        if self.n_sets != P * M:
            raise _hip.AvdError("apply_intra needs one weight set per agent (P * M sets)")
        if advance:
            if stream is None:
                self.step.view(P, M)[lo:hi, (1 if lead_skip else 0):] += 1
            else:
                with torch.cuda.stream(stream):
                    self.step.view(P, M)[lo:hi, (1 if lead_skip else 0):] += 1
        a, b = lo * M, hi * M
        call("avd_adam_polyak_intra_f32", self._layp, hi - lo, M, 1 if lead_skip else 0, ptr(self.theta[a:b]), ptr(self.stats[a:b]),
             ptr(self.theta_t[a:b]), ptr(self.stats_t[a:b]), ptr(self.m[a:b]), ptr(self.v[a:b]), ptr(grads[a:b]), ptr(self.step[a:b]),
             ptr(None if weights is None else weights.reshape(-1)[a:b]), c.actor_lr, c.critic_lr, float(c.tau),
             stream_handle() if stream is None else _hip.C.c_void_p(stream.cuda_stream))

    def learn_apply_intra(self, s, a, r, s2, grads, P, M, losses=None, chunks=8, weights=None, lead_skip=False, timers=None):
        main = torch.cuda.current_stream()
        if getattr(self, "_side", None) is None:
            self._side = torch.cuda.Stream(device=self.device)
        side = self._side
        c = self.config
        chunks = max(1, min(chunks, P))
        bounds = [(P * i) // chunks for i in range(chunks + 1)]
        T = lambda: torch.cuda.Event(enable_timing=timers is not None)
        self.step.view(P, M)[:, (1 if lead_skip else 0):] += 1
        for i in range(chunks):
            lo, hi = bounds[i] * M, bounds[i + 1] * M
            if hi == lo:
                continue
            t0, t1 = T(), T()
            if timers is not None:
                t0.record(main)
            call("avd_learn_f32", self._layp, hi - lo, 0, ptr(self.theta[lo:hi]), ptr(self.stats[lo:hi]), ptr(self.theta_t[lo:hi]),
                 ptr(self.stats_t[lo:hi]), ptr(s[lo:hi]), ptr(a[lo:hi]), ptr(r[lo:hi]), ptr(s2[lo:hi]), c.gamma, self.high,
                 ptr(grads[lo:hi]), ptr(losses[lo:hi]) if losses is not None else None, _hip.C.c_void_p(main.cuda_stream))
            t1.record(main)
            side.wait_event(t1)
            u0, u1 = T(), T()
            if timers is not None:
                u0.record(side)
            self.apply_intra(grads, P, M, weights=weights, lead_skip=lead_skip, lo=bounds[i], hi=bounds[i + 1], stream=side, advance=False)
            if timers is not None:
                u1.record(side)
                timers.setdefault("learn", []).append((t0, t1))
                timers.setdefault("update", []).append((u0, u1))
        done = torch.cuda.Event()
        done.record(side)
        main.wait_event(done)

    def learn_update(self, s, a, r, s2, grads, losses=None, next_states=None, x_stride=None, next_actions=None):
        n = self.n_sets
        if s.shape[0] != n:
            raise _hip.AvdError("learn_update needs one weight set per agent (set_mod == 0)")
        if getattr(self, "theta_alt", None) is None:
            self.theta_alt = self.theta.clone()
        c = self.config
        self.step += 1
        args = (self._layp, n, ptr(self.theta), ptr(self.stats), ptr(self.theta_alt), ptr(self.theta_t), ptr(self.stats_t),
                ptr(self.m), ptr(self.v), ptr(self.step), ptr(s), ptr(a), ptr(r), ptr(s2), c.gamma, self.high, c.actor_lr,
                c.critic_lr, float(c.tau), ptr(grads), ptr(losses))
        if next_actions is not None:
            if self.lay.A != 1:
                raise _hip.AvdError("next-action epilogue: A == 1 only")
            xs = next_states.shape[-1] if x_stride is None else x_stride
            call("avd_learn_update_act_f32", *args, ptr(next_states), xs, ptr(next_actions), stream_handle())
        else:
            call("avd_learn_update_f32", *args, stream_handle())
        self.theta, self.theta_alt = self.theta_alt, self.theta

    def learn_apply(self, s, a, r, s2, grads, losses=None, chunks=4, timers=None):
        n = self.n_sets
        if s.shape[0] != n:
            raise _hip.AvdError("learn_apply needs one weight set per agent (set_mod == 0)")
        main = torch.cuda.current_stream()
        if getattr(self, "_side", None) is None:
            self._side = torch.cuda.Stream(device=self.device)
        side = self._side
        c = self.config
        self.step += 1
        chunks = max(1, min(chunks, n))
        bounds = [(n * i) // chunks for i in range(chunks + 1)]
        T = lambda: torch.cuda.Event(enable_timing=timers is not None)
        for i in range(chunks):
            lo, hi = bounds[i], bounds[i + 1]
            if hi == lo:
                continue
            t0, t1 = T(), T()
            if timers is not None:
                t0.record(main)
            call("avd_learn_f32", self._layp, hi - lo, 0, ptr(self.theta[lo:hi]), ptr(self.stats[lo:hi]),
                 ptr(self.theta_t[lo:hi]), ptr(self.stats_t[lo:hi]), ptr(s[lo:hi]), ptr(a[lo:hi]), ptr(r[lo:hi]),
                 ptr(s2[lo:hi]), c.gamma, self.high, ptr(grads[lo:hi]), ptr(losses[lo:hi]) if losses is not None else None,
                 _hip.C.c_void_p(main.cuda_stream))
            t1.record(main)
            side.wait_event(t1)
            u0, u1 = T(), T()
            if timers is not None:
                u0.record(side)
            call("avd_adam_polyak_f32", self._layp, hi - lo, ptr(self.theta[lo:hi]), ptr(self.stats[lo:hi]),
                 ptr(self.theta_t[lo:hi]), ptr(self.stats_t[lo:hi]), ptr(self.m[lo:hi]), ptr(self.v[lo:hi]),
                 ptr(grads[lo:hi]), ptr(self.step[lo:hi]), c.actor_lr, c.critic_lr, float(c.tau),
                 _hip.C.c_void_p(side.cuda_stream))
            if timers is not None:
                u1.record(side)
                timers.setdefault("learn", []).append((t0, t1))
                timers.setdefault("update", []).append((u0, u1))
        done = torch.cuda.Event()
        done.record(side)
        main.wait_event(done)

    def get_weights(self, set_idx, which, target=False, trainable_only=False):
        th, st = (self.theta_t, self.stats_t) if target else (self.theta, self.stats)
        return params.unpack(self.lay, th[set_idx].cpu().numpy(), st[set_idx].cpu().numpy(), which, trainable_only,
                             dims=self.dims)

    def set_weights(self, set_idx, which, weights, target=False):
        th, st = (self.theta_t, self.stats_t) if target else (self.theta, self.stats)
        h_th, h_st = th[set_idx].cpu().numpy(), st[set_idx].cpu().numpy()
        params.pack(self.lay, weights, h_th, h_st, which, dims=self.dims)
        th[set_idx].copy_(torch.from_numpy(h_th))
        st[set_idx].copy_(torch.from_numpy(h_st))

    def grads_as_lists(self, grads_row):
        g = grads_row.cpu().numpy()
        dummy = np.zeros(self.lay.stats_size, dtype=np.float32)
        return (params.unpack(self.lay, g, dummy, "critic", trainable_only=True, dims=self.dims),
                params.unpack(self.lay, g, dummy, "actor", trainable_only=True, dims=self.dims))


def fed_mean(grads, P, M, weights=None, group=None, method="interfrl", total=None):
    n = grads.shape[-1]
    if method == "interfrl":
        n_out, n_in, so, si = M, P, 1, M
    elif method == "intrafrl":
        n_out, n_in, so, si = P, M, M, 1
    else:
        raise ValueError(method)
    out = torch.empty(n_out, n, dtype=torch.float32, device=grads.device)
    wsum = torch.empty(n_out, dtype=torch.float32, device=grads.device) if weights is not None else None
    call("avd_fed_sum_f32", n_out, n_in, so, si, n, ptr(grads), ptr(weights), ptr(out), ptr(wsum), stream_handle())
    count = float(n_in)
    if group is not None and method == "interfrl":
        from .dist import exchange_fed_sums
        count = exchange_fed_sums(out, wsum, n_in, group, total=total)
    call("avd_fed_finalize_f32", n_out, n, ptr(out), count, ptr(wsum), stream_handle())
    return out


def fed_scatter(avg, dst, P, M, method="interfrl", i_begin=0):
    n = avg.shape[-1]
    n_out, n_in, so, si = (M, P, 1, M) if method == "interfrl" else (P, M, M, 1)
    call("avd_fed_scatter_f32", n_out, n_in, so, si, i_begin, n, ptr(avg), ptr(dst), stream_handle())
    return dst
```

include/avddpg_hip.h:

```cpp
#ifndef AVDDPG_HIP_H
#define AVDDPG_HIP_H

#include <stddef.h>
#include <stdint.h>

#ifdef __cplusplus
extern "C" {
#pragma GCC visibility push(default)
#endif

#define AVD_MAX_L 16

#define AVD_OK 0
#define AVD_E_INVALID (-1)
#define AVD_E_LAUNCH (-2)
#define AVD_E_UNSUPPORTED (-3)

typedef struct avd_env_consts {
    int32_t L;
    int32_t model_a;
    int32_t can_terminate;
    int32_t uniform_reset;
    float max_ep, max_ev;
    float abs_action_high;
    float two_max_a;
    float T;
    float ca, cb, cc, cd;
    float re_scalar, terminal_reward;
    float stand_still, timegap;
    float reset_ep_max, reset_max_ev, reset_max_a;
    float reset_ep_eval, reset_ev_eval, reset_a_eval;
    float leader_reset_a;
    float A[AVD_MAX_L][16];
    float B[AVD_MAX_L][4];
    float C[AVD_MAX_L][4];
} avd_env_consts;

typedef struct avd_mlp_layout {
    int32_t S, A, H1, H2, Ha, B;
    int32_t aW1, ab1, ag1, abe1, aW2, ab2, ag2, abe2, aW3, ab3;
    int32_t actor_size;
    int32_t cWs, cbs, cgs, cbes, cWa, cba, cga, cbea, cW2, cb2, cg3, cbe3, cW3, cb3;
    int32_t theta_size;
    int32_t amm1, amv1, amm2, amv2, cmms, cmvs, cmma, cmva, cmm3, cmv3;
    int32_t stats_size;
} avd_mlp_layout;

const char* avd_last_error(void);
int avd_version(void);
int avd_diagnostics_enabled(void);

int avd_mlp_layout_init(avd_mlp_layout* out, int S, int A, int H1, int H2, int Ha, int B);

int avd_env_step_f32(const avd_env_consts* d_consts, int P, int L, const float* x_in, float* x_out, float* prev_a,
                     float* cum_accel, const float* u, const float* leader_exog, float* reward, uint8_t* term,
                     uint8_t* done, float* reward_mean, int32_t* any_done, void* stream);

int avd_env_reset_f32(const avd_env_consts* d_consts, int P, int L, float* x, float* prev_a, float* cum_accel,
                      const float* draws, const float* front_accel, int mode, uint64_t seed, uint64_t counter,
                      const int32_t* cond, void* stream);

int avd_episode_end_f32(const avd_env_consts* d_consts, int P, int L, int M, float* x, float* prev_a, float* cum_accel,
                        const uint8_t* done, int32_t* ep_len, float* ep_reward, int limit, float* ret_sum, float* len_sum,
                        int32_t* ep_cnt, int32_t* any_reset, int mode, uint64_t seed, uint64_t counter, void* stream);


int avd_ou_step_f32(int n, float* ou_state, const float* normals, float theta, float mean, float dt, float std_dev,
                    uint64_t seed, uint64_t counter, void* stream);

int avd_policy_f32(int n, const float* actor_out, const float* noise, float lo, float hi, float* action,
                   void* stream);

int avd_normal_f32(int n, float* out, float std_dev, uint64_t seed, uint64_t counter, void* stream);

int avd_uniform_f32(int n, float* out, float half_width, uint64_t seed, uint64_t counter, void* stream);

int avd_replay_add_f32(int n_agents, int cap, int S, int A, float* ring, int64_t counter, const float* s_prev,
                       const float* s_next, int x_stride, const float* action, const float* reward, void* stream);

int avd_replay_indices(int n_agents, int B, int range, uint64_t seed, uint64_t counter, int32_t* idx, void* stream);

int avd_replay_gather_f32(int n_agents, int cap, int S, int A, int B, const float* ring, const int32_t* idx, float* s,
                          float* a, float* r, float* s2, void* stream);


int avd_actor_forward_f32(const avd_mlp_layout* lay, int n_agents, int set_mod, const float* theta, const float* stats,
                          const float* state, int x_stride, float high, float* out, void* stream);

int avd_actor_forward_cond_f32(const avd_mlp_layout* lay, int n_agents, int set_mod, const float* theta,
                               const float* stats, const float* state, int x_stride, float high, float* out,
                               const int32_t* run_if_nonzero, void* stream);

int avd_critic_forward_f32(const avd_mlp_layout* lay, int n_agents, int set_mod, const float* theta,
                           const float* stats, const float* state, int x_stride, const float* action, float* q,
                           void* stream);

int avd_learn_f32(const avd_mlp_layout* lay, int n_agents, int set_mod, const float* theta, const float* stats,
                  const float* theta_t, const float* stats_t, const float* s, const float* a, const float* r,
                  const float* s2, float gamma, float high, float* grads, float* losses, void* stream);

int avd_adam_polyak_f32(const avd_mlp_layout* lay, int n_sets, float* theta, float* stats, float* theta_t,
                        float* stats_t, float* m, float* v, const float* grads, const int32_t* step, float actor_lr,
                        float critic_lr, double tau, void* stream);

int avd_adam_polyak_guarded_f32(const avd_mlp_layout* lay, int n_sets, float* theta, float* stats, float* theta_t, float* stats_t,
                                float* m, float* v, const float* grads, int32_t* step, float actor_lr, float critic_lr, double tau,
                                int32_t* skipped, void* stream);

int avd_learn_update_f32(const avd_mlp_layout* lay, int n_agents, const float* theta, const float* stats,
                         float* theta_out, float* theta_t, float* stats_t, float* m, float* v, const int32_t* step,
                         const float* s, const float* a, const float* r, const float* s2, float gamma, float high,
                         float actor_lr, float critic_lr, double tau, float* grads_scratch, float* losses,
                         void* stream);

int avd_learn_update_plan(const avd_mlp_layout* lay, int n_agents, int* chunk_agents, int* n_chunks, int* update_groups);

int avd_learn_update_act_f32(const avd_mlp_layout* lay, int n_agents, const float* theta, const float* stats,
                             float* theta_out, float* theta_t, float* stats_t, float* m, float* v, const int32_t* step,
                             const float* s, const float* a, const float* r, const float* s2, float gamma, float high,
                             float actor_lr, float critic_lr, double tau, float* grads_scratch, float* losses,
                             const float* next_state, int x_stride, float* next_action, void* stream);

int avd_polyak_f32(int64_t n, const float* w, float* t, double tau, void* stream);

int avd_fed_sum_f32(int n_out, int n_in, int stride_out, int stride_in, int n, const float* g, const float* weights,
                    float* out, float* wsum, void* stream);
int avd_fed_finalize_f32(int n_out, int n, float* out, float count, const float* wsum, void* stream);
int avd_fed_scatter_f32(int n_out, int n_in, int stride_out, int stride_in, int i_begin, int n, const float* src,
                        float* dst, void* stream);

int avd_adam_polyak_intra_f32(const avd_mlp_layout* lay, int P, int M, int lead_skip, float* theta, float* stats, float* theta_t,
                              float* stats_t, float* m, float* v, const float* grads, const int32_t* step, const float* weights,
                              float actor_lr, float critic_lr, double tau, void* stream);

int avd_fed_history_push_f32(int P, int M, int W, float* ep_reward, const uint8_t* done, const int32_t* ep_len, int limit,
                             const int32_t* cond, int force, int zero_after, float* ring, int32_t* hist_cnt, void* stream);
int avd_fed_weights_f32(int P, int M, int W, const float* ring, const int32_t* hist_cnt, int host_enabled, float* w_raw,
                        float* agent_weight, float* wsum, void* stream);

int avd_step_fused_f32(const avd_env_consts* d_consts, int P, int L, int S, const float* x_in, float* x_out, float* prev_a,
                       float* cum_accel, float* reward, uint8_t* term, uint8_t* done, int32_t* any_done, int32_t* any_done_other,
                       const float* actor_out, float* ou_state, float* action, float* leader_exog, float ou_theta, float ou_mean,
                       float ou_dt, float ou_std_dev, float action_low, float action_high, float exog_scale, int exog_uniform,
                       uint64_t seed, uint64_t ou_counter, uint64_t exog_counter, float* ring, int cap, int64_t replay_counter,
                       float* ep_reward, void* stream);

int avd_replay_sample_f32(int n_agents, int cap, int S, int A, int B, const float* ring, int range, uint64_t seed, uint64_t counter,
                          int32_t* idx, float* s, float* a, float* r, float* s2, void* stream);

int avd_actor_forward_set_f32(const avd_mlp_layout* lay, int n_agents, int n_sets, const float* theta, const float* stats,
                              const float* states, int x_stride, float high, float* out, const int32_t* run_if_nonzero, void* stream);

int avd_learn_shared_workspace(const avd_mlp_layout* lay, int n_agents, int n_sets, size_t* bytes);
int avd_learn_shared_bf16(const avd_mlp_layout* lay, int n_agents, int n_sets, const float* theta, const float* stats,
                          const float* theta_t, const float* stats_t, const float* s, const float* a, const float* r,
                          const float* s2, const float* row_weight, float gamma, float high, float* grads, float* losses,
                          void* workspace, size_t workspace_bytes, void* stream);

int avd_learn_set_fused_workspace(const avd_mlp_layout* lay, int n_agents, int n_sets, size_t* bytes);
int avd_learn_set_fused_bf16(const avd_mlp_layout* lay, int n_agents, int n_sets, const float* theta, const float* stats,
                             const float* theta_t, const float* stats_t, const float* s, const float* a, const float* r,
                             const float* s2, const float* agent_weight, float gamma, float high, float* grads, float* losses,
                             void* workspace, size_t workspace_bytes, void* stream);

int avd_learn_set_split_mfma_count(const avd_mlp_layout* lay, int n_agents, int n_sets, unsigned long long* mfma_32x32x16);
int avd_learn_set_split_critic(const avd_mlp_layout* lay, int n_agents, int n_sets, const float* theta, const float* stats,
                               const float* theta_t, const float* stats_t, const float* s, const float* a, const float* r,
                               const float* s2, const float* agent_weight, float gamma, float high, float* grads, float* losses,
                               void* workspace, size_t workspace_bytes, void* stream);
int avd_learn_set_split_actor(const avd_mlp_layout* lay, int n_agents, int n_sets, const float* theta, const float* stats,
                              const float* s, float high, float* grads, void* workspace, size_t workspace_bytes, void* stream);
int avd_learn_set_split_workspace(const avd_mlp_layout* lay, int n_agents, int n_sets, size_t* bytes);
int avd_learn_set_split_f16x3(const avd_mlp_layout* lay, int n_agents, int n_sets, const float* theta, const float* stats,
                               const float* theta_t, const float* stats_t, const float* s, const float* a, const float* r,
                               const float* s2, const float* agent_weight, float gamma, float high, float* grads, float* losses,
                               void* workspace, size_t workspace_bytes, void* stream);

int avd_learn_set_split_bf16x3(const avd_mlp_layout* lay, int n_agents, int n_sets, const float* theta, const float* stats,
                               const float* theta_t, const float* stats_t, const float* s, const float* a, const float* r,
                               const float* s2, const float* agent_weight, float gamma, float high, float* grads, float* losses,
                               void* workspace, size_t workspace_bytes, void* stream);

int avd_actor_forward_shared_workspace(const avd_mlp_layout* lay, int n_agents, int n_sets, size_t* bytes);
int avd_actor_forward_shared_bf16(const avd_mlp_layout* lay, int n_agents, int n_sets, const float* theta,
                                  const float* stats, const float* state, float high, float* out, void* workspace,
                                  size_t workspace_bytes, void* stream);

int avd_eval_rollout_f32(const avd_mlp_layout* lay, const avd_env_consts* d_consts, int R, int L, int M, int T, const float* theta,
                         const float* stats, int n_sets, const int32_t* set_base, const float* x0, const float* prev_a0,
                         const float* leader, int n_start, const int32_t* start_idx, float high, float lo, float hi,
                         float sample_rate, float* counters, int n_trace, const int32_t* trace_idx, float* tr_states,
                         float* tr_actions, float* tr_jerks, void* stream);

int avd_gemm_bt_bf16(int M, int Nc, int K, const void* A, long lda, const void* B, long ldb, float* D, long ldd,
                     void* stream);

#ifdef __cplusplus
#pragma GCC visibility pop
}
#endif
#endif
```

Before: 1.979 million.

## Fuse f16 hi/lo input packing into replay sampling for split learner

The replay sampler can now write the f16 hi/lo packed input fragments for s and s2 directly, together with a not-packable flag. The split f16x3 learner takes those buffers, so it no longer launches its own pack kernel or re-reads s2. The scale kernel now writes per-slice maxima instead of using atomics, which removes the workspace memset, and the grad memset is limited to the critic-only phase (the actor bias gradient padding is now zeroed explicitly). This saves kernel launches and a memory pass over the samples, at the cost of extra sampler work and added coupling between the sampler and the learner.

```diff
diff --git a/avddpg_amd/_hip.py b/avddpg_amd/_hip.py
--- a/avddpg_amd/_hip.py
+++ b/avddpg_amd/_hip.py
@@ -54,6 +54,7 @@
     "avd_step_fused_f32": [_P, _i, _i, _i, _P, _P, _P, _P, _P, _P, _P, _P, _P, _P, _P, _P, _P, _f, _f, _f, _f, _f, _f, _f, _i, _u64, _u64,
                            _u64, _P, _i, _i64, _P, _P],
     "avd_replay_sample_f32": [_i, _i, _i, _i, _i, _P, _i, _u64, _u64, _P, _P, _P, _P, _P, _P],
+    "avd_replay_sample_packed_f32": [_i, _i, _i, _i, _i, _P, _i, _u64, _u64, _P, _P, _P, _P, _P, _P, _P, _P, _P],
     "avd_actor_forward_set_f32": [_LP, _i, _i, _P, _P, _P, _i, _f, _P, _P, _P],
     "avd_replay_add_f32": [_i, _i, _i, _i, _P, _i64, _P, _P, _i, _P, _P, _P],
     "avd_replay_indices": [_i, _i, _i, _u64, _u64, _P, _P],
@@ -84,6 +85,7 @@
     "avd_learn_set_split_actor": [_LP, _i, _i, _P, _P, _P, _f, _P, _P, C.c_size_t, _P],
     "avd_learn_set_split_bf16x3": [_LP, _i, _i, _P, _P, _P, _P, _P, _P, _P, _P, _P, _f, _f, _P, _P, _P, C.c_size_t, _P],
     "avd_learn_set_split_f16x3": [_LP, _i, _i, _P, _P, _P, _P, _P, _P, _P, _P, _P, _f, _f, _P, _P, _P, C.c_size_t, _P],
+    "avd_learn_set_split_f16x3_packed": [_LP, _i, _i, _P, _P, _P, _P, _P, _P, _P, _P, _P, _P, _P, _f, _f, _P, _P, _P, C.c_size_t, _P],
     "avd_actor_forward_shared_workspace": [_LP, _i, _i, C.POINTER(C.c_size_t)],
     "avd_actor_forward_shared_bf16": [_LP, _i, _i, _P, _P, _P, _f, _P, _P, C.c_size_t, _P],
     "avd_eval_rollout_f32": [_LP, _P, _i, _i, _i, _i, _P, _P, _i, _P, _P, _P, _P, _i, _P, _f, _f, _f, _f, _P, _i, _P, _P, _P, _P,
diff --git a/avddpg_amd/csrc/fset.hip b/avddpg_amd/csrc/fset.hip
--- a/avddpg_amd/csrc/fset.hip
+++ b/avddpg_amd/csrc/fset.hip
@@ -738,7 +738,10 @@
             }
             g[obe2 + n] = w3 * D;
             g[ob2 + n] = S2;
-            if (n == 0) g[ob3] = D;
+            if (n == 0) {
+                g[ob3] = D;
+                for (int k = 1; k < 4; ++k) g[ob3 + k] = 0.f;
+            }
             if (critic && n == 0 && a.losses) a.losses[2 * set] = Lc * a.inv_n, a.losses[2 * set + 1] = -La * a.inv_n;
         }
         return;
diff --git a/avddpg_amd/csrc/fsplit.hip b/avddpg_amd/csrc/fsplit.hip
--- a/avddpg_amd/csrc/fsplit.hip
+++ b/avddpg_amd/csrc/fsplit.hip
@@ -1,6 +1,6 @@
 #include <type_traits>
 
-#include "fset_common.h"
+#include "fsplit_pack.h"
 
 namespace avd {
 namespace fsplit {
@@ -24,11 +24,8 @@
     }
 }
 
-typedef _Float16 f16;
 typedef _Float16 f16x2 __attribute__((ext_vector_type(2)));
-typedef _Float16 f16x8 __attribute__((ext_vector_type(8)));
 constexpr float S1 = 64.f;
-constexpr float F16_OVERFLOW = 65520.f;
 #if defined(FSPLIT_ABL_CONST)
 #define FSPLIT_ABL(x) FSPLIT_ABL_CONST
 #elif defined(AVD_DIAG)
@@ -49,10 +46,6 @@
 #endif
     lo = __builtin_bit_cast(unsigned, __builtin_convertvector(l, f16x2));
 }
-__device__ __forceinline__ void split1h(float x, f16& hi, f16& lo) {
-    hi = (f16)x;
-    lo = (f16)(x - (float)hi);
-}
 template <class V>
 __device__ __forceinline__ void pin16(V& x) {
 #pragma unroll
@@ -69,15 +62,6 @@
 }
 __device__ __forceinline__ f32x16 mfmah(f16x8 a, f16x8 b, f32x16 c) {
     return __builtin_amdgcn_mfma_f32_32x32x16_f16(a, b, c, 0, 0, 0);
-}
-__device__ __forceinline__ f16x8 make_xh(float x0, float x1, float x2, float x3, int h) {
-    f16 a0, a1, a2, a3, l0, l1, l2, l3;
-    split1h(x0, a0, l0), split1h(x1, a1, l1), split1h(x2, a2, l2), split1h(x3, a3, l3);
-    const f16 one = (f16)1.f, zero = (f16)0.f;
-    f16x8 v;
-    v[0] = a0, v[1] = a1, v[2] = a2, v[3] = a3;
-    v[4] = h ? one : l0, v[5] = h ? one : l1, v[6] = h ? zero : l2, v[7] = h ? zero : l3;
-    return v;
 }
 __device__ __forceinline__ f16x8 make_wh(float w0, float w1, float w2, float w3, float b, float sc, int h) {
     f16 a0, a1, a2, a3, l0, l1, l2, l3, bh, bl;
@@ -140,8 +124,7 @@
     if (i >= 2 * a.rows) return;
     float v[4];
     load_x<S>(x, i >> 1, v);
-    bool nf = not_finite(v[0]) || not_finite(v[1]) || not_finite(v[2]) || not_finite(v[3]);
-    nf = nf || fmaxf(fmaxf(fabsf(v[0]), fabsf(v[1])), fmaxf(fabsf(v[2]), fabsf(v[3]))) >= F16_OVERFLOW;
+    bool nf = x_unpackable(v);
     if (!(i & 1)) {
         const float e = extra[i >> 1];
         nf = nf || not_finite(e) || (extra_is_action && fabsf(e) >= F16_OVERFLOW);
@@ -161,6 +144,7 @@
     unsigned* wap;
     unsigned* smax;
     int* bad;
+    int* sbad;
 };
 constexpr int SCALE_SLICES = 16;
 __device__ __forceinline__ float pow2_for(float mx) {
@@ -202,9 +186,13 @@
         __syncthreads();
     }
     if (tid == 0) {
-        unsigned* dst = a.smax + ((long)net * gridDim.y + set) * 2;
-        atomicMax(dst, __float_as_uint(red[0]));
-        atomicMax(dst + 1, __float_as_uint(red2[0]));
+        unsigned* dst = a.smax + (((long)net * gridDim.y + set) * SCALE_SLICES + slice) * 2;
+        dst[0] = __float_as_uint(red[0]);
+        dst[1] = __float_as_uint(red2[0]);
+        if (net == 0 && set == 0 && slice == 0) {
+            *a.bad = a.sbad ? *a.sbad : 0;
+            if (a.sbad) *a.sbad = 0;
+        }
     }
 }
 __global__ __launch_bounds__(320) void prep_kernel(const PrepArgs a) {
@@ -218,8 +206,11 @@
     const int oW2 = critic ? L.cW2 : L.aW2, ob2 = critic ? L.cb2 : L.ab2, oW3 = critic ? L.cW3 : L.aW3, ob3 = critic ? L.cb3 : L.ab3;
     const int og2 = critic ? L.cg3 : L.ag2, obe2 = critic ? L.cbe3 : L.abe2, omm2 = critic ? L.cmm3 : L.amm2, omv2 = critic ? L.cmv3 : L.amv2;
     const float inv2n = (1.0f / sqrtf(st[omv2 + n] + BN_EPS)) * th[og2 + n], c3n = inv2n * th[oW3 + n];
-    const unsigned* smax = a.smax + ((long)net * gridDim.z + set) * 2;
-    const float SW = pow2_for(__uint_as_float(smax[0])), SWC = pow2_for(__uint_as_float(smax[1]));
+    const unsigned* smax = a.smax + ((long)net * gridDim.z + set) * SCALE_SLICES * 2;
+    unsigned m0 = 0, m1 = 0;
+#pragma unroll
+    for (int q = 0; q < SCALE_SLICES; ++q) m0 = max(m0, smax[2 * q]), m1 = max(m1, smax[2 * q + 1]);
+    const float SW = pow2_for(__uint_as_float(m0)), SWC = pow2_for(__uint_as_float(m1));
     float shw = 0.f;
     if (f < KP) {
         float w = 0.f, inv = 0.f;
@@ -1215,7 +1206,7 @@
 struct Plan {
     int grid, J;
     size_t Whi[4], Wlo[4], Wchi[2], Wclo[2], wf1h[4], vec[4], wap, a2, y, mu, dmu, g3, sm, sma, tz, t1p, s2raw, xfs, xfs2, partHs[3], partM[2],
-        partV[2], partG[2], bad, total;
+        partV[2], partG[2], bad, smax, total;
 };
 static Plan make_plan(int n_agents, int n_sets) {
     Plan pl;
@@ -1253,7 +1244,8 @@
         pl.partG[i] = take(4 * (size_t)pl.grid * KG * H2);
     }
     for (int i = 0; i < 3; ++i) pl.partHs[i] = take(4 * (size_t)pl.grid * 8 * 2);
-    pl.bad = take(sizeof(int) + sizeof(unsigned) * 4 * (size_t)n_sets * 2);
+    pl.bad = take(sizeof(int));
+    pl.smax = take(sizeof(unsigned) * 4 * (size_t)n_sets * SCALE_SLICES * 2);
     pl.total = o;
     return pl;
 }
@@ -1273,11 +1265,12 @@
 enum Phase { PH_CRITIC = 1, PH_ACTOR = 2, PH_BOTH = 3 };
 template <int S>
 static int run(int phases, const avd_mlp_layout& L, int n_agents, int n_sets, const float* theta, const float* stats, const float* theta_t,
-               const float* stats_t, const float* s, const float* a, const float* r, const float* s2, const float* aw, float gamma,
-               float high, float* grads, float* losses, unsigned char* ws, const Plan& pl, hipStream_t st) {
+               const float* stats_t, const float* s, const float* a, const float* r, const float* s2, const f16x8* pxfs,
+               const f16x8* pxfs2, int* sbad, const float* aw, float gamma, float high, float* grads, float* losses, unsigned char* ws,
+               const Plan& pl, hipStream_t st) {
     PrepArgs pa;
     pa.L = L, pa.S = S, pa.theta = theta, pa.stats = stats, pa.theta_t = theta_t, pa.stats_t = stats_t;
-    pa.wap = (unsigned*)(ws + pl.wap), pa.bad = (int*)(ws + pl.bad), pa.smax = (unsigned*)(ws + pl.bad + sizeof(int));
+    pa.wap = (unsigned*)(ws + pl.wap), pa.bad = (int*)(ws + pl.bad), pa.smax = (unsigned*)(ws + pl.smax), pa.sbad = sbad;
     NetP net[4];
     for (int i = 0; i < 4; ++i) {
         const bool critic = i & 1, target = i >= 2;
@@ -1292,7 +1285,8 @@
     const int P = n_agents / n_sets;
     const float inv_n = 1.0f / ((float)P * TILE);
     const long nrows = (long)n_agents * TILE;
-    f16x8 *xfs = (f16x8*)(ws + pl.xfs), *xfs2 = (f16x8*)(ws + pl.xfs2);
+    const f16x8* xfs = pxfs ? pxfs : (const f16x8*)(ws + pl.xfs);
+    const f16x8* xfs2 = pxfs ? pxfs2 : (const f16x8*)(ws + pl.xfs2);
     int* bad = (int*)(ws + pl.bad);
     float *a2 = (float*)(ws + pl.a2), *y = (float*)(ws + pl.y), *mu = (float*)(ws + pl.mu), *dmu = (float*)(ws + pl.dmu);
     float* g3 = (float*)(ws + pl.g3);
@@ -1329,14 +1323,15 @@
         fa.partG[i] = F(pl.partG[i]), fa.c3[i] = F(pl.vec[i]);
     fa.t1_from_g[0] = fa.t1_from_g[1] = 1, fa.t1p = F(pl.t1p), fa.s2raw = F(pl.s2raw);
     if (phases & PH_CRITIC) {
-        if (hipMemsetAsync(ws + pl.bad, 0, sizeof(int) + sizeof(unsigned) * 4 * (size_t)n_sets * 2, st) != hipSuccess)
-            return check_launch("avd_learn_set_split: memset");
         hipLaunchKernelGGL(scale_kernel, dim3(4, n_sets, SCALE_SLICES), dim3(256), 0, st, pa);
         hipLaunchKernelGGL(prep_kernel, dim3(H2, 4, n_sets), dim3(320), 0, st, pa);
         hipLaunchKernelGGL(prep1_kernel, dim3(NGT_MAX, 4, n_sets), dim3(64), 0, st, pa);
-        PackArgs pk;
-        pk.x[0] = s, pk.extra[0] = a, pk.outh[0] = xfs, pk.x[1] = s2, pk.extra[1] = r, pk.outh[1] = xfs2, pk.rows = nrows, pk.bad = bad;
-        hipLaunchKernelGGL(pack_x_kernel<S>, dim3((unsigned)((2 * nrows + 255) / 256), 2), dim3(256), 0, st, pk);
+        if (!pxfs) {
+            PackArgs pk;
+            pk.x[0] = s, pk.extra[0] = a, pk.outh[0] = (f16x8*)(ws + pl.xfs), pk.x[1] = s2, pk.extra[1] = r, pk.outh[1] = (f16x8*)(ws + pl.xfs2);
+            pk.rows = nrows, pk.bad = bad;
+            hipLaunchKernelGGL(pack_x_kernel<S>, dim3((unsigned)((2 * nrows + 255) / 256), 2), dim3(256), 0, st, pk);
+        }
         head(head_kernel<S, ActorS, OUT_TANH>, 2, xfs2, nullptr, nullptr, nullptr, a2, nullptr);
         head(head_kernel<S, CriticS, OUT_TD>, 3, xfs2, a2, r, nullptr, y, nullptr);
         h.sm = sma;
@@ -1399,21 +1394,24 @@
 
 static int split_entry(int phases, const char* who, const avd_mlp_layout* lay, int n_agents, int n_sets, const float* theta, const float* stats,
                        const float* theta_t, const float* stats_t, const float* s, const float* a, const float* r, const float* s2,
-                       const float* agent_weight, float gamma, float high, float* grads, float* losses, void* workspace,
-                       size_t workspace_bytes, void* stream) {
+                       const void* xfs, const void* xfs2, int32_t* sample_flag, const float* agent_weight, float gamma, float high,
+                       float* grads, float* losses, void* workspace, size_t workspace_bytes, void* stream) {
     int rc = fsplit::check_shape(lay, n_agents, n_sets, who);
     if (rc) return rc;
     const bool cr = phases & fsplit::PH_CRITIC;
-    AVD_REQUIRE(theta && stats && s && grads && workspace && (!cr || (theta_t && stats_t && a && r && s2)), "%s: null pointer", who);
+    AVD_REQUIRE(theta && stats && s && grads && workspace && (!cr || (theta_t && stats_t && a && r && (s2 || (xfs && xfs2 && sample_flag)))),
+                "%s: null pointer", who);
+    AVD_REQUIRE((size_t)xfs % 16 == 0 && (size_t)xfs2 % 16 == 0, "%s: xfs / xfs2 must be 16-byte aligned", who);
     const fsplit::Plan pl = fsplit::make_plan(n_agents, n_sets);
     AVD_REQUIRE(workspace_bytes >= pl.total, "%s: workspace %zu B < %zu B", who, workspace_bytes, pl.total);
-    if (cr && hipMemsetAsync(grads, 0, sizeof(float) * (size_t)n_sets * lay->theta_size, (hipStream_t)stream) != hipSuccess)
-        return check_launch("avd_learn_set_split: hipMemsetAsync(grads)");
+    if (phases == fsplit::PH_CRITIC && hipMemsetAsync(grads, 0, sizeof(float) * (size_t)n_sets * lay->theta_size, (hipStream_t)stream) != hipSuccess)
+        return check_launch("avd_learn_set_split_critic: hipMemsetAsync(grads)");
+    using fsplit::f16x8;
     if (lay->S == 4)
-        return fsplit::run<4>(phases, *lay, n_agents, n_sets, theta, stats, theta_t, stats_t, s, a, r, s2, agent_weight, gamma, high, grads,
-                              losses, (unsigned char*)workspace, pl, (hipStream_t)stream);
-    return fsplit::run<3>(phases, *lay, n_agents, n_sets, theta, stats, theta_t, stats_t, s, a, r, s2, agent_weight, gamma, high, grads, losses,
-                          (unsigned char*)workspace, pl, (hipStream_t)stream);
+        return fsplit::run<4>(phases, *lay, n_agents, n_sets, theta, stats, theta_t, stats_t, s, a, r, s2, (const f16x8*)xfs, (const f16x8*)xfs2,
+                              sample_flag, agent_weight, gamma, high, grads, losses, (unsigned char*)workspace, pl, (hipStream_t)stream);
+    return fsplit::run<3>(phases, *lay, n_agents, n_sets, theta, stats, theta_t, stats_t, s, a, r, s2, (const f16x8*)xfs, (const f16x8*)xfs2,
+                          sample_flag, agent_weight, gamma, high, grads, losses, (unsigned char*)workspace, pl, (hipStream_t)stream);
 }
 
 extern "C" int avd_learn_set_split_f16x3(const avd_mlp_layout* lay, int n_agents, int n_sets, const float* theta, const float* stats,
@@ -1421,7 +1419,15 @@
                                           const float* s2, const float* agent_weight, float gamma, float high, float* grads,
                                           float* losses, void* workspace, size_t workspace_bytes, void* stream) {
     return split_entry(fsplit::PH_BOTH, "avd_learn_set_split_f16x3", lay, n_agents, n_sets, theta, stats, theta_t, stats_t, s, a, r, s2,
-                       agent_weight, gamma, high, grads, losses, workspace, workspace_bytes, stream);
+                       nullptr, nullptr, nullptr, agent_weight, gamma, high, grads, losses, workspace, workspace_bytes, stream);
+}
+
+extern "C" int avd_learn_set_split_f16x3_packed(const avd_mlp_layout* lay, int n_agents, int n_sets, const float* theta, const float* stats,
+                                                 const float* theta_t, const float* stats_t, const float* s, const float* a, const float* r,
+                                                 const void* xfs, const void* xfs2, int32_t* sample_flag, const float* agent_weight, float gamma,
+                                                 float high, float* grads, float* losses, void* workspace, size_t workspace_bytes, void* stream) {
+    return split_entry(fsplit::PH_BOTH, "avd_learn_set_split_f16x3_packed", lay, n_agents, n_sets, theta, stats, theta_t, stats_t, s, a, r,
+                       nullptr, xfs, xfs2, sample_flag, agent_weight, gamma, high, grads, losses, workspace, workspace_bytes, stream);
 }
 
 extern "C" int avd_learn_set_split_bf16x3(const avd_mlp_layout* lay, int n_agents, int n_sets, const float* theta, const float* stats,
@@ -1437,11 +1443,11 @@
                                           const float* s2, const float* agent_weight, float gamma, float high, float* grads,
                                           float* losses, void* workspace, size_t workspace_bytes, void* stream) {
     return split_entry(fsplit::PH_CRITIC, "avd_learn_set_split_critic", lay, n_agents, n_sets, theta, stats, theta_t, stats_t, s, a, r, s2,
-                       agent_weight, gamma, high, grads, losses, workspace, workspace_bytes, stream);
+                       nullptr, nullptr, nullptr, agent_weight, gamma, high, grads, losses, workspace, workspace_bytes, stream);
 }
 
 extern "C" int avd_learn_set_split_actor(const avd_mlp_layout* lay, int n_agents, int n_sets, const float* theta, const float* stats,
                                          const float* s, float high, float* grads, void* workspace, size_t workspace_bytes, void* stream) {
     return split_entry(fsplit::PH_ACTOR, "avd_learn_set_split_actor", lay, n_agents, n_sets, theta, stats, nullptr, nullptr, s, nullptr, nullptr,
-                       nullptr, nullptr, 0.f, high, grads, nullptr, workspace, workspace_bytes, stream);
-}
+                       nullptr, nullptr, nullptr, nullptr, nullptr, 0.f, high, grads, nullptr, workspace, workspace_bytes, stream);
+}
diff --git a/avddpg_amd/csrc/fsplit_pack.h b/avddpg_amd/csrc/fsplit_pack.h
--- /dev/null
+++ b/avddpg_amd/csrc/fsplit_pack.h
@@ -0,0 +1,31 @@
+#pragma once
+#include "fset_common.h"
+
+namespace avd {
+namespace fsplit {
+using namespace fset;
+
+typedef _Float16 f16;
+typedef _Float16 f16x8 __attribute__((ext_vector_type(8)));
+constexpr float F16_OVERFLOW = 65520.f;
+
+__device__ __forceinline__ void split1h(float x, f16& hi, f16& lo) {
+    hi = (f16)x;
+    lo = (f16)(x - (float)hi);
+}
+__device__ __forceinline__ f16x8 make_xh(float x0, float x1, float x2, float x3, int h) {
+    f16 a0, a1, a2, a3, l0, l1, l2, l3;
+    split1h(x0, a0, l0), split1h(x1, a1, l1), split1h(x2, a2, l2), split1h(x3, a3, l3);
+    const f16 one = (f16)1.f, zero = (f16)0.f;
+    f16x8 v;
+    v[0] = a0, v[1] = a1, v[2] = a2, v[3] = a3;
+    v[4] = h ? one : l0, v[5] = h ? one : l1, v[6] = h ? zero : l2, v[7] = h ? zero : l3;
+    return v;
+}
+__device__ __forceinline__ bool x_unpackable(const float (&v)[4]) {
+    const bool nf = not_finite(v[0]) || not_finite(v[1]) || not_finite(v[2]) || not_finite(v[3]);
+    return nf || fmaxf(fmaxf(fabsf(v[0]), fabsf(v[1])), fmaxf(fabsf(v[2]), fabsf(v[3]))) >= F16_OVERFLOW;
+}
+
+}
+}
diff --git a/avddpg_amd/csrc/replay.hip b/avddpg_amd/csrc/replay.hip
--- a/avddpg_amd/csrc/replay.hip
+++ b/avddpg_amd/csrc/replay.hip
@@ -1,4 +1,5 @@
 #include "common.h"
+#include "fsplit_pack.h"
 
 namespace avd {
 
@@ -57,23 +58,65 @@
         s2[ab * S + (j - S - A - 1)] = val;
 }
 
-template <int S>
+template <int S, int ROW>
+__device__ __forceinline__ void pack_rows(const float (&v)[4][ROW], bool live, long total, long t, fsplit::f16x8* __restrict__ xfs,
+                                          fsplit::f16x8* __restrict__ xfs2, int32_t* __restrict__ flag) {
+    using namespace fsplit;
+    __shared__ uint4 stage[256 * 8];
+    const int lane = threadIdx.x & 63;
+    uint4* ws = stage + (threadIdx.x & ~63) * 8;
+    const long c0 = (t - lane) * 8;
+    auto at = [](int o, int c) { return 8 * o + (c ^ (o & 7)); };
+    bool bad = false;
+#pragma unroll
+    for (int in = 0; in < 2; ++in) {
+#pragma unroll
+        for (int k = 0; k < 4; ++k) {
+            const int off = in ? S + 2 : 0;
+            float x[4];
+#pragma unroll
+            for (int j = 0; j < 4; ++j) x[j] = j < S ? v[k][off + j] : 0.f;
+            const float e = v[k][S + in];
+            bad = bad || x_unpackable(x) || not_finite(e) || (!in && fabsf(e) >= F16_OVERFLOW);
+            ws[at(lane, 2 * k)] = __builtin_bit_cast(uint4, make_xh(x[0], x[1], x[2], x[3], 0));
+            ws[at(lane, 2 * k + 1)] = __builtin_bit_cast(uint4, make_xh(x[0], x[1], x[2], x[3], 1));
+        }
+        __syncthreads();
+        uint4* out = (uint4*)(in ? xfs2 : xfs);
+#pragma unroll
+        for (int q = 0; q < 8; ++q) {
+            const int c = 64 * q + lane;
+            if (c0 + c < 2 * total) out[c0 + c] = ws[at(c >> 3, c & 7)];
+        }
+        __syncthreads();
+    }
+    if (live && bad) atomicOr(flag, 1);
+}
+
+template <int S, bool PACK>
 __global__ __launch_bounds__(256) void replay_sample_kernel(int n_agents, int cap, int B, const float* __restrict__ ring,
                                                             uint32_t range, uint64_t seed, uint64_t counter,
                                                             int32_t* __restrict__ idx, float* __restrict__ s,
                                                             float* __restrict__ a, float* __restrict__ r,
-                                                            float* __restrict__ s2) {
+                                                            float* __restrict__ s2, fsplit::f16x8* __restrict__ xfs,
+                                                            fsplit::f16x8* __restrict__ xfs2, int32_t* __restrict__ flag) {
     constexpr int row = 2 * S + 2;
     const long t = (long)blockIdx.x * blockDim.x + threadIdx.x;
     const long total = (long)n_agents * B, base = t * 4;
-    if (base >= total) return;
+    const bool live = base < total;
+    if (!PACK && !live) return;
     const u32x4 rr = philox_at(seed, counter, (uint32_t)t, STREAM_REPLAY);
     const uint32_t w[4] = {rr.x, rr.y, rr.z, rr.w};
-    const int ag = (int)(base / B);
+    const int ag = live ? (int)(base / B) : 0;
     int ix[4];
     float v[4][row];
 #pragma unroll
     for (int k = 0; k < 4; ++k) {
+        if (!live) {
+#pragma unroll
+            for (int j = 0; j < row; ++j) v[k][j] = 0.f;
+            continue;
+        }
         ix[k] = (int32_t)(((uint64_t)w[k] * range) >> 32);
         const float2* src = (const float2*)(ring + ((long)ag * cap + ix[k]) * row);
 #pragma unroll
@@ -82,6 +125,8 @@
             v[k][2 * j] = q.x, v[k][2 * j + 1] = q.y;
         }
     }
+    if constexpr (PACK) pack_rows<S>(v, live, total, t, xfs, xfs2, flag);
+    if (!live) return;
     *(int4*)(idx + base) = make_int4(ix[0], ix[1], ix[2], ix[3]);
     *(float4*)(a + base) = make_float4(v[0][S], v[1][S], v[2][S], v[3][S]);
     *(float4*)(r + base) = make_float4(v[0][S + 1], v[1][S + 1], v[2][S + 1], v[3][S + 1]);
@@ -101,21 +146,38 @@
 
 using namespace avd;
 
+static int replay_sample(const char* who, int n_agents, int cap, int S, int A, int B, const float* ring, int range, uint64_t seed,
+                         uint64_t counter, int32_t* idx, float* s, float* a, float* r, float* s2, void* xfs, void* xfs2, int32_t* flag,
+                         void* stream) {
+    AVD_REQUIRE(n_agents > 0 && cap > 0 && (S == 3 || S == 4) && A == 1 && B > 0 && B % 4 == 0 && range > 0 && range <= cap,
+                "%s: n=%d cap=%d S=%d A=%d B=%d range=%d (S in {3, 4}, A = 1, B a multiple of 4)", who, n_agents, cap, S, A, B, range);
+    AVD_REQUIRE(ring && idx && s && a && r && s2, "%s: null pointer", who);
+    const bool pack = xfs != nullptr;
+    AVD_REQUIRE(!pack || (xfs2 && flag && (size_t)xfs % 16 == 0 && (size_t)xfs2 % 16 == 0),
+                "%s: xfs, xfs2 (16-byte aligned) and flag are needed together", who);
+    const long calls = (long)n_agents * B / 4;
+    const dim3 grid((unsigned)((calls + 255) / 256));
+    auto go = [&](auto kern) {
+        hipLaunchKernelGGL(kern, grid, dim3(256), 0, (hipStream_t)stream, n_agents, cap, B, ring, (uint32_t)range, seed, counter, idx, s,
+                           a, r, s2, (fsplit::f16x8*)xfs, (fsplit::f16x8*)xfs2, flag);
+    };
+    if (S == 4) pack ? go(replay_sample_kernel<4, true>) : go(replay_sample_kernel<4, false>);
+    else pack ? go(replay_sample_kernel<3, true>) : go(replay_sample_kernel<3, false>);
+    return check_launch(who);
+}
+
 extern "C" int avd_replay_sample_f32(int n_agents, int cap, int S, int A, int B, const float* ring, int range, uint64_t seed,
                                      uint64_t counter, int32_t* idx, float* s, float* a, float* r, float* s2, void* stream) {
-    AVD_REQUIRE(n_agents > 0 && cap > 0 && (S == 3 || S == 4) && A == 1 && B > 0 && B % 4 == 0 && range > 0 && range <= cap,
-                "avd_replay_sample_f32: n=%d cap=%d S=%d A=%d B=%d range=%d (S in {3, 4}, A = 1, B a multiple of 4)", n_agents, cap, S,
-                A, B, range);
-    AVD_REQUIRE(ring && idx && s && a && r && s2, "avd_replay_sample_f32: null pointer");
-    const long calls = (long)n_agents * B / 4;
-    const dim3 grid((unsigned)((calls + 255) / 256));
-    if (S == 4)
-        hipLaunchKernelGGL(replay_sample_kernel<4>, grid, dim3(256), 0, (hipStream_t)stream, n_agents, cap, B, ring, (uint32_t)range,
-                           seed, counter, idx, s, a, r, s2);
-    else
-        hipLaunchKernelGGL(replay_sample_kernel<3>, grid, dim3(256), 0, (hipStream_t)stream, n_agents, cap, B, ring, (uint32_t)range,
-                           seed, counter, idx, s, a, r, s2);
-    return check_launch("avd_replay_sample_f32");
+    return replay_sample("avd_replay_sample_f32", n_agents, cap, S, A, B, ring, range, seed, counter, idx, s, a, r, s2, nullptr, nullptr,
+                         nullptr, stream);
+}
+
+extern "C" int avd_replay_sample_packed_f32(int n_agents, int cap, int S, int A, int B, const float* ring, int range, uint64_t seed,
+                                            uint64_t counter, int32_t* idx, float* s, float* a, float* r, float* s2, void* xfs,
+                                            void* xfs2, int32_t* flag, void* stream) {
+    AVD_REQUIRE(xfs, "avd_replay_sample_packed_f32: null pointer");
+    return replay_sample("avd_replay_sample_packed_f32", n_agents, cap, S, A, B, ring, range, seed, counter, idx, s, a, r, s2, xfs, xfs2,
+                         flag, stream);
 }
 
 extern "C" int avd_replay_add_f32(int n_agents, int cap, int S, int A, float* ring, int64_t counter,
diff --git a/avddpg_amd/trainer.py b/avddpg_amd/trainer.py
--- a/avddpg_amd/trainer.py
+++ b/avddpg_amd/trainer.py
@@ -124,6 +124,7 @@
                          and (lay.H1, lay.H2, lay.A) == (256, 128, 1) and lay.S in (3, 4))
         can_overlap = group is not None and self.shared and self.shared_engine == "fused3"
         self.overlap_allreduce = False if overlap_allreduce is None else bool(overlap_allreduce)
+        self.replay.pack = self.shared_engine == "fused3" and not self.overlap_allreduce
         if self.overlap_allreduce and not can_overlap:
             raise ValueError("overlap_allreduce needs a process group and shared_engine='fused3' (the two-phase learn call)")
         self._side = None
@@ -311,7 +312,7 @@
                 self._flag_exchanged = carry is not None
                 return
             self.agents.learn_set_fused(s, a, r, s2, P * M, grads=self.set_grads, losses=self.set_losses, agent_weight=aw,
-                                        split=self.shared_engine == "fused3")
+                                        split=self.shared_engine == "fused3", packed=self.replay.packed)
         else:
             if aw_dev is not None:
                 rw = aw_dev.view(P, M).transpose(0, 1).reshape(M, P, 1).expand(M, P, B).reshape(M, P * B).contiguous()
diff --git a/avddpg_amd/vec.py b/avddpg_amd/vec.py
--- a/avddpg_amd/vec.py
+++ b/avddpg_amd/vec.py
@@ -199,6 +199,9 @@
         self.a = torch.zeros(self.n, self.B, self.A, **f32)
         self.r = torch.zeros(self.n, self.B, **f32)
         self.s2 = torch.zeros(self.n, self.B, self.S, **f32)
+        self.pack = False
+        self.packed = None
+        self._pack_bufs = None
 
     def add(self, s_prev, action, reward, s_next, x_stride):
         call("avd_replay_add_f32", self.n, self.cap, self.S, self.A, ptr(self.ring), self.buffer_counter, ptr(s_prev),
@@ -226,9 +229,20 @@
         return self.s, self.a, self.r, self.s2
 
     def sample(self, host_idx=None):
+        self.packed = None
         if self.rng != "host" and host_idx is None and self.A == 1 and self.S in (3, 4) and self.B % 4 == 0:
-            call("avd_replay_sample_f32", self.n, self.cap, self.S, self.A, self.B, ptr(self.ring), self.sample_range(), self.seed,
-                 self.samples, ptr(self.idx), ptr(self.s), ptr(self.a), ptr(self.r), ptr(self.s2), stream_handle())
+            args = (self.n, self.cap, self.S, self.A, self.B, ptr(self.ring), self.sample_range(), self.seed, self.samples,
+                    ptr(self.idx), ptr(self.s), ptr(self.a), ptr(self.r), ptr(self.s2))
+            if self.pack:
+                if self._pack_bufs is None:
+                    u8 = dict(dtype=torch.uint8, device=self.device)
+                    self._pack_bufs = (torch.empty(self.n, self.B, 32, **u8), torch.empty(self.n, self.B, 32, **u8),
+                                       torch.zeros(1, dtype=torch.int32, device=self.device))
+                xfs, xfs2, flag = self._pack_bufs
+                call("avd_replay_sample_packed_f32", *args, ptr(xfs), ptr(xfs2), ptr(flag), stream_handle())
+                self.packed = self._pack_bufs
+            else:
+                call("avd_replay_sample_f32", *args, stream_handle())
             self.samples += 1
             return self.s, self.a, self.r, self.s2
         self.draw_indices(host_idx)
@@ -318,7 +332,7 @@
              self.high, ptr(grads), ptr(losses), ptr(ws), ws.numel(), stream_handle())
         return grads
 
-    def learn_set_fused(self, s, a, r, s2, n_agents, grads=None, losses=None, agent_weight=None, split=False, phase=None):
+    def learn_set_fused(self, s, a, r, s2, n_agents, grads=None, losses=None, agent_weight=None, split=False, phase=None, packed=None):
         import ctypes
         self._check_agent_major(s, a, r, s2, n_agents, agent_weight)
         if grads is None:
@@ -333,6 +347,16 @@
             setattr(self, attr, ws)
         if phase is not None and not split:
             raise _hip.AvdError("phase= needs split=True (csrc/fsplit.hip)")
+        if packed is not None:
+            if not split or phase is not None:
+                raise _hip.AvdError("packed= needs split=True and the whole call (phase=None)")
+            xfs, xfs2, flag = packed
+            if xfs.numel() != n_agents * self.lay.B * 32 or xfs2.numel() != xfs.numel():
+                raise _hip.AvdError(f"packed fragments hold {xfs.numel()} bytes, {n_agents} agents need {n_agents * self.lay.B * 32}")
+            call("avd_learn_set_split_f16x3_packed", self._layp, n_agents, self.n_sets, ptr(self.theta), ptr(self.stats),
+                 ptr(self.theta_t), ptr(self.stats_t), ptr(s), ptr(a), ptr(r), ptr(xfs), ptr(xfs2), ptr(flag), ptr(agent_weight),
+                 self.config.gamma, self.high, ptr(grads), ptr(losses), ptr(ws), ws.numel(), stream_handle())
+            return grads
         if phase == "actor":
             call("avd_learn_set_split_actor", self._layp, n_agents, self.n_sets, ptr(self.theta), ptr(self.stats), ptr(s), self.high,
                  ptr(grads), ptr(ws), ws.numel(), stream_handle())
diff --git a/include/avddpg_hip.h b/include/avddpg_hip.h
--- a/include/avddpg_hip.h
+++ b/include/avddpg_hip.h
@@ -147,6 +147,9 @@
 
 int avd_replay_sample_f32(int n_agents, int cap, int S, int A, int B, const float* ring, int range, uint64_t seed, uint64_t counter,
                           int32_t* idx, float* s, float* a, float* r, float* s2, void* stream);
+int avd_replay_sample_packed_f32(int n_agents, int cap, int S, int A, int B, const float* ring, int range, uint64_t seed,
+                                 uint64_t counter, int32_t* idx, float* s, float* a, float* r, float* s2, void* xfs, void* xfs2,
+                                 int32_t* flag, void* stream);
 
 int avd_actor_forward_set_f32(const avd_mlp_layout* lay, int n_agents, int n_sets, const float* theta, const float* stats,
                               const float* states, int x_stride, float high, float* out, const int32_t* run_if_nonzero, void* stream);
@@ -175,6 +178,10 @@
                                const float* theta_t, const float* stats_t, const float* s, const float* a, const float* r,
                                const float* s2, const float* agent_weight, float gamma, float high, float* grads, float* losses,
                                void* workspace, size_t workspace_bytes, void* stream);
+int avd_learn_set_split_f16x3_packed(const avd_mlp_layout* lay, int n_agents, int n_sets, const float* theta, const float* stats,
+                                     const float* theta_t, const float* stats_t, const float* s, const float* a, const float* r,
+                                     const void* xfs, const void* xfs2, int32_t* sample_flag, const float* agent_weight, float gamma,
+                                     float high, float* grads, float* losses, void* workspace, size_t workspace_bytes, void* stream);
 
 int avd_learn_set_split_bf16x3(const avd_mlp_layout* lay, int n_agents, int n_sets, const float* theta, const float* stats,
                                const float* theta_t, const float* stats_t, const float* s, const float* a, const float* r,
```

Result: no change. 1.990 million, median of 6 (+0.6%).
